# kfkq/DQMC

Hardware: AMD Instinct MI355X
Metric: MC sweeps/sec, 2D Hubbard N=256 Ltau=200 (higher is better)
Workload: dtype f64; 1 GPU; cfg3: 16x16 Hubbard U=8.0 beta=8.0 Ltau=200 n_stab=10 t=1 mu=-0.1; chains_per_gpu=1, n_chains_total=1, parallelism=independent chains, 1 gpu x 1 chain

## Files before the change

dqmc_amd/csrc/common.h:

```cpp
#pragma once

#include <hip/hip_runtime.h>
#include <cstdint>
#include <memory>
#include <string>

struct dqmc_engine;

namespace dq {

constexpr int WAVE = 64;

void set_error(const std::string& msg);
const char* get_error();

#define DQ_HIP(call)                                                                    \
    do {                                                                                \
        hipError_t _e = (call);                                                         \
        if (_e != hipSuccess) {                                                         \
            ::dq::set_error(std::string(#call) + ": " + hipGetErrorString(_e));         \
            return -2;                                              \
        }                                                                               \
    } while (0)

#define DQ_TRY(expr)                \
    do {                            \
        int _rc = (expr);           \
        if (_rc != 0) return _rc;   \
    } while (0)

template <class T, hipError_t (*Free)(void*)> struct HipDelete { void operator()(T* p) const { (void)Free(p); } };
template <class T> using DevPtr = std::unique_ptr<T[], HipDelete<T, hipFree>>;
using PinnedPtr = std::unique_ptr<char[], HipDelete<char, hipHostFree>>;
template <class T> int dev_alloc(DevPtr<T>& out, size_t count) {
    void* p = nullptr;
    DQ_HIP(hipMalloc(&p, sizeof(T) * count));
    out.reset(static_cast<T*>(p));
    return 0;
}

constexpr int DQ_STATUS_PIVOT = 1;
constexpr int DQ_STATUS_COOP_QR = 2;
constexpr int DQ_STATUS_HANDOFF = 4;
constexpr int DQ_STATUS_CENSUS = 8;

struct Mat {
    double* p = nullptr;
    long stride = 0;
    __host__ __device__ double* at(int c) const { return p + (long)c * stride; }
};
struct CMat {
    const double* p = nullptr;
    long stride = 0;
    CMat() = default;
    __host__ __device__ CMat(const double* p_, long s) : p(p_), stride(s) {}
    __host__ __device__ CMat(const Mat& m) : p(m.p), stride(m.stride) {}
    __host__ __device__ const double* at(int c) const { return p + (long)c * stride; }
};
using Vec = Mat;
using CVec = CMat;

struct GemmDesc {
    CMat A, B;
    Mat C;
    Mat CT{nullptr, 0};
    CVec rs, ks, cs;
    int n = 0;
    int transA = 0;
    int accumulate = 0;
};
int launch_gemm(const GemmDesc& g, int n_chains, hipStream_t s);

int launch_build_expv(const int8_t* fields, long f_stride, int nt, int n, const double* tab_expv ,
                      double* expv, double* invexpv, long v_stride, int n_chains, hipStream_t s);
int launch_split_d(CVec d, Vec dl_inv, Vec ds, double* logsum, int n, int n_chains, hipStream_t s);
int launch_split_d2(CVec d1, Vec dl1, Vec ds1, CVec d2, Vec dl2, Vec ds2, int n, int n_chains, hipStream_t s);
int launch_measure_equal_time(CMat G, double* out, long out_stride, int L1, int L2, int accumulate, int n_chains, hipStream_t s);
int launch_measure_unequal_time(const double* Gtt, const double* Gt0, const double* G0t, double* out, long out_stride, int L1, int L2, int nt,
                                int accumulate, int n_chains, hipStream_t s);
int launch_axpb_identity(CMat in, Mat out, double a, double b, int n, int n_chains, hipStream_t s);
int launch_copy(CMat in, Mat out, long count, int n_chains, hipStream_t s);
int launch_set_identity(Mat out, int n, int n_chains, hipStream_t s);
int launch_transpose_scale(CMat in, Mat out, CVec rs, int n, int n_chains, hipStream_t s);
int launch_max_abs_diff(CMat A, CMat B, double* err, long err_stride, int n, int n_chains, hipStream_t s);
int launch_add_scaled_cols(CMat A, CMat B, CVec cs, Mat C, int n, int n_chains, hipStream_t s);
int launch_scale_rows(CMat in, CVec rs, Mat out, int n, int n_chains, hipStream_t s);
struct DevStats { double acc_rate, max_err, sum_err, n_err; long long n_accepted, n_proposed; };
int launch_fold_stats(DevStats* st, const int* acc, long acc_stride, int n_slices, const double* err, long err_stride, int n_err,
                      int n, int nt, int n_chains, hipStream_t s);

struct QrWork {
    double* tau; long tau_stride;
    int* jpvt; long jpvt_stride;
    unsigned long long* sync = nullptr; long sync_stride = 0;
    int* abort_words = nullptr;
    int* info = nullptr;
    double* pw = nullptr; long pw_stride = 0;
    bool pw_two_launch = false;
    int* pivpos = nullptr; long pivpos_stride = 0;
};
bool qr_panel_fused_fits(int n);
bool qr_panel_fused_default(int n);
long qr_panel_work_doubles(int n, bool two_launch);
int launch_qr_panel(Mat A, Mat L, QrWork w, int n, int n_chains, hipStream_t s);
long qrcp_coop_sync_granules(int n);
int qrcp_coop_workgroups(int n, int n_chains);
enum class QrFamily { Panel, ColumnOwner, Cooperative, Streaming };
int launch_to_ldr(QrFamily f, Mat A, Mat L, Vec d, Mat R, QrWork w, int n, int n_chains, hipStream_t s);

int launch_lu_blocked(Mat A, int* perm, long perm_stride, int* rowpos, long rowpos_stride, double* logabsdet, int accumulate_logdet,
                      int* info, int n, int n_chains, hipStream_t s);
int launch_lu_solve(CMat LU, const int* perm, long perm_stride, Mat X, CVec dg, int mode, int n, int n_chains, hipStream_t s);

int launch_tri_solve(CMat R, const int* perm, long perm_stride, Mat X, CVec dg, double* scratch, long scratch_stride, int n, int n_chains, hipStream_t s);

bool gj_fused_fits(int n);
bool gj_fused_default(int n);
int launch_gj_solve(Mat A, Mat B, Mat X, Mat SA, double* tinv, int* perm, long perm_stride, int* rowpos, int* rowpos_alt, long rowpos_stride,
                    double* logabsdet, int accumulate_logdet, int* info, int n, int n_chains, bool fused, hipStream_t s);

struct UpdateTables {
    double rb[4][3];
    double delta[4][3];
    double ev[4];
    double iev[4];
    double pad[32];
};
struct SliceRider {
    const double* A = nullptr; const double* B = nullptr; double* C = nullptr; const double* rs = nullptr; const double* ks = nullptr;
    __host__ __device__ GemmDesc gemm(int n) const { GemmDesc g; g.A = CMat(A, 0); g.B = CMat(B, 0); g.C = Mat{C, 0}; g.rs = CVec(rs, 0); g.ks = CVec(ks, 0); g.n = n; return g; }
};
struct UpdateDesc {
    Mat G;
    int8_t* fields; long f_stride;
    double* expv; double* invexpv; long v_stride;
    const UpdateTables* tabs;
    const int32_t* perm; const uint8_t* kprop; const double* u; long rs_stride;
    double* Upanel; double* Wpanel; long panel_stride;
    double* Cpanel = nullptr;
    int* state; long state_stride;
    double* prep; long prep_stride;
    Mat GT{nullptr, 0};
    int gt_valid = 0;
    void* slice_sync = nullptr;
    unsigned slice_epoch = 0;
    int slice_absent_tile = -1;
    int slice_absent_l = -1;
    int slice_late_tile = -1, slice_late_us = 0;
    int* info = nullptr;
    int* acc_out; long acc_stride;
    int n, nt;
    SliceRider rider;
};
constexpr int UPDATE_KD = 32;

struct SliceSync {
    unsigned long long seq; unsigned int error; unsigned int solo_count; unsigned int pad[12];
    unsigned int arrive[496];
};
constexpr size_t SLICE_SYNC_BYTES = 2048;
static_assert(sizeof(SliceSync) == SLICE_SYNC_BYTES, "SliceSync layout");
constexpr unsigned SLICE_EPOCH_LIMIT = 1u << 24;
constexpr unsigned SLICE_SOLO_BIT = 1u << 30, SLICE_FINAL_BIT = 1u << 31;
constexpr int SLICE_RING_ROWS = 2 * UPDATE_KD;
constexpr unsigned SLICE_K_MASK = 0xffu, SLICE_BASE_SHIFT = 8, SLICE_BASE_MASK = SLICE_RING_ROWS - 1;
__host__ __device__ inline unsigned slice_tag(unsigned epoch, unsigned window) { return (epoch << 8) | window; }
enum class SlicePath { PersistentWalk, PersistentWalkDump, PersistentSubmatrix, Solo, Pairs, PairsTailSolo };
int launch_update_slice(SlicePath path, const UpdateDesc& d, int l, int acc_slot, int n_chains, hipStream_t s);
int launch_update_slice_sm(const UpdateDesc& d, int l, int acc_slot, int n_chains, hipStream_t s);
int slice_flush_workgroups(int n);
bool slice_reserve(int device, int n, int n_chains);
void slice_release(int device, int n, int n_chains);
int launch_rank1(Mat G, int i, double delta, double* scratch , long scratch_stride, int n, int n_chains, hipStream_t s);

int launch_rng_fill(int32_t* perm, uint8_t* kprop, double* u, int n, int nt, unsigned long long seed, unsigned first_chain, unsigned h,
                    int n_chains, hipStream_t s);

struct CbDesc {
    CMat in;
    Mat out{nullptr, 0}, outT{nullptr, 0};
    const int* partner = nullptr;
    int n_groups = 0, reverse = 0, inverse = 0;
    const double* par = nullptr; long par_stride = 0;
    CVec rs_in, cs_in, rs_out, cs_out;
    int n = 0;
};
int launch_cb_apply(const CbDesc& d, int n_chains, hipStream_t s);

int update_init_device();
int update_sm_init_device();
int qr_init_device();
int qr_colown_init_device();
int init_device_kernels(int device);

struct EngineFieldsView { int device, n, nt, n_chains; int8_t* fields; hipStream_t stream; };
int engine_fields_view(dqmc_engine* h, EngineFieldsView* v);
int engine_fields_changed(dqmc_engine* h);
int engine_exchange_scratch(dqmc_engine* h, int8_t** saved, int8_t** recv, int** tab);

}
```

dqmc_amd/csrc/engine.hip:

```cpp
#include "common.h"
#include "../../include/dqmc_hip.h"

#include <cmath>
#include <cstdlib>
#include <cstring>
#include <map>
#include <memory>
#include <mutex>
#include <vector>

namespace dq {

static thread_local std::string g_err;
void set_error(const std::string& msg) { g_err = msg; }
const char* get_error() { return g_err.c_str(); }

int init_device_kernels(int device) {
    static std::mutex mu; static bool done[64] = {};
    std::lock_guard<std::mutex> lk(mu);
    if (device < 0 || device >= 64) { set_error("device ordinal out of range"); return -1; }
    if (done[device]) return 0;
    DQ_HIP(hipSetDevice(device));
    DQ_TRY(update_init_device()); DQ_TRY(update_sm_init_device()); DQ_TRY(qr_init_device()); DQ_TRY(qr_colown_init_device());
    done[device] = true;
    return 0;
}

struct Switches { bool qr_panel; int qr_panel_fused, gj_fused; bool qr_streaming, walk_submatrix, lu_classic, slice_multikernel, bbar_rider, slice_stream; };
static const Switches& switches() {
    static const Switches sw = [] {
        const char* panel = getenv("DQMC_QR_PANEL");
        const char* fused = getenv("DQMC_QR_PANEL_FUSED");
        const char* gj = getenv("DQMC_GJ_FUSED");
        const char* rider = getenv("DQMC_BBAR_RIDER");
        const char* stream = getenv("DQMC_SLICE_STREAM");
        return Switches{!(panel && atoi(panel) == 0), fused ? (atoi(fused) != 0 ? 1 : 0) : -1, gj ? (atoi(gj) != 0 ? 1 : 0) : -1, getenv("DQMC_QR_STREAMING") != nullptr, getenv("DQMC_WALK_SUBMATRIX") != nullptr,
                        getenv("DQMC_LU_CLASSIC") != nullptr, getenv("DQMC_SLICE_MULTIKERNEL") != nullptr, !(rider && atoi(rider) == 0), !(stream && atoi(stream) == 0)};
    }();
    return sw;
}

constexpr int GJ_MAX_N = 1024, GJ_MAX_CHAINS = 8;
constexpr int TRI_MAX_N = 640;

static QrFamily pick_qr(int n, int chains, bool allow_panel) {
    const Switches& sw = switches();
    if (sw.qr_streaming) return QrFamily::Streaming;
    if (allow_panel && sw.qr_panel && n >= 64 && n <= 1024 && n % 16 == 0 && chains <= 8) return QrFamily::Panel;
    if (n <= 256) return QrFamily::ColumnOwner;
    return qrcp_coop_workgroups(n, chains) <= 200 ? QrFamily::Cooperative : QrFamily::Streaming;
}

struct KernelPlan {
    QrFamily qr;
    enum class Solve { GaussJordan, BlockedLu } solve;
    enum class Rinv { Blocked, PerColumn } rinv;
    static KernelPlan pick(int n, int chains) {
        return KernelPlan{pick_qr(n, chains, true),
                          n <= GJ_MAX_N && chains <= GJ_MAX_CHAINS && !switches().lu_classic ? Solve::GaussJordan : Solve::BlockedLu,
                          n <= TRI_MAX_N ? Rinv::Blocked : Rinv::PerColumn};
    }
};

static SlicePath pick_slice_path(int n, int chains, bool reserved) {
    const Switches& sw = switches();
    const bool walk = n <= 256;
    if (sw.slice_multikernel) return SlicePath::Pairs;
    if (reserved) return walk && !sw.walk_submatrix ? (sw.slice_stream ? SlicePath::PersistentWalk : SlicePath::PersistentWalkDump) : SlicePath::PersistentSubmatrix;
    if (!walk) return SlicePath::Pairs;
    return chains >= 224 ? SlicePath::Solo : SlicePath::PairsTailSolo;
}
static bool is_persistent_walk(SlicePath p) { return p == SlicePath::PersistentWalk || p == SlicePath::PersistentWalkDump; }
static bool is_persistent(SlicePath p) { return is_persistent_walk(p) || p == SlicePath::PersistentSubmatrix; }

struct LdrRef {
    Mat L; Vec d; Mat R;
    int* jpvt = nullptr;
    bool* tri = nullptr;
    Mat X{nullptr, 0};
    bool* xok = nullptr;
    void touch() const { if (xok) *xok = false; }
};
struct LdrStore {
    int n = 0, C = 0;
    DevPtr<double> L, d, R, X;
    DevPtr<int> jpvt;
    std::unique_ptr<bool[]> tri, xok;
    int alloc(int k, int n_, int C_, bool with_x = false) {
        n = n_; C = C_;
        const size_t nn = (size_t)n * n;
        DQ_TRY(dev_alloc(L, (size_t)k * C * nn)); DQ_TRY(dev_alloc(d, (size_t)k * C * n));
        DQ_TRY(dev_alloc(R, (size_t)k * C * nn)); DQ_TRY(dev_alloc(jpvt, (size_t)k * C * n));
        if (with_x) DQ_TRY(dev_alloc(X, (size_t)k * C * nn));
        tri.reset(new bool[k]()); xok.reset(new bool[k]());
        return 0;
    }
    LdrRef at(int i) const {
        const long nn = (long)n * n;
        LdrRef f{Mat{L.get() + (long)i * C * nn, nn}, Vec{d.get() + (long)i * C * n, (long)n}, Mat{R.get() + (long)i * C * nn, nn},
                 jpvt.get() + (long)i * C * n, &tri[i]};
        if (X) { f.X = Mat{X.get() + (long)i * C * nn, nn}; f.xok = &xok[i]; }
        return f;
    }
};

struct Ctx {
    int n = 0, C = 0, device = 0;
    long nn = 0;
    hipStream_t stream = nullptr;
    static constexpr int NT = 6, NV = 5;
    DevPtr<double> pool;
    DevPtr<double> vpool;
    DevPtr<int> ipool;
    DevPtr<unsigned long long> qsync;
    DevPtr<int> qabort;
    DevPtr<double> tinv;
    DevPtr<double> qpw;
    bool gj_fused = false;
    bool qpw_two_launch = false;
    DevPtr<int> qpivpos;
    DevPtr<double> trinv;
    KernelPlan plan{};

    Mat T(int k) const { return Mat{pool.get() + (long)k * C * nn, nn}; }
    Vec V(int k) const { return Vec{vpool.get() + (long)k * C * n, (long)n}; }
    int* jpvt() const { return ipool.get(); }
    int* lperm() const { return ipool.get() + (long)C * n; }
    int* rowpos() const { return ipool.get() + 2L * C * n; }
    int* rowpos_alt() const { return ipool.get() + 3L * C * n; }
    int* info() const { return ipool.get() + 4L * C * n; }

    int init(int n_, int C_, int device_) {
        n = n_; C = C_; device = device_; nn = (long)n * n;
        DQ_HIP(hipSetDevice(device));
        DQ_TRY(init_device_kernels(device));
        DQ_HIP(hipStreamCreateWithFlags(&stream, hipStreamNonBlocking));
        DQ_TRY(dev_alloc(pool, (size_t)NT * C * nn));
        DQ_TRY(dev_alloc(vpool, (size_t)NV * C * n));
        DQ_TRY(dev_alloc(ipool, 4L * C * n + 4));
        plan = KernelPlan::pick(n, C);
        if (plan.qr == QrFamily::Cooperative) { DQ_TRY(dev_alloc(qsync, (size_t)qrcp_coop_sync_granules(n) * C)); DQ_TRY(dev_alloc(qabort, C)); }
        if (plan.qr == QrFamily::Panel) {
            const int fused = switches().qr_panel_fused;
            qpw_two_launch = !(fused < 0 ? qr_panel_fused_default(n) : fused == 1 && qr_panel_fused_fits(n));
            const size_t qpw_count = (size_t)qr_panel_work_doubles(n, qpw_two_launch) * C;
            DQ_TRY(dev_alloc(qpw, qpw_count)); DQ_TRY(dev_alloc(qpivpos, (size_t)n * C));
            DQ_HIP(hipMemsetAsync(qpw.get(), 0, sizeof(double) * qpw_count, stream));
        }
        if (plan.solve == KernelPlan::Solve::GaussJordan) {
            DQ_TRY(dev_alloc(tinv, (size_t)2048 * C));
            const int fused = switches().gj_fused;
            gj_fused = fused < 0 ? gj_fused_default(n) : fused == 1 && gj_fused_fits(n);
        }
        if (plan.rinv == KernelPlan::Rinv::Blocked) DQ_TRY(dev_alloc(trinv, (size_t)16 * (n + 16) * C));
        DQ_HIP(hipMemsetAsync(ipool.get(), 0, sizeof(int) * (4L * C * n + 4), stream));
        return 0;
    }
    ~Ctx() { if (stream) (void)hipStreamDestroy(stream); }

    int gemm(CMat A, CMat B, Mat Cm, CVec rs = CVec(), CVec ks = CVec(), CVec cs = CVec(), int transA = 0, int accumulate = 0, Mat CT = Mat{nullptr, 0}) {
        GemmDesc g; g.A = A; g.B = B; g.C = Cm; g.CT = CT; g.rs = rs; g.ks = ks; g.cs = cs; g.n = n; g.transA = transA; g.accumulate = accumulate;
        return launch_gemm(g, C, stream);
    }
    int to_ldr(Mat A, LdrRef out, bool direct = true) {
        const bool keep = direct && out.jpvt != nullptr;
        QrWork w{V(4).p, (long)n, keep ? out.jpvt : jpvt(), (long)n};
        w.sync = qsync.get(); w.sync_stride = qrcp_coop_sync_granules(n); w.abort_words = qabort.get(); w.info = info();
        w.pw = qpw.get(); w.pw_stride = qr_panel_work_doubles(n, qpw_two_launch); w.pw_two_launch = qpw_two_launch; w.pivpos = qpivpos.get(); w.pivpos_stride = n;
        if (out.tri) *out.tri = keep;
        out.touch();
        return launch_to_ldr(plan.qr, A, out.L, out.d, out.R, w, n, C, stream);
    }
    int r_inverse_scaled(LdrRef F, CVec dinv, Mat scratch, Mat lu_scratch, Mat* Xout) {
        const Mat X = F.X.p ? F.X : scratch;
        *Xout = X;
        if (F.xok && *F.xok) return 0;
        if (F.tri && *F.tri && F.jpvt) {
            if (plan.rinv == KernelPlan::Rinv::Blocked) DQ_TRY(launch_tri_solve(F.R, F.jpvt, n, X, dinv, trinv.get(), 16L * (n + 16), n, C, stream));
            else DQ_TRY(launch_lu_solve(F.R, F.jpvt, n, X, dinv, 2, n, C, stream));
        } else {
            DQ_TRY(launch_copy(F.R, lu_scratch, nn, C, stream));
            DQ_TRY(launch_lu_blocked(lu_scratch, lperm(), n, rowpos(), n, nullptr, 0, info(), n, C, stream));
            DQ_TRY(launch_lu_solve(lu_scratch, lperm(), n, X, dinv, 1, n, C, stream));
        }
        if (F.xok) *F.xok = true;
        return 0;
    }
    int mat_mul_ldr(CMat M, LdrRef F, LdrRef out) {
        DQ_TRY(gemm(M, F.L, T(0), CVec(), CVec(), CVec(F.d)));
        LdrRef q{out.L, out.d, T(1)};
        DQ_TRY(to_ldr(T(0), q));
        if (out.tri) *out.tri = false;
        out.touch();
        return gemm(T(1), F.R, out.R);
    }
    int ldr_mul_mat(LdrRef F, CMat M, LdrRef out) {
        DQ_TRY(gemm(F.R, M, T(0), CVec(F.d)));
        LdrRef q{T(1), out.d, out.R, out.jpvt, out.tri};
        q.xok = out.xok;
        DQ_TRY(to_ldr(T(0), q));
        return gemm(F.L, T(1), out.L);
    }
    int ldr_mul_ldr(LdrRef F1, LdrRef F2, LdrRef out) {
        DQ_TRY(gemm(F1.R, F2.L, T(0), CVec(F1.d), CVec(), CVec(F2.d)));
        LdrRef q{T(1), out.d, T(2)};
        DQ_TRY(to_ldr(T(0), q));
        if (out.tri) *out.tri = false;
        out.touch();
        DQ_TRY(gemm(F1.L, T(1), out.L));
        return gemm(T(2), F2.R, out.R);
    }
    int solve(Mat M, Mat RHS, Mat out, double* logdet_acc, Mat* Y) {
        if (plan.solve == KernelPlan::Solve::GaussJordan) {
            DQ_TRY(launch_gj_solve(M, RHS, out, T(5), tinv.get(), lperm(), n, rowpos(), rowpos_alt(), n, logdet_acc, 1, info(), n, C, gj_fused, stream));
            *Y = out; return 0;
        }
        DQ_TRY(launch_lu_blocked(M, lperm(), n, rowpos(), n, logdet_acc, 1, info(), n, C, stream));
        DQ_TRY(launch_lu_solve(M, lperm(), n, RHS, CVec(), 0, n, C, stream));
        *Y = RHS; return 0;
    }
    int inv_I_plus_ldr(LdrRef F, Mat G, double* logdet ) {
        DQ_TRY(launch_split_d(F.d, V(0), V(1), logdet, n, C, stream));
        Mat X; DQ_TRY(r_inverse_scaled(F, V(0), T(1), T(0), &X));
        DQ_TRY(launch_add_scaled_cols(X, F.L, V(1), T(2), n, C, stream));
        DQ_TRY(launch_transpose_scale(T(2), T(3), CVec(), n, C, stream));
        DQ_TRY(launch_transpose_scale(X, T(4), CVec(), n, C, stream));
        Mat Y; DQ_TRY(solve(T(3), T(4), T(0), logdet, &Y));
        return launch_transpose_scale(Y, G, CVec(), n, C, stream);
    }
    int inv_I_plus_ldr_mul_ldr(LdrRef F1, LdrRef F2, Mat G, Mat GT = Mat{nullptr, 0}) {
        DQ_TRY(launch_split_d2(F1.d, V(0), V(1), F2.d, V(2), V(3), n, C, stream));
        Mat X; DQ_TRY(r_inverse_scaled(F2, V(2), T(1), T(0), &X));
        DQ_TRY(gemm(F1.L, X, T(2), V(0), CVec(), CVec(), 1));
        DQ_TRY(gemm(F1.R, F2.L, T(2), V(1), CVec(), V(3), 0, 1));
        DQ_TRY(launch_transpose_scale(F1.L, T(3), V(0), n, C, stream));
        Mat Y; DQ_TRY(solve(T(2), T(3), T(0), nullptr, &Y));
        return gemm(X, Y, G, CVec(), CVec(), CVec(), 0, 0, GT);
    }
    int inv_invldr_plus_ldr(LdrRef F1, LdrRef F2, Mat G, bool negate) {
        DQ_TRY(launch_split_d(F1.d, V(0), V(1), nullptr, n, C, stream));
        DQ_TRY(launch_split_d(F2.d, V(2), V(3), nullptr, n, C, stream));
        Mat X; DQ_TRY(r_inverse_scaled(F2, V(2), T(1), T(0), &X));
        DQ_TRY(gemm(F1.L, X, T(2), V(0), CVec(), CVec(), 1));
        DQ_TRY(gemm(F1.R, F2.L, T(2), V(1), CVec(), V(3), 0, 1));
        DQ_TRY(launch_scale_rows(F1.R, V(1), T(3), n, C, stream));
        Mat Y; DQ_TRY(solve(T(2), T(3), T(0), nullptr, &Y));
        DQ_TRY(gemm(X, Y, G));
        if (negate) DQ_TRY(launch_axpb_identity(G, G, -1.0, 0.0, n, C, stream));
        return 0;
    }
};

static int take_status(const Ctx& c, int* bits = nullptr) {
    int w[4] = {0, 0, 0, 0};
    DQ_HIP(hipMemcpy(w, c.info(), sizeof w, hipMemcpyDeviceToHost));
    if (bits) *bits = w[0];
    if (w[0] == 0) return 0;
    (void)hipMemset(c.info(), 0, sizeof w);
    if (w[0] & DQ_STATUS_HANDOFF) {
        set_error("persistent slice kernel: a workgroup that had checked in stopped answering (device fault or pre-emption beyond the spin bound); the chain state is undefined -- set the fields again and call dqmc_init; this engine uses the scan / flush kernel pairs from now on");
    } else if (w[0] & DQ_STATUS_CENSUS) {
        char msg[640];
        snprintf(msg, sizeof msg, "persistent sub-matrix slice kernel: its workgroups did not all become resident at time slice %d (device shared with other "
                 "work?).  That slice and every later slice of the call(s) in flight proposed NOTHING (fields unchanged there, acceptance counts 0, their part of "
                 "the random stream is spent); wraps and stabilisations ran, so fields, G and the stack are consistent with each other, but the sweep is not the "
                 "one the stream describes from that slice on.  This engine uses the scan / flush kernel pairs from now on: restore the fields of the last "
                 "completed sweep and call dqmc_init, or keep the state as a valid (shortened) sweep", w[1] - 1);
        set_error(msg);
    } else if (w[0] & DQ_STATUS_COOP_QR) {
        set_error("cooperative QRCP gave up waiting for a partner workgroup (not co-resident?)");
    } else {
        set_error("LU factorisation hit a zero or NaN pivot");
    }
    return DQMC_ENUMERIC;
}

struct Engine {
    int n = 0, nt = 0, n_stab = 0, n_stack = 0, C = 1, device = 0;
    long nn = 0;
    std::vector<int> loc_l_end;
    std::vector<double> g_host, gamma_host, eta_host;
    std::vector<unsigned char> seen;
    Ctx ctx;
    hipStream_t s = nullptr;

    DevPtr<double> expK, invexpK;
    bool cb = false; int cb_groups = 0;
    DevPtr<int> cb_partner;
    DevPtr<double> cb_par;
    DevPtr<int8_t> fields;
    DevPtr<double> expv, invexpv;
    DevPtr<UpdateTables> tabs; DevPtr<double> tab8;
    bool gt_valid = false;
    bool gt_check = false; long long gt_checks = 0; DevPtr<double> gt_err;
    DevPtr<double> G, Gtmp, GT;
    DevPtr<double> pg_eye, pg_ones;
    DevPtr<double> bb0, bb1;
    long long rider_launches = 0;
    LdrStore stack;
    LdrStore spare;
    DevPtr<double> logdet;
    DevPtr<int32_t> rs_perm; DevPtr<uint8_t> rs_k; DevPtr<double> rs_u;
    PinnedPtr h_stage;
    bool rng_seeded = false; uint64_t rng_seed = 0; uint32_t rng_first_chain = 0, rng_counter = 0;
    hipEvent_t stage_free = nullptr;
    DevPtr<double> Upanel, Wpanel;
    int panel_rows = UPDATE_KD;
    DevPtr<double> Cpanel;
    struct InitBatch { DevPtr<double> bb, tau; LdrStore f; } ib;
    DevPtr<int> state;
    DevPtr<double> prep;
    DevPtr<double> meas_now, meas_sum;
    struct UnequalTime { DevPtr<double> G[3], tmp, err, meas_now, meas_sum; LdrStore bt; } ut;
    bool ut_valid = false; long long ut_meas_count = 0;
    struct HalfWarp { DevPtr<double> expK, invexpK, out; } hw;
    long long meas_count = 0;
    DevPtr<char> slice_sync;
    bool reserved = false;
    SlicePath slice_path = SlicePath::Pairs;
    unsigned slice_epoch = 0;
    int slice_absent_l = -1;
    int slice_late_tile = -1, slice_late_us = 0;
    int slice_absent_tile = -1;
    DevPtr<int> acc;
    struct Exchange { DevPtr<int8_t> saved, recv; DevPtr<int> tab; } xch;
    DevPtr<double> err;
    DevPtr<DevStats> dstats;
    bool stack_valid = false;
    bool profiling = false;
    std::vector<std::pair<hipEvent_t, hipEvent_t>> ev_pairs;
    size_t ev_used = 0;
    double upd_ms = 0.0; long long upd_launches = 0; long long upd_accept_base = 0;

    Mat mG() const { return Mat{G.get(), nn}; }
    CVec ev(int l) const { return CVec(expv.get() + (long)l * n, (long)nt * n); }
    CVec iev(int l) const { return CVec(invexpv.get() + (long)l * n, (long)nt * n); }
    int stack_idx(int l) const { return l / n_stab; }
    int local_l(int l) const { return l % n_stab; }

    ~Engine() {
        if (s) (void)hipStreamSynchronize(s);
        if (reserved) slice_release(device, n, C);
        for (auto& p : ev_pairs) { (void)hipEventDestroy(p.first); (void)hipEventDestroy(p.second); }
        if (stage_free) (void)hipEventDestroy(stage_free);
    }

    int create(int device_, int C_, int n_, int nt_, int n_stab_, const double* g, const double* gamma, const double* eta,
               const double* eK, const double* ieK) {
        device = device_; C = C_; n = n_; nt = nt_; n_stab = n_stab_; nn = (long)n * n;
        n_stack = (int)std::ceil(static_cast<double>(nt) / n_stab);
        loc_l_end.assign(n_stack, n_stab - 1);
        if (nt % n_stab != 0) loc_l_end[n_stack - 1] = nt % n_stab - 1;
        g_host.assign(g, g + C); gamma_host.assign(gamma, gamma + 4); eta_host.assign(eta, eta + 4);
        DQ_TRY(ctx.init(n, C, device)); s = ctx.stream;
        reserved = slice_reserve(device, n, C);
        slice_path = pick_slice_path(n, C, reserved);
        if (const char* a = getenv("DQMC_DEBUG_SLICE_ABSENT")) { slice_absent_tile = atoi(a); if (const char* c = strchr(a, ':')) slice_absent_l = atoi(c + 1); }
        if (const char* a = getenv("DQMC_DEBUG_SLICE_LATE")) { slice_late_tile = atoi(a); if (const char* c = strchr(a, ':')) slice_late_us = atoi(c + 1); }
        DQ_TRY(dev_alloc(expK, C * nn)); DQ_TRY(dev_alloc(invexpK, C * nn));
        DQ_TRY(dev_alloc(fields, (size_t)C * nt * n)); DQ_TRY(dev_alloc(expv, (size_t)C * nt * n)); DQ_TRY(dev_alloc(invexpv, (size_t)C * nt * n));
        DQ_TRY(dev_alloc(tabs, C)); DQ_TRY(dev_alloc(tab8, (size_t)C * 8));
        if (C == 1) { DQ_TRY(dev_alloc(pg_eye, nn)); DQ_TRY(dev_alloc(pg_ones, (size_t)n)); DQ_TRY(launch_set_identity(Mat{pg_eye.get(), nn}, n, 1, s)); const std::vector<double> one_h((size_t)n, 1.0); DQ_HIP(hipMemcpy(pg_ones.get(), one_h.data(), sizeof(double) * n, hipMemcpyHostToDevice)); }
        DQ_TRY(dev_alloc(G, C * nn)); DQ_TRY(dev_alloc(Gtmp, C * nn)); DQ_TRY(dev_alloc(GT, C * nn)); DQ_TRY(dev_alloc(bb0, C * nn)); DQ_TRY(dev_alloc(bb1, C * nn));
        DQ_TRY(stack.alloc(n_stack, n, C, C <= 8)); DQ_TRY(spare.alloc(1, n, C));
        DQ_TRY(dev_alloc(logdet, C));
        DQ_TRY(dev_alloc(rs_perm, (size_t)C * nt * n)); DQ_TRY(dev_alloc(rs_k, (size_t)C * nt * n)); DQ_TRY(dev_alloc(rs_u, (size_t)C * nt * n));
        panel_rows = slice_path == SlicePath::PersistentWalk ? SLICE_RING_ROWS : UPDATE_KD;
        DQ_TRY(dev_alloc(Upanel, (size_t)C * panel_rows * n)); DQ_TRY(dev_alloc(Wpanel, (size_t)C * panel_rows * n)); DQ_TRY(dev_alloc(Cpanel, (size_t)C * UPDATE_KD * UPDATE_KD));
        DQ_TRY(dev_alloc(state, (size_t)C * 4)); DQ_TRY(dev_alloc(prep, (size_t)C * 4 * n)); DQ_TRY(dev_alloc(meas_now, (size_t)C * (3 + n))); DQ_TRY(dev_alloc(meas_sum, (size_t)C * (3 + n))); DQ_HIP(hipMemsetAsync(meas_sum.get(), 0, sizeof(double) * C * (3 + n), s)); DQ_TRY(dev_alloc(slice_sync, (size_t)C * SLICE_SYNC_BYTES)); DQ_HIP(hipMemsetAsync(slice_sync.get(), 0, (size_t)C * SLICE_SYNC_BYTES, s)); DQ_TRY(dev_alloc(acc, (size_t)C * nt)); DQ_TRY(dev_alloc(err, (size_t)C * n_stack));
        DQ_TRY(dev_alloc(dstats, C));
        void* stage = nullptr;
        DQ_HIP(hipHostMalloc(&stage, (size_t)C * nt * n * (sizeof(int32_t) + sizeof(uint8_t) + sizeof(double)), hipHostMallocDefault)); h_stage.reset(static_cast<char*>(stage));
        DQ_HIP(hipEventCreateWithFlags(&stage_free, hipEventDisableTiming));
        DQ_HIP(hipEventRecord(stage_free, s));
        DQ_HIP(hipMemcpyAsync(expK.get(), eK, sizeof(double) * C * nn, hipMemcpyHostToDevice, s));
        DQ_HIP(hipMemcpyAsync(invexpK.get(), ieK, sizeof(double) * C * nn, hipMemcpyHostToDevice, s));
        DQ_HIP(hipMemsetAsync(fields.get(), 0, (size_t)C * nt * n, s));
        DQ_HIP(hipMemsetAsync(G.get(), 0, sizeof(double) * C * nn, s));
        DQ_HIP(hipMemsetAsync(dstats.get(), 0, sizeof(DevStats) * C, s));
        DQ_HIP(hipMemsetAsync(logdet.get(), 0, sizeof(double) * C, s));
        DQ_HIP(hipMemsetAsync(state.get(), 0, sizeof(int) * C * 4, s));
        std::vector<UpdateTables> ht(C); std::vector<double> h8((size_t)C * 8);
        static const int proposal[4][3] = {{1, 2, 3}, {0, 2, 3}, {0, 1, 3}, {0, 1, 2}};
        const double alpha = -1.0;
        for (int c = 0; c < C; ++c) {
            std::memset(&ht[c], 0, sizeof(UpdateTables));
            for (int o = 0; o < 4; ++o) for (int k = 0; k < 3; ++k) {
                const int nf = proposal[o][k];
                const double gammaR = gamma[nf] / gamma[o];
                const double d_eta = eta[nf] - eta[o];
                const double bosonR = std::exp(alpha * g[c] * d_eta);
                ht[c].rb[o][k] = gammaR * bosonR;
                ht[c].delta[o][k] = (1.0 / bosonR) - 1.0;
            }
            for (int f = 0; f < 4; ++f) { ht[c].ev[f] = std::exp(g[c] * eta[f]); ht[c].iev[f] = std::exp(-g[c] * eta[f]); h8[(size_t)c * 8 + f] = ht[c].ev[f]; h8[(size_t)c * 8 + 4 + f] = ht[c].iev[f]; }
        }
        DQ_HIP(hipMemcpyAsync(tabs.get(), ht.data(), sizeof(UpdateTables) * C, hipMemcpyHostToDevice, s));
        DQ_HIP(hipMemcpyAsync(tab8.get(), h8.data(), sizeof(double) * C * 8, hipMemcpyHostToDevice, s));
        DQ_TRY(launch_build_expv(fields.get(), (long)nt * n, nt, n, tab8.get(), expv.get(), invexpv.get(), (long)nt * n, C, s));
        DQ_HIP(hipStreamSynchronize(s));
        return 0;
    }

    int cb_apply(CMat in, Mat out, Mat outT, bool reverse, bool inverse, CVec rs_in, CVec cs_in, CVec rs_out, CVec cs_out, int chains, long par_stride) {
        CbDesc d; d.in = in; d.out = out; d.outT = outT; d.partner = cb_partner.get(); d.n_groups = cb_groups; d.reverse = reverse ? 1 : 0; d.inverse = inverse ? 1 : 0;
        d.par = cb_par.get(); d.par_stride = par_stride; d.rs_in = rs_in; d.cs_in = cs_in; d.rs_out = rs_out; d.cs_out = cs_out; d.n = n;
        return launch_cb_apply(d, chains, s);
    }
    int set_checkerboard(int n_groups, const int32_t* bonds, const int32_t* group_sizes, const double* ch, const double* sh, const double* f) {
        if (n_groups < 1 || n_groups > 64 || !bonds || !group_sizes || !ch || !sh || !f) { set_error("set_checkerboard: bad argument"); return DQMC_EINVAL; }
        if (n > 4096) { set_error("set_checkerboard: n_sites > 4096"); return DQMC_EINVAL; }
        std::vector<int> partner((size_t)n_groups * n);
        size_t b = 0;
        for (int g = 0; g < n_groups; ++g) {
            int* pt = partner.data() + (size_t)g * n;
            for (int i = 0; i < n; ++i) pt[i] = i;
            if (group_sizes[g] < 0 || group_sizes[g] > n / 2) { set_error("set_checkerboard: a group holds at most n_sites/2 bonds"); return DQMC_EINVAL; }
            for (int k = 0; k < group_sizes[g]; ++k, ++b) {
                const int i = bonds[2 * b], j = bonds[2 * b + 1];
                if (i < 0 || i >= n || j < 0 || j >= n || i == j) { set_error("set_checkerboard: bond site out of range"); return DQMC_EINVAL; }
                if (pt[i] != i || pt[j] != j) { set_error("set_checkerboard: the bonds of one group must be disjoint"); return DQMC_EINVAL; }
                pt[i] = j; pt[j] = i;
            }
        }
        std::vector<double> par((size_t)C * 4);
        for (int c = 0; c < C; ++c) {
            if (!(f[c] > 0.0) || !std::isfinite(ch[c]) || !std::isfinite(sh[c])) { set_error("set_checkerboard: diag_factor must be positive, cosh / sinh finite"); return DQMC_EINVAL; }
            par[4 * c] = ch[c]; par[4 * c + 1] = sh[c]; par[4 * c + 2] = f[c]; par[4 * c + 3] = 1.0 / f[c];
        }
        DQ_HIP(hipStreamSynchronize(s));
        if (!cb_par) DQ_TRY(dev_alloc(cb_par, (size_t)C * 4));
        DevPtr<int> pt;
        DQ_TRY(dev_alloc(pt, partner.size()));
        DQ_HIP(hipMemcpy(pt.get(), partner.data(), sizeof(int) * partner.size(), hipMemcpyHostToDevice));
        DQ_HIP(hipMemcpy(cb_par.get(), par.data(), sizeof(double) * par.size(), hipMemcpyHostToDevice));
        cb_partner = std::move(pt); cb_groups = n_groups; cb = true;
        Mat id{bb0.get(), nn};
        DQ_TRY(launch_set_identity(id, n, C, s));
        DQ_TRY(cb_apply(id, Mat{expK.get(), nn}, Mat{nullptr, 0}, false, false, CVec(), CVec(), CVec(), CVec(), C, 4));
        DQ_TRY(cb_apply(id, Mat{invexpK.get(), nn}, Mat{nullptr, 0}, true, true, CVec(), CVec(), CVec(), CVec(), C, 4));
        stack_valid = false; gt_valid = false; ut_valid = false;
        DQ_HIP(hipStreamSynchronize(s));
        return 0;
    }

    int Bbar(int is, Mat* out) {
        const int l0 = is * n_stab;
        Mat cur{bb0.get(), nn}, nxt{bb1.get(), nn};
        DQ_TRY(launch_scale_rows(CMat(expK.get(), nn), ev(l0), cur, n, C, s));
        for (int loc = 1; loc <= loc_l_end[is]; ++loc) {
            if (cb) DQ_TRY(cb_apply(cur, nxt, Mat{nullptr, 0}, false, false, CVec(), CVec(), ev(l0 + loc), CVec(), C, 4));
            else DQ_TRY(ctx.gemm(CMat(expK.get(), nn), cur, nxt, ev(l0 + loc)));
            std::swap(cur, nxt);
        }
        *out = cur; return 0;
    }
    int init() {
        if (C == 1 && n <= 256 && nt % n_stab == 0 && n_stack >= 2) return init_batched();
        const LdrRef tmp = spare.at(0);
        for (int i = n_stack - 1; i >= 0; --i) {
            Mat bb; DQ_TRY(Bbar(i, &bb));
            if (i == n_stack - 1) DQ_TRY(ctx.to_ldr(bb, stack.at(i)));
            else { DQ_TRY(ctx.to_ldr(bb, tmp)); DQ_TRY(ctx.ldr_mul_ldr(stack.at(i + 1), tmp, stack.at(i))); }
        }
        stack_valid = true;
        gt_valid = false;
        return ctx.inv_I_plus_ldr(stack.at(0), mG(), logdet.get());
    }
    int init_batched() {
        const int S = n_stack;
        if (!ib.tau) {
            InitBatch b; DQ_TRY(dev_alloc(b.bb, (size_t)2 * S * nn)); DQ_TRY(dev_alloc(b.tau, (size_t)S * n)); DQ_TRY(b.f.alloc(S, n, 1));
            ib = std::move(b);
        }
        const long bstride = (long)n_stab * n;
        Mat cur{ib.bb.get(), nn}, nxt{ib.bb.get() + (size_t)S * nn, nn};
        DQ_TRY(launch_scale_rows(CMat(expK.get(), 0), CVec(expv.get(), bstride), cur, n, S, s));
        for (int loc = 1; loc < n_stab; ++loc) {
            if (cb) DQ_TRY(cb_apply(cur, nxt, Mat{nullptr, 0}, false, false, CVec(), CVec(), CVec(expv.get() + (long)loc * n, bstride), CVec(), S, 0));
            else {
                GemmDesc g; g.A = CMat(expK.get(), 0); g.B = cur; g.C = nxt; g.rs = CVec(expv.get() + (long)loc * n, bstride); g.n = n;
                DQ_TRY(launch_gemm(g, S, s));
            }
            std::swap(cur, nxt);
        }
        const LdrRef all = ib.f.at(0);
        QrWork w{ib.tau.get(), (long)n, all.jpvt, (long)n};
        w.info = ctx.info();
        DQ_TRY(launch_to_ldr(pick_qr(n, S, false), cur, all.L, all.d, all.R, w, n, S, s));
        const LdrRef last = stack.at(S - 1), own = ib.f.at(S - 1);
        DQ_TRY(launch_copy(own.L, last.L, nn, 1, s));
        DQ_TRY(launch_copy(own.R, last.R, nn, 1, s));
        DQ_HIP(hipMemcpyAsync(last.d.p, own.d.p, sizeof(double) * n, hipMemcpyDeviceToDevice, s));
        DQ_HIP(hipMemcpyAsync(last.jpvt, own.jpvt, sizeof(int) * n, hipMemcpyDeviceToDevice, s));
        *last.tri = true; last.touch();
        for (int i = S - 2; i >= 0; --i) DQ_TRY(ctx.ldr_mul_ldr(stack.at(i + 1), ib.f.at(i), stack.at(i)));
        stack_valid = true;
        gt_valid = false;
        return ctx.inv_I_plus_ldr(stack.at(0), mG(), logdet.get());
    }
    int wrap_forward(int l) {
        if (cb) {
            DQ_TRY(cb_apply(mG(), Mat{nullptr, 0}, ctx.T(0), false, false, CVec(), CVec(), CVec(), CVec(), C, 4));
            gt_valid = use_gt();
            return cb_apply(ctx.T(0), Mat{GT.get(), nn}, mG(), false, true, CVec(), CVec(), iev(l), ev(l), C, 4);
        }
        DQ_TRY(ctx.gemm(CMat(expK.get(), nn), mG(), ctx.T(0)));
        gt_valid = use_gt();
        return ctx.gemm(ctx.T(0), CMat(invexpK.get(), nn), mG(), ev(l), CVec(), iev(l), 0, 0, use_gt() ? Mat{GT.get(), nn} : Mat{nullptr, 0});
    }
    bool piggyback() const { return C == 1 && !cb && n <= 256 && pg_eye != nullptr; }
    bool bbar_rides() const { return piggyback() && is_persistent_walk(slice_path) && switches().bbar_rider; }
    SliceRider rider_forward(int l, const double* Pprev, double* Pnext) const {
        SliceRider r; r.A = expK.get(); r.B = Pprev; r.C = Pnext; r.rs = expv.get() + (long)(l - 1) * n;
        return r;
    }
    SliceRider rider_backward(int l, const double* Pprev, double* Pnext) const {
        SliceRider r; r.A = Pprev; r.B = expK.get(); r.C = Pnext; r.ks = expv.get() + (long)l * n;
        return r;
    }
    int wrap_forward_piggy(int l, const double* Pprev, double* Pnext) {
        GemmDesc g; g.A = CMat(expK.get(), 0); g.B = CMat(G.get(), (long)(Pprev - G.get())); g.C = Mat{ctx.T(0).p, (long)(Pnext - ctx.T(0).p)};
        g.rs = CVec(pg_ones.get(), (long)((expv.get() + (long)(l - 1) * n) - pg_ones.get())); g.n = n;
        DQ_TRY(launch_gemm(g, 2, s));
        gt_valid = use_gt();
        return ctx.gemm(ctx.T(0), CMat(invexpK.get(), nn), mG(), ev(l), CVec(), iev(l), 0, 0, use_gt() ? Mat{GT.get(), nn} : Mat{nullptr, 0});
    }
    int wrap_backward_piggy(int l, const double* Pprev, double* Pnext) {
        DQ_TRY(ctx.gemm(CMat(invexpK.get(), nn), mG(), ctx.T(0), CVec(), iev(l)));
        gt_valid = use_gt();
        GemmDesc g; g.A = CMat(ctx.T(0).p, (long)(Pprev - ctx.T(0).p)); g.B = CMat(expK.get(), 0); g.C = Mat{G.get(), (long)(Pnext - G.get())};
        g.ks = CVec(expv.get() + (long)l * n, 0); g.n = n;
        if (use_gt()) g.CT = Mat{GT.get(), (long)(ctx.T(1).p - GT.get())};
        return launch_gemm(g, 2, s);
    }
    int wrap_backward(int l) {
        if (cb) {
            DQ_TRY(cb_apply(mG(), Mat{nullptr, 0}, ctx.T(0), true, true, iev(l), ev(l), CVec(), CVec(), C, 4));
            gt_valid = use_gt();
            return cb_apply(ctx.T(0), Mat{GT.get(), nn}, mG(), true, false, CVec(), CVec(), CVec(), CVec(), C, 4);
        }
        DQ_TRY(ctx.gemm(CMat(invexpK.get(), nn), mG(), ctx.T(0), CVec(), iev(l)));
        gt_valid = use_gt();
        return ctx.gemm(ctx.T(0), CMat(expK.get(), nn), mG(), CVec(), ev(l), CVec(), 0, 0, use_gt() ? Mat{GT.get(), nn} : Mat{nullptr, 0});
    }
    bool use_gt() const { return n <= 256 || slice_path == SlicePath::PersistentSubmatrix; }
    UpdateDesc udesc() const {
        UpdateDesc d; d.G = mG(); d.fields = fields.get(); d.f_stride = (long)nt * n; d.expv = expv.get(); d.invexpv = invexpv.get(); d.v_stride = (long)nt * n;
        d.tabs = tabs.get(); d.perm = rs_perm.get(); d.kprop = rs_k.get(); d.u = rs_u.get(); d.rs_stride = (long)nt * n; d.Upanel = Upanel.get(); d.Wpanel = Wpanel.get(); d.Cpanel = Cpanel.get();
        d.panel_stride = (long)panel_rows * n; d.state = state.get(); d.state_stride = 4; d.prep = prep.get(); d.prep_stride = 4L * n; d.slice_sync = is_persistent(slice_path) ? slice_sync.get() : nullptr; d.slice_epoch = slice_epoch; d.slice_absent_tile = slice_absent_tile; d.slice_absent_l = slice_absent_l; d.slice_late_tile = slice_late_tile; d.slice_late_us = slice_late_us; d.GT = Mat{GT.get(), nn}; d.gt_valid = gt_valid ? 1 : 0; d.info = ctx.info(); d.acc_out = acc.get(); d.acc_stride = nt; d.n = n; d.nt = nt;
        return d;
    }
    int local_update(int l, const SliceRider* rider = nullptr) {
        hipEvent_t e0 = nullptr, e1 = nullptr;
        if (profiling) {
            if (ev_used == ev_pairs.size()) { hipEvent_t a, b; DQ_HIP(hipEventCreate(&a)); DQ_HIP(hipEventCreate(&b)); ev_pairs.emplace_back(a, b); }
            e0 = ev_pairs[ev_used].first; e1 = ev_pairs[ev_used].second; ++ev_used;
            DQ_HIP(hipEventRecord(e0, s));
        }
        if (is_persistent(slice_path)) {
            if (++slice_epoch >= SLICE_EPOCH_LIMIT) { DQ_HIP(hipMemsetAsync(slice_sync.get(), 0, (size_t)C * SLICE_SYNC_BYTES, s)); slice_epoch = 1; }
        }
        UpdateDesc d = udesc();
        if (rider) d.rider = *rider;
        DQ_TRY(launch_update_slice(slice_path, d, l, l, C, s));
        if (rider) ++rider_launches;
        if (profiling) DQ_HIP(hipEventRecord(e1, s));
        return 0;
    }
    int check_stream(const char* who, const int32_t* perm, const uint8_t* kprop, const double* u, size_t rows) {
        if (!perm || !kprop || !u) { set_error(std::string(who) + ": null random-stream pointer"); return DQMC_EINVAL; }
        seen.assign((size_t)n, 0);
        for (size_t row = 0; row < rows; ++row) {
            const int32_t* pr = perm + row * n; const uint8_t* kr = kprop + row * n; const unsigned char mark = (unsigned char)(1 + (row & 1));
            if ((row & 1) == 0) std::fill(seen.begin(), seen.end(), 0);
            for (int idx = 0; idx < n; ++idx) {
                const int32_t i = pr[idx];
                if (i < 0 || i >= n || seen[i] == mark || kr[idx] > 2) { set_error(std::string(who) + ": perm is not a permutation of the sites, or kprop > 2"); return DQMC_EINVAL; }
                seen[i] = mark;
            }
        }
        return 0;
    }
    int upload_stream(const int32_t* perm, const uint8_t* kprop, const double* u) {
        const size_t cnt = (size_t)C * nt * n;
        DQ_TRY(check_stream("sweep", perm, kprop, u, (size_t)C * nt));
        DQ_HIP(hipEventSynchronize(stage_free));
        char* base = h_stage.get();
        double* hu = reinterpret_cast<double*>(base);
        int32_t* hp = reinterpret_cast<int32_t*>(base + cnt * sizeof(double));
        uint8_t* hk = reinterpret_cast<uint8_t*>(base + cnt * (sizeof(double) + sizeof(int32_t)));
        std::memcpy(hu, u, cnt * sizeof(double)); std::memcpy(hp, perm, cnt * sizeof(int32_t)); std::memcpy(hk, kprop, cnt);
        DQ_HIP(hipMemcpyAsync(rs_u.get(), hu, cnt * sizeof(double), hipMemcpyHostToDevice, s));
        DQ_HIP(hipMemcpyAsync(rs_perm.get(), hp, cnt * sizeof(int32_t), hipMemcpyHostToDevice, s));
        DQ_HIP(hipMemcpyAsync(rs_k.get(), hk, cnt, hipMemcpyHostToDevice, s));
        DQ_HIP(hipEventRecord(stage_free, s));
        return 0;
    }
    int fill_stream(uint32_t h) {
        return launch_rng_fill(rs_perm.get(), rs_k.get(), rs_u.get(), n, nt, rng_seed, rng_first_chain, h, C, s);
    }
    int stage_stream(const char* who, const int32_t* perm, const uint8_t* kprop, const double* u) {
        if (perm && kprop && u) return upload_stream(perm, kprop, u);
        if (perm || kprop || u) { set_error(std::string(who) + ": pass all three random-stream arrays or none"); return DQMC_EINVAL; }
        if (!rng_seeded) { set_error(std::string(who) + ": null random-stream pointer (the engine draws its own stream only after dqmc_rng_seed)"); return DQMC_EINVAL; }
        if (rng_counter == UINT32_MAX) { set_error(std::string(who) + ": the half-sweep counter of this seed is used up (2^32 - 1)"); return DQMC_ERANGE; }
        DQ_TRY(fill_stream(rng_counter));
        ++rng_counter;
        return 0;
    }
    int sweep_fwd() {
        int n_err = 0;
        DQ_HIP(hipMemsetAsync(err.get(), 0, sizeof(double) * C * n_stack, s));
        const bool pg = piggyback(), ride = bbar_rides();
        double* Pcur = bb0.get(); double* Pnxt = bb1.get();
        for (int l = 0; l < nt; ++l) {
            const int is = stack_idx(l), loc = local_l(l);
            if (pg && loc >= 1) {
                const double* Pprev = loc == 1 ? pg_eye.get() : Pcur;
                if (ride) { const SliceRider r = rider_forward(l, Pprev, Pnxt); DQ_TRY(wrap_forward(l)); DQ_TRY(local_update(l, &r)); }
                else { DQ_TRY(wrap_forward_piggy(l, Pprev, Pnxt)); DQ_TRY(local_update(l)); }
                std::swap(Pcur, Pnxt);
            } else { DQ_TRY(wrap_forward(l)); DQ_TRY(local_update(l)); }
            if (loc == loc_l_end[is]) {
                std::swap(G, Gtmp);
                Mat bb;
                if (pg) {
                    if (loc == 0) DQ_TRY(launch_scale_rows(CMat(expK.get(), nn), ev(l), Mat{Pnxt, nn}, n, C, s));
                    else DQ_TRY(ctx.gemm(CMat(expK.get(), nn), CMat(Pcur, nn), Mat{Pnxt, nn}, ev(l)));
                    std::swap(Pcur, Pnxt); bb = Mat{Pcur, nn};
                } else DQ_TRY(Bbar(is, &bb));
                if (is == 0) DQ_TRY(ctx.to_ldr(bb, stack.at(0)));
                else DQ_TRY(ctx.mat_mul_ldr(bb, stack.at(is - 1), stack.at(is)));
                gt_valid = false;
                if (l == nt - 1) DQ_TRY(ctx.inv_I_plus_ldr(stack.at(is), mG(), logdet.get()));
                else DQ_TRY(ctx.inv_I_plus_ldr_mul_ldr(stack.at(is), stack.at(is + 1), mG()));
                DQ_TRY(launch_max_abs_diff(CMat(Gtmp.get(), nn), mG(), err.get() + n_err, n_stack, n, C, s));
                ++n_err;
            }
        }
        return launch_fold_stats(dstats.get(), acc.get(), nt, nt, err.get(), n_stack, n_err, n, nt, C, s);
    }
    int sweep_bwd() {
        int n_err = 0;
        DQ_HIP(hipMemsetAsync(err.get(), 0, sizeof(double) * C * n_stack, s));
        const bool pg = piggyback(), ride = bbar_rides();
        double* Pcur = bb0.get(); double* Pnxt = bb1.get();
        SliceRider pending; bool have_pending = false;
        for (int l = nt - 1; l >= 0; --l) {
            DQ_TRY(local_update(l, have_pending ? &pending : nullptr));
            if (have_pending) { std::swap(Pcur, Pnxt); have_pending = false; }
            const int is = stack_idx(l);
            if (pg) {
                const double* Pprev = local_l(l) == loc_l_end[is] ? pg_eye.get() : Pcur;
                if (ride && local_l(l) != 0) { DQ_TRY(wrap_backward(l)); pending = rider_backward(l, Pprev, Pnxt); have_pending = true; }
                else { DQ_TRY(wrap_backward_piggy(l, Pprev, Pnxt)); std::swap(Pcur, Pnxt); }
            } else DQ_TRY(wrap_backward(l));
            if (local_l(l) == 0) {
                std::swap(G, Gtmp);
                Mat bb;
                if (pg) bb = Mat{Pcur, nn}; else DQ_TRY(Bbar(is, &bb));
                if (is == n_stack - 1) DQ_TRY(ctx.to_ldr(bb, stack.at(is)));
                else DQ_TRY(ctx.ldr_mul_mat(stack.at(is + 1), bb, stack.at(is)));
                gt_valid = false;
                if (l == 0) DQ_TRY(ctx.inv_I_plus_ldr(stack.at(is), mG(), logdet.get()));
                else {
                    DQ_TRY(ctx.inv_I_plus_ldr_mul_ldr(stack.at(is - 1), stack.at(is), mG(), use_gt() ? Mat{GT.get(), nn} : Mat{nullptr, 0}));
                    gt_valid = use_gt();
                    if (gt_check && gt_valid) {
                        DQ_TRY(launch_transpose_scale(mG(), ctx.T(0), CVec(), n, C, s));
                        DQ_TRY(launch_max_abs_diff(CMat(GT.get(), nn), ctx.T(0), gt_err.get(), 1, n, C, s));
                        ++gt_checks;
                    }
                }
                DQ_TRY(launch_max_abs_diff(CMat(Gtmp.get(), nn), mG(), err.get() + n_err, n_stack, n, C, s));
                ++n_err;
            }
        }
        return launch_fold_stats(dstats.get(), acc.get(), nt, nt, err.get(), n_stack, n_err, n, nt, C, s);
    }
    Mat utm(int which, int l) const { return Mat{ut.G[which].get() + (long)l * C * nn, nn}; }
    int sweep_unequal() {
        if (!ut.tmp) {
            UnequalTime u;
            for (int w = 0; w < 3; ++w) DQ_TRY(dev_alloc(u.G[w], (size_t)(nt + 1) * C * nn));
            DQ_TRY(dev_alloc(u.tmp, (size_t)3 * C * nn)); DQ_TRY(dev_alloc(u.err, (size_t)C * 3 * n_stack));
            const size_t mcount = (size_t)C * 3 * (nt + 1) * n;
            DQ_TRY(dev_alloc(u.meas_now, mcount)); DQ_TRY(dev_alloc(u.meas_sum, mcount)); DQ_TRY(u.bt.alloc(2, n, C));
            DQ_HIP(hipMemsetAsync(u.meas_sum.get(), 0, sizeof(double) * mcount, s));
            ut = std::move(u);
        }
        auto bt = [&](int b) { return ut.bt.at(b); };
        int cur = 0, n_err = 0;
        DQ_HIP(hipMemsetAsync(ut.err.get(), 0, sizeof(double) * C * 3 * n_stack, s));
        DQ_TRY(launch_copy(mG(), utm(0, 0), nn, C, s));
        for (int l = 0; l < nt; ++l) {
            if (l == 0) {
                DQ_TRY(launch_copy(utm(0, 0), utm(1, 0), nn, C, s));
                DQ_TRY(launch_axpb_identity(utm(0, 0), utm(2, 0), 1.0, -1.0, n, C, s));
            }
            DQ_TRY(ctx.gemm(CMat(expK.get(), nn), utm(0, l), ctx.T(0)));
            DQ_TRY(ctx.gemm(ctx.T(0), CMat(invexpK.get(), nn), utm(0, l + 1), ev(l), CVec(), iev(l)));
            DQ_TRY(ctx.gemm(CMat(expK.get(), nn), utm(1, l), utm(1, l + 1), ev(l)));
            DQ_TRY(ctx.gemm(utm(2, l), CMat(invexpK.get(), nn), utm(2, l + 1), CVec(), CVec(), iev(l)));
            const int is = stack_idx(l);
            if (local_l(l) == loc_l_end[is]) {
                for (int w = 0; w < 3; ++w) DQ_TRY(launch_copy(utm(w, l + 1), Mat{ut.tmp.get() + (long)w * C * nn, nn}, nn, C, s));
                Mat bb; DQ_TRY(Bbar(is, &bb));
                if (is == 0) DQ_TRY(ctx.to_ldr(bb, bt(cur)));
                else { DQ_TRY(ctx.mat_mul_ldr(bb, bt(cur), bt(cur ^ 1))); cur ^= 1; }
                if (l == nt - 1) {
                    DQ_TRY(ctx.inv_I_plus_ldr(bt(cur), utm(0, l + 1), logdet.get()));
                    DQ_TRY(launch_axpb_identity(utm(0, l + 1), utm(1, l + 1), -1.0, 1.0, n, C, s));
                    DQ_TRY(launch_axpb_identity(utm(0, l + 1), utm(2, l + 1), -1.0, 0.0, n, C, s));
                } else {
                    DQ_TRY(ctx.inv_I_plus_ldr_mul_ldr(bt(cur), stack.at(is + 1), utm(0, l + 1)));
                    DQ_TRY(ctx.inv_invldr_plus_ldr(bt(cur), stack.at(is + 1), utm(1, l + 1), false));
                    DQ_TRY(ctx.inv_invldr_plus_ldr(stack.at(is + 1), bt(cur), utm(2, l + 1), true));
                }
                for (int w = 0; w < 3; ++w) {
                    DQ_TRY(launch_max_abs_diff(CMat(ut.tmp.get() + (long)w * C * nn, nn), utm(w, l + 1), ut.err.get() + n_err, 3L * n_stack, n, C, s));
                    ++n_err;
                }
            }
        }
        ut_valid = true;
        return launch_fold_stats(dstats.get(), acc.get(), nt, 0, ut.err.get(), 3L * n_stack, n_err, n, nt, C, s);
    }
    int sync_and_check() {
        DQ_HIP(hipStreamSynchronize(s));
        if (profiling && ev_used) {
            for (size_t k = 0; k < ev_used; ++k) { float ms = 0.f; DQ_HIP(hipEventElapsedTime(&ms, ev_pairs[k].first, ev_pairs[k].second)); upd_ms += ms; }
            upd_launches += (long long)ev_used; ev_used = 0;
        }
        int bits = 0;
        const int rc = take_status(ctx, &bits);
        if (bits & (DQ_STATUS_HANDOFF | DQ_STATUS_CENSUS)) {
            slice_path = pick_slice_path(n, C, false); gt_valid = false;
            if (bits & DQ_STATUS_HANDOFF) { (void)hipMemset(slice_sync.get(), 0, (size_t)C * SLICE_SYNC_BYTES); slice_epoch = 0; }
        }
        return rc;
    }
    int download_fields(std::vector<int8_t>& f) const {
        std::vector<int8_t> dev((size_t)C * nt * n);
        DQ_HIP(hipMemcpy(dev.data(), fields.get(), dev.size(), hipMemcpyDeviceToHost));
        f.resize(dev.size());
        for (int c = 0; c < C; ++c) for (int i = 0; i < n; ++i) for (int l = 0; l < nt; ++l)
            f[(size_t)c * nt * n + l + (size_t)nt * i] = dev[(size_t)c * nt * n + (size_t)l * n + i];
        return 0;
    }
    int copy_out_equal_time(const double* src, double* scalars, double* chi_r) const {
        const size_t w = 3 + (size_t)n;
        std::vector<double> tmp((size_t)C * w);
        DQ_HIP(hipMemcpy(tmp.data(), src, sizeof(double) * tmp.size(), hipMemcpyDeviceToHost));
        for (int c = 0; c < C; ++c) {
            if (scalars) std::copy(tmp.begin() + c * w, tmp.begin() + c * w + 3, scalars + 3 * (size_t)c);
            if (chi_r) std::copy(tmp.begin() + c * w + 3, tmp.begin() + (c + 1) * w, chi_r + (size_t)c * n);
        }
        return 0;
    }
};

struct Stateless {
    Ctx ctx;
    LdrStore ldr;
    DevPtr<double> mats;
    DevPtr<double> logdet;
    Mat M(int k) const { return Mat{mats.get() + k * ctx.nn, ctx.nn}; }
};
static std::mutex g_ctx_mu;
static std::map<int, std::unique_ptr<Stateless>> g_ctx;

static int get_ctx(int n, Stateless** out) {
    if (n <= 0) { set_error("n must be positive"); return DQMC_EINVAL; }
    int count = 0;
    if (hipGetDeviceCount(&count) != hipSuccess || count == 0) { set_error("no HIP device available: this library requires a gfx950 GPU"); return DQMC_ENODEVICE; }
    auto it = g_ctx.find(n);
    if (it == g_ctx.end()) {
        std::unique_ptr<Stateless> x(new Stateless);
        DQ_TRY(x->ctx.init(n, 1, 0));
        DQ_TRY(x->ldr.alloc(3, n, 1)); DQ_TRY(dev_alloc(x->mats, 4L * n * n)); DQ_TRY(dev_alloc(x->logdet, 1));
        it = g_ctx.emplace(n, std::move(x)).first;
    }
    *out = it->second.get();
    return hipSetDevice(0) == hipSuccess ? 0 : DQMC_ENODEVICE;
}
static int upload_ldr(Stateless* x, int k, const double* L, const double* d, const double* R, LdrRef* out) {
    const Ctx& c = x->ctx;
    *out = x->ldr.at(k); *out->tri = false;
    DQ_HIP(hipMemcpyAsync(out->L.p, L, sizeof(double) * c.nn, hipMemcpyHostToDevice, c.stream));
    DQ_HIP(hipMemcpyAsync(out->R.p, R, sizeof(double) * c.nn, hipMemcpyHostToDevice, c.stream));
    DQ_HIP(hipMemcpyAsync(out->d.p, d, sizeof(double) * c.n, hipMemcpyHostToDevice, c.stream));
    return 0;
}
static int download_ldr(Ctx* c, LdrRef f, double* L, double* d, double* R) {
    DQ_HIP(hipMemcpyAsync(L, f.L.p, sizeof(double) * c->nn, hipMemcpyDeviceToHost, c->stream));
    DQ_HIP(hipMemcpyAsync(R, f.R.p, sizeof(double) * c->nn, hipMemcpyDeviceToHost, c->stream));
    DQ_HIP(hipMemcpyAsync(d, f.d.p, sizeof(double) * c->n, hipMemcpyDeviceToHost, c->stream));
    DQ_HIP(hipStreamSynchronize(c->stream));
    return take_status(*c);
}

}

using namespace dq;

struct dqmc_engine { Engine e; };

#define ENGINE_CALL(h) if (!(h)) { set_error("null engine"); return DQMC_EINVAL; } Engine& e = (h)->e; DQ_HIP(hipSetDevice(e.device))

namespace dq {
int engine_fields_view(dqmc_engine* h, EngineFieldsView* v) {
    if (!h || !v) { set_error("null engine"); return DQMC_EINVAL; }
    Engine& e = h->e;
    v->device = e.device; v->n = e.n; v->nt = e.nt; v->n_chains = e.C; v->fields = e.fields.get(); v->stream = e.s;
    return 0;
}
int engine_fields_changed(dqmc_engine* h) {
    ENGINE_CALL(h);
    e.stack_valid = false; e.gt_valid = false;
    return launch_build_expv(e.fields.get(), (long)e.nt * e.n, e.nt, e.n, e.tab8.get(), e.expv.get(), e.invexpv.get(), (long)e.nt * e.n, e.C, e.s);
}
int engine_exchange_scratch(dqmc_engine* h, int8_t** saved, int8_t** recv, int** tab) {
    ENGINE_CALL(h);
    if (!e.xch.tab) {
        Engine::Exchange x; DQ_TRY(dev_alloc(x.saved, (size_t)e.C * e.nt * e.n)); DQ_TRY(dev_alloc(x.recv, (size_t)2 * e.nt * e.n)); DQ_TRY(dev_alloc(x.tab, (size_t)2 * e.C));
        e.xch = std::move(x);
    }
    *saved = e.xch.saved.get(); *recv = e.xch.recv.get(); *tab = e.xch.tab.get();
    return 0;
}
}

#define API_LOCK std::lock_guard<std::mutex> _lk(g_ctx_mu)

extern "C" {

const char* dqmc_last_error(void) { return get_error(); }
const char* dqmc_backend(void) { return "hip:gfx950"; }
int dqmc_device_count(void) { int c = 0; if (hipGetDeviceCount(&c) != hipSuccess) return 0; return c; }

int dqmc_to_ldr(int n, const double* M, double* L, double* d, double* R) {
    API_LOCK; Stateless* x; DQ_TRY(get_ctx(n, &x)); Ctx* c = &x->ctx;
    if (!M || !L || !d || !R) { set_error("null pointer"); return DQMC_EINVAL; }
    DQ_HIP(hipMemcpyAsync(x->M(0).p, M, sizeof(double) * c->nn, hipMemcpyHostToDevice, c->stream));
    LdrRef out = x->ldr.at(0);
    DQ_TRY(c->to_ldr(x->M(0), out));
    return download_ldr(c, out, L, d, R);
}
int dqmc_ldr_mul_mat(int n, const double* L, const double* d, const double* R, const double* M, double* Lo, double* d_o, double* Ro) {
    API_LOCK; Stateless* x; DQ_TRY(get_ctx(n, &x)); Ctx* c = &x->ctx;
    LdrRef F; DQ_TRY(upload_ldr(x, 0, L, d, R, &F));
    DQ_HIP(hipMemcpyAsync(x->M(0).p, M, sizeof(double) * c->nn, hipMemcpyHostToDevice, c->stream));
    LdrRef out = x->ldr.at(2);
    DQ_TRY(c->ldr_mul_mat(F, x->M(0), out));
    return download_ldr(c, out, Lo, d_o, Ro);
}
int dqmc_mat_mul_ldr(int n, const double* M, const double* L, const double* d, const double* R, double* Lo, double* d_o, double* Ro) {
    API_LOCK; Stateless* x; DQ_TRY(get_ctx(n, &x)); Ctx* c = &x->ctx;
    LdrRef F; DQ_TRY(upload_ldr(x, 0, L, d, R, &F));
    DQ_HIP(hipMemcpyAsync(x->M(0).p, M, sizeof(double) * c->nn, hipMemcpyHostToDevice, c->stream));
    LdrRef out = x->ldr.at(2);
    DQ_TRY(c->mat_mul_ldr(x->M(0), F, out));
    return download_ldr(c, out, Lo, d_o, Ro);
}
int dqmc_ldr_mul_ldr(int n, const double* L1, const double* d1, const double* R1, const double* L2, const double* d2, const double* R2, double* Lo, double* d_o, double* Ro) {
    API_LOCK; Stateless* x; DQ_TRY(get_ctx(n, &x)); Ctx* c = &x->ctx;
    LdrRef F1, F2; DQ_TRY(upload_ldr(x, 0, L1, d1, R1, &F1)); DQ_TRY(upload_ldr(x, 1, L2, d2, R2, &F2));
    LdrRef out = x->ldr.at(2);
    DQ_TRY(c->ldr_mul_ldr(F1, F2, out));
    return download_ldr(c, out, Lo, d_o, Ro);
}
int dqmc_inv_I_plus_ldr(int n, const double* L, const double* d, const double* R, double* G, double* logdet) {
    API_LOCK; Stateless* x; DQ_TRY(get_ctx(n, &x)); Ctx* c = &x->ctx;
    LdrRef F; DQ_TRY(upload_ldr(x, 0, L, d, R, &F));
    DQ_TRY(c->inv_I_plus_ldr(F, x->M(1), x->logdet.get()));
    DQ_HIP(hipMemcpyAsync(G, x->M(1).p, sizeof(double) * c->nn, hipMemcpyDeviceToHost, c->stream));
    double ld = 0.0;
    DQ_HIP(hipMemcpyAsync(&ld, x->logdet.get(), sizeof(double), hipMemcpyDeviceToHost, c->stream));
    DQ_HIP(hipStreamSynchronize(c->stream));
    if (logdet) *logdet = ld;
    return take_status(*c);
}
int dqmc_inv_I_plus_ldr_mul_ldr(int n, const double* L1, const double* d1, const double* R1, const double* L2, const double* d2, const double* R2, double* G) {
    API_LOCK; Stateless* x; DQ_TRY(get_ctx(n, &x)); Ctx* c = &x->ctx;
    LdrRef F1, F2; DQ_TRY(upload_ldr(x, 0, L1, d1, R1, &F1)); DQ_TRY(upload_ldr(x, 1, L2, d2, R2, &F2));
    DQ_TRY(c->inv_I_plus_ldr_mul_ldr(F1, F2, x->M(1)));
    DQ_HIP(hipMemcpyAsync(G, x->M(1).p, sizeof(double) * c->nn, hipMemcpyDeviceToHost, c->stream));
    DQ_HIP(hipStreamSynchronize(c->stream));
    return take_status(*c);
}
int dqmc_gemm(int n, const double* A, int transA, const double* B, int transB, double* Cm) {
    API_LOCK; Stateless* x; DQ_TRY(get_ctx(n, &x)); Ctx* c = &x->ctx;
    DQ_HIP(hipMemcpyAsync(x->M(0).p, A, sizeof(double) * c->nn, hipMemcpyHostToDevice, c->stream));
    DQ_HIP(hipMemcpyAsync(x->M(1).p, B, sizeof(double) * c->nn, hipMemcpyHostToDevice, c->stream));
    CMat Bm = x->M(1);
    if (transB) { DQ_TRY(launch_transpose_scale(x->M(1), x->M(2), CVec(), n, 1, c->stream)); Bm = x->M(2); }
    DQ_TRY(c->gemm(x->M(0), Bm, x->M(3), CVec(), CVec(), CVec(), transA ? 1 : 0));
    DQ_HIP(hipMemcpyAsync(Cm, x->M(3).p, sizeof(double) * c->nn, hipMemcpyDeviceToHost, c->stream));
    DQ_HIP(hipStreamSynchronize(c->stream));
    return 0;
}
int dqmc_rank1_update(int n, double* G, int i, double delta) {
    API_LOCK; Stateless* x; DQ_TRY(get_ctx(n, &x)); Ctx* c = &x->ctx;
    if (i < 0 || i >= n) { set_error("site index out of range"); return DQMC_ERANGE; }
    DQ_HIP(hipMemcpyAsync(x->M(0).p, G, sizeof(double) * c->nn, hipMemcpyHostToDevice, c->stream));
    DQ_TRY(launch_rank1(x->M(0), i, delta, x->M(1).p, 2L * n + 1, n, 1, c->stream));
    DQ_HIP(hipMemcpyAsync(G, x->M(0).p, sizeof(double) * c->nn, hipMemcpyDeviceToHost, c->stream));
    DQ_HIP(hipStreamSynchronize(c->stream));
    return 0;
}

int dqmc_create_batch(dqmc_engine** out, int device, int n_chains, int n_sites, int nt, int n_stab, const double* g,
                      const double gamma[4], const double eta[4], const double* expK, const double* invexpK) {
    if (!out || n_chains <= 0 || n_sites <= 0 || nt <= 0 || n_stab <= 0 || !g || !gamma || !eta || !expK || !invexpK) { set_error("bad argument"); return DQMC_EINVAL; }
    if (n_sites > 1024) { set_error("n_sites > 1024 is not supported by the single-workgroup kernels"); return DQMC_EINVAL; }
    int count = 0;
    if (hipGetDeviceCount(&count) != hipSuccess || count == 0) { set_error("no HIP device available: this library requires a gfx950 GPU"); return DQMC_ENODEVICE; }
    if (device < 0 || device >= count) { set_error("device ordinal out of range"); return DQMC_EINVAL; }
    dqmc_engine* h = new (std::nothrow) dqmc_engine;
    if (!h) return DQMC_ENOMEM;
    int rc = h->e.create(device, n_chains, n_sites, nt, n_stab, g, gamma, eta, expK, invexpK);
    if (rc) { delete h; return rc; }
    *out = h; return 0;
}
int dqmc_create(dqmc_engine** out, int device, int n_sites, int nt, int n_stab, double g, const double gamma[4], const double eta[4],
                const double* expK, const double* invexpK) {
    return dqmc_create_batch(out, device, 1, n_sites, nt, n_stab, &g, gamma, eta, expK, invexpK);
}
int dqmc_set_checkerboard(dqmc_engine* h, int n_groups, const int32_t* bonds, const int32_t* group_sizes, const double* cosh_t, const double* sinh_t,
                          const double* diag_factor) {
    ENGINE_CALL(h);
    return e.set_checkerboard(n_groups, bonds, group_sizes, cosh_t, sinh_t, diag_factor);
}
void dqmc_destroy(dqmc_engine* h) { if (h) { (void)hipSetDevice(h->e.device); delete h; } }
int dqmc_n_chains(dqmc_engine* h) { return h ? h->e.C : 0; }

int dqmc_set_fields(dqmc_engine* h, const int64_t* f) {
    ENGINE_CALL(h);
    std::vector<int8_t> tmp((size_t)e.C * e.nt * e.n);
    for (int c = 0; c < e.C; ++c) for (int i = 0; i < e.n; ++i) for (int l = 0; l < e.nt; ++l) {
        const int64_t v = f[(size_t)c * e.nt * e.n + l + (size_t)e.nt * i];
        if (v < 0 || v > 3) { set_error("field value outside {0,1,2,3}"); return DQMC_EINVAL; }
        tmp[(size_t)c * e.nt * e.n + (size_t)l * e.n + i] = (int8_t)v;
    }
    DQ_HIP(hipStreamSynchronize(e.s));
    DQ_HIP(hipMemcpy(e.fields.get(), tmp.data(), tmp.size(), hipMemcpyHostToDevice));
    DQ_TRY(launch_build_expv(e.fields.get(), (long)e.nt * e.n, e.nt, e.n, e.tab8.get(), e.expv.get(), e.invexpv.get(), (long)e.nt * e.n, e.C, e.s));
    DQ_HIP(hipStreamSynchronize(e.s));
    return 0;
}
int dqmc_get_fields(dqmc_engine* h, int64_t* f) {
    ENGINE_CALL(h);
    DQ_TRY(e.sync_and_check());
    std::vector<int8_t> tmp; DQ_TRY(e.download_fields(tmp));
    std::copy(tmp.begin(), tmp.end(), f);
    return 0;
}
int dqmc_init(dqmc_engine* h) { ENGINE_CALL(h); DQ_TRY(e.init()); return e.sync_and_check(); }
int dqmc_get_G(dqmc_engine* h, double* G) {
    ENGINE_CALL(h); DQ_TRY(e.sync_and_check());
    DQ_HIP(hipMemcpy(G, e.G.get(), sizeof(double) * e.C * e.nn, hipMemcpyDeviceToHost)); return 0;
}
int dqmc_set_G(dqmc_engine* h, const double* G) {
    ENGINE_CALL(h); DQ_HIP(hipStreamSynchronize(e.s));
    DQ_HIP(hipMemcpy(e.G.get(), G, sizeof(double) * e.C * e.nn, hipMemcpyHostToDevice)); e.gt_valid = false; return 0;
}
int dqmc_get_logdet(dqmc_engine* h, double* ld) {
    ENGINE_CALL(h); DQ_TRY(e.sync_and_check());
    DQ_HIP(hipMemcpy(ld, e.logdet.get(), sizeof(double) * e.C, hipMemcpyDeviceToHost)); return 0;
}
int dqmc_n_stack(dqmc_engine* h) { return h ? h->e.n_stack : 0; }
int dqmc_get_stack(dqmc_engine* h, int i, double* L, double* d, double* R) {
    ENGINE_CALL(h);
    if (i < 0 || i >= e.n_stack) { set_error("LDR Stack index out of bounds"); return DQMC_ERANGE; }
    if (!e.stack_valid) { set_error("stack not initialised: call dqmc_init first"); return DQMC_EINVAL; }
    DQ_TRY(e.sync_and_check());
    LdrRef f = e.stack.at(i);
    DQ_HIP(hipMemcpy(L, f.L.p, sizeof(double) * e.C * e.nn, hipMemcpyDeviceToHost));
    DQ_HIP(hipMemcpy(R, f.R.p, sizeof(double) * e.C * e.nn, hipMemcpyDeviceToHost));
    DQ_HIP(hipMemcpy(d, f.d.p, sizeof(double) * e.C * e.n, hipMemcpyDeviceToHost));
    return 0;
}
int dqmc_sweep_0_to_beta(dqmc_engine* h, const int32_t* perm, const uint8_t* kprop, const double* u) {
    ENGINE_CALL(h);
    if (!e.stack_valid) { set_error("dqmc_init must be called before sweeping"); return DQMC_EINVAL; }
    DQ_TRY(e.stage_stream("sweep_0_to_beta", perm, kprop, u)); return e.sweep_fwd();
}
int dqmc_sweep_beta_to_0(dqmc_engine* h, const int32_t* perm, const uint8_t* kprop, const double* u) {
    ENGINE_CALL(h);
    if (!e.stack_valid) { set_error("dqmc_init must be called before sweeping"); return DQMC_EINVAL; }
    DQ_TRY(e.stage_stream("sweep_beta_to_0", perm, kprop, u)); return e.sweep_bwd();
}
int dqmc_sync(dqmc_engine* h) { ENGINE_CALL(h); return e.sync_and_check(); }
int dqmc_rng_seed(dqmc_engine* h, uint64_t seed, uint32_t first_chain, uint32_t counter) {
    ENGINE_CALL(h);
    if ((uint64_t)first_chain + (uint64_t)e.C - 1 > UINT32_MAX) { set_error("rng_seed: first_chain + n_chains - 1 exceeds 32 bits"); return DQMC_EINVAL; }
    e.rng_seeded = true; e.rng_seed = seed; e.rng_first_chain = first_chain; e.rng_counter = counter;
    return 0;
}
int dqmc_rng_state(dqmc_engine* h, uint64_t* seed, uint32_t* first_chain, uint32_t* counter, int* seeded) {
    if (!h) { set_error("null engine"); return DQMC_EINVAL; }
    const Engine& e = h->e;
    if (seed) *seed = e.rng_seed;
    if (first_chain) *first_chain = e.rng_first_chain;
    if (counter) *counter = e.rng_counter;
    if (seeded) *seeded = e.rng_seeded ? 1 : 0;
    return 0;
}
int dqmc_rng_draw(dqmc_engine* h, uint32_t counter, int32_t* perm, uint8_t* kprop, double* u) {
    ENGINE_CALL(h);
    if (!perm || !kprop || !u) { set_error("rng_draw: null pointer"); return DQMC_EINVAL; }
    if (!e.rng_seeded) { set_error("rng_draw: the engine has no seed (dqmc_rng_seed)"); return DQMC_EINVAL; }
    DQ_TRY(e.fill_stream(counter));
    DQ_TRY(e.sync_and_check());
    const size_t cnt = (size_t)e.C * e.nt * e.n;
    DQ_HIP(hipMemcpy(perm, e.rs_perm.get(), cnt * sizeof(int32_t), hipMemcpyDeviceToHost));
    DQ_HIP(hipMemcpy(kprop, e.rs_k.get(), cnt, hipMemcpyDeviceToHost));
    DQ_HIP(hipMemcpy(u, e.rs_u.get(), cnt * sizeof(double), hipMemcpyDeviceToHost));
    return 0;
}
int dqmc_get_stats(dqmc_engine* h, dqmc_stats* out) {
    ENGINE_CALL(h); DQ_TRY(e.sync_and_check());
    static_assert(sizeof(DevStats) == sizeof(dqmc_stats), "stats layout");
    DQ_HIP(hipMemcpy(out, e.dstats.get(), sizeof(DevStats) * e.C, hipMemcpyDeviceToHost)); return 0;
}
int dqmc_wrap_forward(dqmc_engine* h, int l) {
    ENGINE_CALL(h);
    if (l < 0 || l >= e.nt) { set_error("time slice out of range"); return DQMC_ERANGE; }
    return e.wrap_forward(l);
}
int dqmc_wrap_backward(dqmc_engine* h, int l) {
    ENGINE_CALL(h);
    if (l < 0 || l >= e.nt) { set_error("time slice out of range"); return DQMC_ERANGE; }
    return e.wrap_backward(l);
}
int dqmc_local_update_slice(dqmc_engine* h, int l, const int32_t* perm, const uint8_t* kprop, const double* u, int* accepted) {
    ENGINE_CALL(h);
    if (l < 0 || l >= e.nt) { set_error("time slice out of range"); return DQMC_ERANGE; }
    DQ_TRY(e.check_stream("local_update_slice", perm, kprop, u, e.C));
    DQ_HIP(hipStreamSynchronize(e.s));
    for (int c = 0; c < e.C; ++c) {
        const size_t off = ((size_t)c * e.nt + l) * e.n;
        DQ_HIP(hipMemcpy(e.rs_perm.get() + off, perm + (size_t)c * e.n, sizeof(int32_t) * e.n, hipMemcpyHostToDevice));
        DQ_HIP(hipMemcpy(e.rs_k.get() + off, kprop + (size_t)c * e.n, e.n, hipMemcpyHostToDevice));
        DQ_HIP(hipMemcpy(e.rs_u.get() + off, u + (size_t)c * e.n, sizeof(double) * e.n, hipMemcpyHostToDevice));
    }
    DQ_TRY(e.local_update(l));
    DQ_TRY(launch_fold_stats(e.dstats.get(), e.acc.get() + l, e.nt, 1, e.err.get(), e.n_stack, 0, e.n, e.nt, e.C, e.s));
    DQ_TRY(e.sync_and_check());
    if (accepted) for (int c = 0; c < e.C; ++c) DQ_HIP(hipMemcpy(accepted + c, e.acc.get() + (size_t)c * e.nt + l, sizeof(int), hipMemcpyDeviceToHost));
    return 0;
}
int dqmc_rng_fill_time(dqmc_engine* h, int launches, double* ms_per_launch) {
    ENGINE_CALL(h);
    if (launches < 1 || !ms_per_launch) { set_error("rng_fill_time: launches >= 1 and a result pointer"); return DQMC_EINVAL; }
    if (!e.rng_seeded) { set_error("rng_fill_time: the engine has no seed (dqmc_rng_seed)"); return DQMC_EINVAL; }
    hipEvent_t e0 = nullptr, e1 = nullptr;
    DQ_HIP(hipEventCreate(&e0));
    if (hipEventCreate(&e1) != hipSuccess) { (void)hipEventDestroy(e0); set_error("rng_fill_time: hipEventCreate failed"); return DQMC_ENODEVICE; }
    int rc = e.fill_stream(e.rng_counter);
    if (rc == 0 && hipEventRecord(e0, e.s) != hipSuccess) rc = DQMC_ENODEVICE;
    for (int k = 0; k < launches && rc == 0; ++k) rc = e.fill_stream(e.rng_counter);
    if (rc == 0 && hipEventRecord(e1, e.s) != hipSuccess) rc = DQMC_ENODEVICE;
    if (rc == 0) rc = e.sync_and_check();
    float ms = 0.f;
    if (rc == 0 && hipEventElapsedTime(&ms, e0, e1) != hipSuccess) rc = DQMC_ENODEVICE;
    (void)hipEventDestroy(e0); (void)hipEventDestroy(e1);
    if (rc == 0) *ms_per_launch = (double)ms / launches;
    return rc;
}
int dqmc_calculate_Bbar(dqmc_engine* h, int is, double* out) {
    ENGINE_CALL(h);
    if (is < 0 || is >= e.n_stack) { set_error("stack index out of range"); return DQMC_ERANGE; }
    Mat bb; DQ_TRY(e.Bbar(is, &bb)); DQ_HIP(hipStreamSynchronize(e.s));
    DQ_HIP(hipMemcpy(out, bb.p, sizeof(double) * e.C * e.nn, hipMemcpyDeviceToHost)); return 0;
}
int dqmc_global_action(dqmc_engine* h, double* S) {
    ENGINE_CALL(h); DQ_TRY(e.sync_and_check());
    std::vector<int8_t> tmp; std::vector<double> ld(e.C);
    DQ_TRY(e.download_fields(tmp));
    DQ_HIP(hipMemcpy(ld.data(), e.logdet.get(), sizeof(double) * e.C, hipMemcpyDeviceToHost));
    const double alpha = -1.0;
    const size_t per = (size_t)e.nt * e.n;
    for (int c = 0; c < e.C; ++c) {
        double lb = 0.0, lg = 0.0;
        for (size_t k = 0; k < per; ++k) {
            const int f = tmp[c * per + k];
            lb += alpha * e.g_host[c] * e.eta_host[f]; lg += std::log(e.gamma_host[f]);
        }
        S[c] = -2.0 * ld[c] - (lb + lg);
    }
    return 0;
}
int dqmc_sweep_unequal_time(dqmc_engine* h) {
    ENGINE_CALL(h);
    if (!e.stack_valid) { set_error("sweep_unequal_time: call dqmc_init first"); return DQMC_EINVAL; }
    return e.sweep_unequal();
}
int dqmc_get_G_tau(dqmc_engine* h, int which, int l, double* out) {
    ENGINE_CALL(h);
    if (which < 0 || which > 2 || l < 0 || l > e.nt) { set_error("get_G_tau: which in 0..2, l in 0..nt"); return DQMC_ERANGE; }
    if (!e.ut_valid) { set_error("get_G_tau: run dqmc_sweep_unequal_time first"); return DQMC_EINVAL; }
    DQ_TRY(e.sync_and_check());
    DQ_HIP(hipMemcpy(out, e.utm(which, l).p, sizeof(double) * e.C * e.nn, hipMemcpyDeviceToHost));
    return 0;
}
int dqmc_half_warp(dqmc_engine* h, const double* expK_half, const double* invexpK_half, int which, int l, double* out) {
    ENGINE_CALL(h);
    if (!out) { set_error("half_warp: out is NULL"); return DQMC_EINVAL; }
    if (which < -1 || which > 2 || (which >= 0 && (l < 0 || l > e.nt))) { set_error("half_warp: which in -1..2, l in 0..nt"); return DQMC_ERANGE; }
    if (which >= 0 && !e.ut_valid) { set_error("half_warp: run dqmc_sweep_unequal_time first"); return DQMC_EINVAL; }
    if ((expK_half == nullptr) != (invexpK_half == nullptr)) { set_error("half_warp: pass both half-step matrices or neither"); return DQMC_EINVAL; }
    if (expK_half) {
        if (!e.hw.out) { Engine::HalfWarp x; DQ_TRY(dev_alloc(x.expK, e.nn)); DQ_TRY(dev_alloc(x.invexpK, e.nn)); DQ_TRY(dev_alloc(x.out, (size_t)e.C * e.nn)); e.hw = std::move(x); }
        DQ_HIP(hipStreamSynchronize(e.s));
        DQ_HIP(hipMemcpy(e.hw.expK.get(), expK_half, sizeof(double) * e.nn, hipMemcpyHostToDevice));
        DQ_HIP(hipMemcpy(e.hw.invexpK.get(), invexpK_half, sizeof(double) * e.nn, hipMemcpyHostToDevice));
    } else if (!e.hw.out) { set_error("half_warp: no half-step matrices uploaded yet"); return DQMC_EINVAL; }
    const CMat M = which < 0 ? CMat(e.mG()) : CMat(e.utm(which, l));
    DQ_TRY(e.ctx.gemm(CMat(e.hw.invexpK.get(), 0), M, e.ctx.T(0)));
    DQ_TRY(e.ctx.gemm(e.ctx.T(0), CMat(e.hw.expK.get(), 0), Mat{e.hw.out.get(), e.nn}));
    DQ_TRY(e.sync_and_check());
    DQ_HIP(hipMemcpy(out, e.hw.out.get(), sizeof(double) * e.C * e.nn, hipMemcpyDeviceToHost));
    return 0;
}
int dqmc_measure_unequal_time(dqmc_engine* h, int L1, int L2, int accumulate, double* out) {
    ENGINE_CALL(h);
    if (L1 < 1 || L2 < 1 || L1 * L2 != e.n) { set_error("measure_unequal_time: L1*L2 must equal n_sites"); return DQMC_EINVAL; }
    if (!e.ut_valid) { set_error("measure_unequal_time: run dqmc_sweep_unequal_time first"); return DQMC_EINVAL; }
    const long stride = 3L * (e.nt + 1) * e.n;
    if (accumulate) {
        DQ_TRY(launch_measure_unequal_time(e.ut.G[0].get(), e.ut.G[1].get(), e.ut.G[2].get(), e.ut.meas_sum.get(), stride, L1, L2, e.nt, 1, e.C, e.s));
        ++e.ut_meas_count; return 0;
    }
    if (!out) { set_error("measure_unequal_time: out is NULL"); return DQMC_EINVAL; }
    DQ_TRY(launch_measure_unequal_time(e.ut.G[0].get(), e.ut.G[1].get(), e.ut.G[2].get(), e.ut.meas_now.get(), stride, L1, L2, e.nt, 0, e.C, e.s));
    DQ_TRY(e.sync_and_check());
    DQ_HIP(hipMemcpy(out, e.ut.meas_now.get(), sizeof(double) * e.C * stride, hipMemcpyDeviceToHost));
    return 0;
}
int dqmc_measure_unequal_fetch(dqmc_engine* h, double* out_sum, int64_t* n_measurements, int reset) {
    ENGINE_CALL(h); DQ_TRY(e.sync_and_check());
    if (!e.ut.meas_sum) { set_error("measure_unequal_fetch: nothing measured yet"); return DQMC_EINVAL; }
    const size_t cnt = (size_t)e.C * 3 * (e.nt + 1) * e.n;
    if (out_sum) DQ_HIP(hipMemcpy(out_sum, e.ut.meas_sum.get(), sizeof(double) * cnt, hipMemcpyDeviceToHost));
    if (n_measurements) *n_measurements = e.ut_meas_count;
    if (reset) { DQ_HIP(hipMemset(e.ut.meas_sum.get(), 0, sizeof(double) * cnt)); e.ut_meas_count = 0; }
    return 0;
}
int dqmc_measure_equal_time(dqmc_engine* h, int L1, int L2, double* scalars, double* chi_r) {
    ENGINE_CALL(h);
    if (L1 < 1 || L2 < 1 || L1 * L2 != e.n) { set_error("measure_equal_time: L1*L2 must equal n_sites"); return DQMC_EINVAL; }
    DQ_TRY(launch_measure_equal_time(CMat(e.G.get(), e.nn), e.meas_now.get(), 3 + e.n, L1, L2, 0, e.C, e.s));
    DQ_TRY(e.sync_and_check());
    return e.copy_out_equal_time(e.meas_now.get(), scalars, chi_r);
}
int dqmc_measure_accumulate(dqmc_engine* h, int L1, int L2) {
    ENGINE_CALL(h);
    if (L1 < 1 || L2 < 1 || L1 * L2 != e.n) { set_error("measure_accumulate: L1*L2 must equal n_sites"); return DQMC_EINVAL; }
    DQ_TRY(launch_measure_equal_time(CMat(e.G.get(), e.nn), e.meas_sum.get(), 3 + e.n, L1, L2, 1, e.C, e.s));
    ++e.meas_count;
    return 0;
}
int dqmc_measure_fetch(dqmc_engine* h, double* scalars_sum, double* chi_r_sum, int64_t* n_measurements, int reset) {
    ENGINE_CALL(h); DQ_TRY(e.sync_and_check());
    DQ_TRY(e.copy_out_equal_time(e.meas_sum.get(), scalars_sum, chi_r_sum));
    if (n_measurements) *n_measurements = e.meas_count;
    if (reset) { DQ_HIP(hipMemset(e.meas_sum.get(), 0, sizeof(double) * e.C * (3 + e.n))); e.meas_count = 0; }
    return 0;
}
int dqmc_update_kernel_time(dqmc_engine* h, double* ms, int64_t* n_launches, int64_t* n_accepted) {
    ENGINE_CALL(h); DQ_TRY(e.sync_and_check());
    std::vector<DevStats> st(e.C);
    DQ_HIP(hipMemcpy(st.data(), e.dstats.get(), sizeof(DevStats) * e.C, hipMemcpyDeviceToHost));
    long long acc = 0; for (auto& x : st) acc += x.n_accepted;
    if (ms) *ms = e.upd_ms; if (n_launches) *n_launches = e.upd_launches; if (n_accepted) *n_accepted = acc - e.upd_accept_base;
    e.upd_ms = 0.0; e.upd_launches = 0; e.upd_accept_base = acc;
    return 0;
}
int dqmc_debug_snapshot(dqmc_engine* h, double* wrap_err, int* accepted, unsigned int* sync_words, unsigned int* slice_epoch) {
    ENGINE_CALL(h);
    DQ_HIP(hipStreamSynchronize(e.s));
    if (wrap_err) DQ_HIP(hipMemcpy(wrap_err, e.err.get(), sizeof(double) * e.n_stack, hipMemcpyDeviceToHost));
    if (accepted) DQ_HIP(hipMemcpy(accepted, e.acc.get(), sizeof(int) * e.nt, hipMemcpyDeviceToHost));
    if (sync_words) DQ_HIP(hipMemcpy(sync_words, e.slice_sync.get(), sizeof(unsigned int) * 80, hipMemcpyDeviceToHost));
    if (slice_epoch) *slice_epoch = e.slice_epoch;
    return 0;
}
int dqmc_bbar_rider_launches(dqmc_engine* h, int64_t* n_launches) {
    ENGINE_CALL(h);
    if (n_launches) *n_launches = e.rider_launches;
    return 0;
}
int dqmc_debug_gt_check(dqmc_engine* h, int on, double* max_err, int64_t* n_checks) {
    ENGINE_CALL(h); DQ_TRY(e.sync_and_check());
    if (!e.gt_err) { DQ_TRY(dev_alloc(e.gt_err, e.C)); DQ_HIP(hipMemset(e.gt_err.get(), 0, sizeof(double) * e.C)); }
    if (max_err) DQ_HIP(hipMemcpy(max_err, e.gt_err.get(), sizeof(double) * e.C, hipMemcpyDeviceToHost));
    if (n_checks) *n_checks = e.gt_checks;
    DQ_HIP(hipMemset(e.gt_err.get(), 0, sizeof(double) * e.C));
    e.gt_checks = 0; e.gt_check = on != 0;
    return 0;
}
int dqmc_slice_path(dqmc_engine* h) {
    if (!h) return -1;
    Engine& e = h->e;
    if (!is_persistent(e.slice_path)) return 0;
    unsigned solo = 0;
    for (int c = 0; c < e.C && !solo; ++c) {
        SliceSync hs; if (hipMemcpy(&hs, e.slice_sync.get() + (size_t)c * SLICE_SYNC_BYTES, 64, hipMemcpyDeviceToHost) != hipSuccess) break;
        solo = hs.solo_count;
    }
    return solo ? 2 : 1;
}
int dqmc_set_profiling(dqmc_engine* h, int on) {
    ENGINE_CALL(h); DQ_TRY(e.sync_and_check());
    e.profiling = on != 0; return 0;
}

}
```

dqmc_amd/csrc/lu_gj.hip:

```cpp
#include "common.h"
#include "wave.h"
#include <cstdlib>
#include <utility>

namespace dq {

namespace {
constexpr int GJ_NB = 32;
using d4 = __attribute__((ext_vector_type(4))) double;

__device__ __forceinline__ void lds_wait() { asm volatile("s_waitcnt lgkmcnt(0)" ::: "memory"); }

template <int NR, int J>
__device__ __forceinline__ void gj_step(double (&a)[NR][GJ_NB], bool (&live)[NR], int (&mypos)[NR], int& myperm, bool& singular, int lane, int k0) {
    unsigned long long best = 0ULL; int bq = -1;
#pragma unroll
    for (int q = 0; q < NR; ++q) {
        const unsigned long long kq = live[q] ? ((unsigned long long)__double_as_longlong(fabs(a[q][J])) | 1ULL) : 0ULL;
        if (kq > best) { best = kq; bq = q; }
    }
    const unsigned hi = (unsigned)(best >> 32), lo = (unsigned)best;
    const unsigned m1 = wave_max_u32(hi);
    const unsigned m2 = wave_max_u32(hi == m1 ? lo : 0u);
    const unsigned long long winners = __ballot(hi == m1 && lo == m2 && bq >= 0);
    const int pl = winners ? (int)__builtin_ctzll(winners) : 0;
    const int pq = __builtin_amdgcn_readlane(bq, pl);
    if (lane == J) myperm = pl + 64 * pq;
    double prow[GJ_NB - J];
#pragma unroll
    for (int q = 0; q < NR; ++q) {
        if (q == pq) {
#pragma unroll
            for (int c = J; c < GJ_NB; ++c) prow[c - J] = readlane_f64(a[q][c], pl);
        }
    }
#pragma unroll
    for (int q = 0; q < NR; ++q)
        if (q == pq && lane == pl) { live[q] = false; mypos[q] = k0 + J; }
    const double piv = prow[0];
    singular = singular || !(fabs(piv) > 0.0);
    double r = __builtin_amdgcn_rcp(piv);
    r = fma(fma(-piv, r, 1.0), r, r);
    r = fma(fma(-piv, r, 1.0), r, r);
#pragma unroll
    for (int q = 0; q < NR; ++q) {
        if (live[q]) {
            const double l = a[q][J] * r;
            a[q][J] = l;
#pragma unroll
            for (int c = J + 1; c < GJ_NB; ++c) a[q][c] = fma(-l, prow[c - J], a[q][c]);
        }
    }
}
template <int NR, int J>
struct GjSteps {
    static __device__ __forceinline__ void run(double (&a)[NR][GJ_NB], bool (&live)[NR], int (&mypos)[NR], int& myperm, bool& singular, int lane, int nbw, int k0) {
        if (J < nbw) gj_step<NR, J>(a, live, mypos, myperm, singular, lane, k0);
        GjSteps<NR, J + 1>::run(a, live, mypos, myperm, singular, lane, nbw, k0);
    }
};
template <int NR>
struct GjSteps<NR, GJ_NB> {
    static __device__ __forceinline__ void run(double (&)[NR][GJ_NB], bool (&)[NR], int (&)[NR], int&, bool&, int, int, int) {}
};
}

template <int NR>
__global__ __launch_bounds__(64) void gj_panel_kernel(CMat Am, int* rowpos_p, long rowpos_stride, int* perm_p, long perm_stride, double* tinv_p,
                                                      double* logabsdet, int accumulate, int* info, int n, int k0) {
    __shared__ __attribute__((aligned(16))) double LU[GJ_NB][GJ_NB];
    const int chain = blockIdx.y;
    const double* __restrict__ A = Am.at(chain);
    int* rowpos = rowpos_p + (long)chain * rowpos_stride;
    int* perm = perm_p + (long)chain * perm_stride;
    double* tinv = tinv_p + (long)chain * 2 * GJ_NB * GJ_NB;
    const int lane = threadIdx.x;
    const int nbw = min(GJ_NB, n - k0);

    bool live[NR]; int mypos[NR];
    double a[NR][GJ_NB];
#pragma unroll
    for (int q = 0; q < NR; ++q) {
        const int r = lane + 64 * q;
        live[q] = r < n && (k0 == 0 ? true : rowpos[r] < 0);
        mypos[q] = -1;
#pragma unroll
        for (int c = 0; c < GJ_NB; ++c) a[q][c] = (live[q] && c < nbw) ? A[r + (long)n * (k0 + c)] : 0.0;
    }
    for (int e = lane; e < GJ_NB * GJ_NB; e += 64) (&LU[0][0])[e] = ((e >> 5) == (e & 31)) ? 1.0 : 0.0;
    int myperm = 0; bool singular = false;

    GjSteps<NR, 0>::run(a, live, mypos, myperm, singular, lane, nbw, k0);

    lds_wait();
#pragma unroll
    for (int q = 0; q < NR; ++q) {
        const int r = lane + 64 * q;
        if (r < n) { if (k0 == 0) rowpos[r] = mypos[q]; else if (mypos[q] >= 0) rowpos[r] = mypos[q]; }
        if (mypos[q] >= 0) {
            double* dst = &LU[mypos[q] - k0][0];
#pragma unroll
            for (int c = 0; c < GJ_NB; c += 2) *reinterpret_cast<double2*>(dst + c) = make_double2(a[q][c], a[q][c + 1]);
        }
    }
    if (lane < nbw) perm[k0 + lane] = myperm;
    lds_wait();
#pragma unroll
    for (int e = 0; e < GJ_NB * GJ_NB / 64; ++e) tinv[lane + 64 * e] = (&LU[0][0])[lane + 64 * e];
    {
        const double pv = lane < nbw ? fabs(LU[lane][lane]) : 1.0;
        const double ls = wave_sum(log(pv));
        if (lane == 0) {
            if (logabsdet) logabsdet[chain] = ((accumulate || k0 > 0) ? logabsdet[chain] : 0.0) + ls;
            if (info && (singular || !(ls == ls))) atomicOr(info, DQ_STATUS_PIVOT);
        }
    }
    {
        const int blk = lane >> 4, c = lane & 15;
        const bool up = blk >= 2;
        const int base = (blk & 1) * 16;
        const double* T0 = &LU[0][0] + (up ? (base + 15) * 33 : base * 33);
        const int sg = up ? -1 : 1;
        const int cc = up ? 15 - c : c;
        double x[16];
#pragma unroll
        for (int j = 0; j < 16; ++j) {
            double s0 = (j == cc) ? 1.0 : 0.0, s1 = 0.0;
#pragma unroll
            for (int m = 0; m < j; ++m) {
                const double t = T0[sg * (j * 32 + m)];
                if (m & 1) s1 = fma(-t, x[m], s1); else s0 = fma(-t, x[m], s0);
            }
            const double s = s0 + s1;
            x[j] = up ? s / T0[sg * (j * 33)] : s;
        }
        double* out = tinv + GJ_NB * GJ_NB + 256 * blk + 16 * c;
#pragma unroll
        for (int j = 0; j < 16; ++j) out[up ? 15 - j : j] = x[j];
    }
}

__device__ __forceinline__ void gj_panel_logdet(double (&LU)[GJ_NB][GJ_NB], double* logabsdet, int accumulate, int* info, int chain, int lane, int nbw, int k0, int s_sing) {
    const double pv = lane < nbw ? fabs(LU[lane][lane]) : 1.0;
    const double ls = wave_sum(log(pv));
    if (lane == 0) {
        if (logabsdet) logabsdet[chain] = ((accumulate || k0 > 0) ? logabsdet[chain] : 0.0) + ls;
        if (info && (s_sing || !(ls == ls))) atomicOr(info, DQ_STATUS_PIVOT);
    }
}
template <int... Js>
__device__ __forceinline__ void gj_tri_steps(double (&x)[16], const double* T0, int sg, int cc, bool up, bool hi, double rd, std::integer_sequence<int, Js...>) {
    auto step = [&](auto jc) {
        constexpr int j = decltype(jc)::value;
        double s0 = (j == cc) ? 1.0 : 0.0, s1 = 0.0;
#pragma unroll
        for (int m = 0; m < j; ++m) {
            const double tt = T0[sg * (j * 32 + m)];
            if (m & 1) s1 = fma(-tt, x[m], s1); else s0 = fma(-tt, x[m], s0);
        }
        const double s = s0 + s1;
        const double r0 = readlane_f64(rd, 15 - j), r1 = readlane_f64(rd, 31 - j);
        x[j] = up ? s * (hi ? r1 : r0) : s;
    };
    (step(std::integral_constant<int, Js>{}), ...);
}
__device__ __forceinline__ void gj_panel_tri_inverses(double (&LU)[GJ_NB][GJ_NB], double* inv, int lane) {
    const int blk = lane >> 4, c = lane & 15;
    const bool up = blk >= 2;
    const int base = (blk & 1) * 16;
    const double* T0 = &LU[0][0] + (up ? (base + 15) * 33 : base * 33);
    const int sg = up ? -1 : 1;
    const int cc = up ? 15 - c : c;
    const double rd = 1.0 / LU[lane & 31][lane & 31];
    double x[16];
    gj_tri_steps(x, T0, sg, cc, up, (blk & 1) != 0, rd, std::make_integer_sequence<int, 16>{});
    double* out = inv + 256 * blk + 16 * c;
#pragma unroll
    for (int j = 0; j < 16; ++j) out[up ? 15 - j : j] = x[j];
}

#ifdef DQ_GJ_STAMPS
#define GST(i) { unsigned long long t_; asm volatile("s_waitcnt lgkmcnt(0)\n\ts_memtime %0\n\ts_waitcnt lgkmcnt(0)" : "=s"(t_) :: "memory"); gst[i] += t_ - gprev; gprev = t_; }
#define GST_ARGS , unsigned long long (&gst)[8], unsigned long long& gprev
#define GST_PASS , gst, gprev
#else
#define GST(i)
#define GST_ARGS
#define GST_PASS
#endif
template <int J, int NW, int RPL>
__device__ __forceinline__ void gj_step_mw(double (&a)[RPL][GJ_NB], unsigned& live, int (&mypos)[RPL], int& myperm, bool& singular, int lane, int wave, int k0,
                                           double (*slot_row)[NW][GJ_NB + 2], unsigned long long (*slot_key)[(NW + 1) & ~1] GST_ARGS) {
    constexpr int PAR = J & 1;
    constexpr int C0 = J & ~1;
    GST(0)
    double aj = a[0][J]; int bs = 0;
    if (RPL > 1) asm volatile("" : "+v"(aj));
    unsigned long long key = (live & 1u) ? ((unsigned long long)__double_as_longlong(fabs(aj)) | 1ULL) : 0ULL;
#pragma unroll
    for (int q = 1; q < RPL; ++q) {
        double v = a[q][J];
        asm volatile("" : "+v"(v));
        const unsigned long long kq = ((live >> q) & 1u) ? ((unsigned long long)__double_as_longlong(fabs(v)) | 1ULL) : 0ULL;
        if (kq > key) { key = kq; aj = v; bs = q; }
    }
    double rme = __builtin_amdgcn_rcp(aj);
    rme = fma(fma(-aj, rme, 1.0), rme, rme);
    rme = fma(fma(-aj, rme, 1.0), rme, rme);
    const unsigned hi = (unsigned)(key >> 32), lo = (unsigned)key;
    const unsigned m1 = wave_max_u32(hi);
    const unsigned m2 = wave_max_u32(hi == m1 ? lo : 0u);
    const unsigned long long winners = __ballot(hi == m1 && lo == m2 && key != 0ULL);
    const int cl = winners ? (int)__builtin_ctzll(winners) : 0;
    GST(1)
    if (lane == cl) {
#pragma unroll
        for (int q = 0; q < RPL; ++q) {
            if (bs == q) {
#pragma unroll
                for (int c = C0; c < GJ_NB; c += 2) *reinterpret_cast<double2*>(&slot_row[PAR][wave][c]) = make_double2(a[q][c], a[q][c + 1]);
            }
        }
        slot_row[PAR][wave][GJ_NB] = rme;
        slot_key[PAR][wave] = winners ? ((((unsigned long long)m1 << 32) | m2) & ~0x1FFULL) | (unsigned long long)(cl | (bs << 6)) | 0x100ULL : 0ULL;
    }
    GST(2)
    asm volatile("s_waitcnt lgkmcnt(0)" ::: "memory");
    __builtin_amdgcn_s_barrier();
    asm volatile("" ::: "memory");
    GST(3)
    constexpr int NWK = (NW + 1) & ~1;
    ulonglong2 kp[NWK / 2];
#pragma unroll
    for (int q = 0; q < NWK / 2; ++q) kp[q] = *reinterpret_cast<const ulonglong2*>(&slot_key[PAR][2 * q]);
    unsigned long long best = kp[0].x; int pw = 0;
    if ((kp[0].y >> 9) > (best >> 9)) { best = kp[0].y; pw = 1; }
#pragma unroll
    for (int q = 1; q < NWK / 2; ++q) {
        if ((kp[q].x >> 9) > (best >> 9)) { best = kp[q].x; pw = 2 * q; }
        if ((kp[q].y >> 9) > (best >> 9)) { best = kp[q].y; pw = 2 * q + 1; }
    }
    const int pl = (int)(best & 0x3FULL), ps = (int)((best >> 6) & 3ULL);
    GST(4)
    double prow[GJ_NB - C0];
#pragma unroll
    for (int c = C0; c < GJ_NB; c += 2) { const double2 v = *reinterpret_cast<const double2*>(&slot_row[PAR][pw][c]); prow[c - C0] = v.x; prow[c + 1 - C0] = v.y; }
    const double r = slot_row[PAR][pw][GJ_NB];
    GST(5)
    if (lane == J && wave == 0) myperm = pl + 64 * pw + 64 * NW * ps;
    const bool mine = wave == pw && lane == pl;
    singular = singular || !(fabs(prow[J - C0]) > 0.0);
#pragma unroll
    for (int q = 0; q < RPL; ++q) {
        if (mine && ps == q) { live &= ~(1u << q); mypos[q] = k0 + J; }
        const bool lv = (live >> q) & 1u;
        const double l = lv ? a[q][J] * r : 0.0;
        a[q][J] = lv ? l : a[q][J];
#pragma unroll
        for (int c = J + 1; c < GJ_NB; ++c) a[q][c] = fma(-l, prow[c - C0], a[q][c]);
    }
    GST(6)
}
template <int J, int NW, int RPL>
struct GjStepsMW {
    static __device__ __forceinline__ void run(double (&a)[RPL][GJ_NB], unsigned& live, int (&mypos)[RPL], int& myperm, bool& singular, int lane, int wave, int nbw, int k0,
                                               double (*slot_row)[NW][GJ_NB + 2], unsigned long long (*slot_key)[(NW + 1) & ~1] GST_ARGS) {
        if (J < nbw) gj_step_mw<J, NW, RPL>(a, live, mypos, myperm, singular, lane, wave, k0, slot_row, slot_key GST_PASS);
        GjStepsMW<J + 1, NW, RPL>::run(a, live, mypos, myperm, singular, lane, wave, nbw, k0, slot_row, slot_key GST_PASS);
    }
};
template <int NW, int RPL>
struct GjStepsMW<GJ_NB, NW, RPL> {
    static __device__ __forceinline__ void run(double (&)[RPL][GJ_NB], unsigned&, int (&)[RPL], int&, bool&, int, int, int, int, double (*)[NW][GJ_NB + 2],
                                               unsigned long long (*)[(NW + 1) & ~1] GST_ARGS) {}
};
template <int NW, int RPL>
struct GjPanelShared {
    double LU[GJ_NB][GJ_NB];
    double slot_row[2][NW][GJ_NB + 2];
    unsigned long long slot_key[2][(NW + 1) & ~1];
    int s_sing;
};
template <int NW, int RPL, bool CLAMPED>
__device__ __forceinline__ void gj_panel_load(const double* __restrict__ A, const int* rowpos, int n, int k0, int nbw, int t, double (&a)[RPL][GJ_NB], unsigned& live,
                                              int (&oldpos)[RPL]) {
    live = 0u;
#pragma unroll
    for (int q = 0; q < RPL; ++q) {
        const int r = t + 64 * NW * q;
        const int rc = r < n ? r : 0;
        if (CLAMPED) {
            double v[GJ_NB];
#pragma unroll
            for (int c = 0; c < GJ_NB; ++c) v[c] = A[rc + (long)n * (k0 + (c < nbw ? c : 0))];
            oldpos[q] = k0 == 0 ? -1 : rowpos[rc];
            const bool lv = r < n && oldpos[q] < 0;
            live |= lv ? (1u << q) : 0u;
#pragma unroll
            for (int c = 0; c < GJ_NB; ++c) a[q][c] = (lv && c < nbw) ? v[c] : 0.0;
        } else {
            oldpos[q] = k0 == 0 ? -1 : rowpos[rc];
            const bool lv = r < n && oldpos[q] < 0;
            live |= lv ? (1u << q) : 0u;
#pragma unroll
            for (int c = 0; c < GJ_NB; ++c) a[q][c] = (lv && c < nbw) ? A[r + (long)n * (k0 + c)] : 0.0;
        }
    }
}
template <int NW, int RPL>
__device__ __forceinline__ void gj_panel_factor(GjPanelShared<NW, RPL>& sh, double (&a)[RPL][GJ_NB], unsigned& live, int (&mypos)[RPL], int& myperm, int t, int nbw, int k0
#ifdef DQ_GJ_STAMPS
                                                , unsigned long long& gstart, unsigned long long& gsteps_end
#endif
                                                ) {
    constexpr int NWK = (NW + 1) & ~1;
    static_assert(RPL <= 4, "two key bits name the slot");
    const int lane = t & 63, wave = t >> 6;
    bool singular = false;
    myperm = 0;
#pragma unroll
    for (int q = 0; q < RPL; ++q) mypos[q] = -1;
    for (int e = t; e < GJ_NB * GJ_NB; e += blockDim.x) (&sh.LU[0][0])[e] = ((e >> 5) == (e & 31)) ? 1.0 : 0.0;
    if (t == 0) sh.s_sing = 0;
    if (t < 2 * NWK) (&sh.slot_key[0][0])[t] = 0ULL;
    lds_wait();
    __builtin_amdgcn_s_barrier();
    asm volatile("" ::: "memory");

#ifdef DQ_GJ_STAMPS
    unsigned long long gst[8] = {0, 0, 0, 0, 0, 0, 0, 0}, gprev;
    asm volatile("s_waitcnt vmcnt(0)\n\ts_memtime %0\n\ts_waitcnt lgkmcnt(0)" : "=s"(gprev) :: "memory"); gstart = gprev;
#endif
    GjStepsMW<0, NW, RPL>::run(a, live, mypos, myperm, singular, lane, wave, nbw, k0, sh.slot_row, sh.slot_key GST_PASS);
#ifdef DQ_GJ_STAMPS
    gsteps_end = gprev;
    if (t == 0 && k0 == 0 && blockIdx.x == 0 && blockIdx.y == 0)
        printf("gj panel k0=0 grid.x=%d, %d waves x %d rows per lane, clocks over %d steps (each segment includes one stamp, ~130): (loop) %llu | search %llu | publish %llu | barrier %llu | keys %llu | row %llu | fma %llu | total %llu\n",
               (int)gridDim.x, (int)(blockDim.x >> 6), RPL, nbw, gst[0], gst[1], gst[2], gst[3], gst[4], gst[5], gst[6], gprev - gstart);
#endif

    lds_wait();
    __builtin_amdgcn_s_barrier();
    asm volatile("" ::: "memory");
#pragma unroll
    for (int q = 0; q < RPL; ++q) {
        if (mypos[q] >= 0) {
            double* dst = &sh.LU[mypos[q] - k0][0];
#pragma unroll
            for (int c = 0; c < GJ_NB; c += 2) *reinterpret_cast<double2*>(dst + c) = make_double2(a[q][c], a[q][c + 1]);
        }
    }
    if (singular && lane == 0) sh.s_sing = 1;
}
#ifdef DQ_GJ_STAMPS
#define GJ_STAMP_VM(x) asm volatile("s_waitcnt vmcnt(0)\n\ts_memtime %0\n\ts_waitcnt lgkmcnt(0)" : "=s"(x) :: "memory")
#endif

template <int NW, int RPL>
__global__ __launch_bounds__(64 * NW) void gj_panel_mw_kernel(CMat Am, int* rowpos_p, long rowpos_stride, int* perm_p, long perm_stride, double* tinv_p,
                                                          double* logabsdet, int accumulate, int* info, int n, int k0) {
    __shared__ __attribute__((aligned(16))) GjPanelShared<NW, RPL> sh;
    const int chain = blockIdx.y;
    const double* __restrict__ A = Am.at(chain);
    int* rowpos = rowpos_p + (long)chain * rowpos_stride;
    int* perm = perm_p + (long)chain * perm_stride;
    double* tinv = tinv_p + (long)chain * 2 * GJ_NB * GJ_NB;
    const int t = threadIdx.x, lane = t & 63, wave = t >> 6;
#ifdef DQ_GJ_STAMPS
    unsigned long long gentry, gstart, gprev;
    asm volatile("s_memtime %0\n\ts_waitcnt lgkmcnt(0)" : "=s"(gentry) :: "memory");
#endif
    const int nbw = min(GJ_NB, n - k0);
    unsigned live;
    int oldpos[RPL], mypos[RPL], myperm;
    double a[RPL][GJ_NB];
    gj_panel_load<NW, RPL, false>(A, rowpos, n, k0, nbw, t, a, live, oldpos);
#ifdef DQ_GJ_STAMPS
    gj_panel_factor<NW, RPL>(sh, a, live, mypos, myperm, t, nbw, k0, gstart, gprev);
#else
    gj_panel_factor<NW, RPL>(sh, a, live, mypos, myperm, t, nbw, k0);
#endif
#pragma unroll
    for (int q = 0; q < RPL; ++q) {
        const int r = t + 64 * NW * q;
        if (r < n) { if (k0 == 0) rowpos[r] = mypos[q]; else if (mypos[q] >= 0) rowpos[r] = mypos[q]; }
    }
    if (wave == 0 && lane < nbw) perm[k0 + lane] = myperm;
    __syncthreads();
    for (int e = t; e < GJ_NB * GJ_NB; e += blockDim.x) tinv[e] = (&sh.LU[0][0])[e];
#ifdef DQ_GJ_STAMPS
    unsigned long long gmid;
    GJ_STAMP_VM(gmid);
#endif
    if (wave == 0) gj_panel_tri_inverses(sh.LU, tinv + GJ_NB * GJ_NB, lane);
    else if (wave == 1) gj_panel_logdet(sh.LU, logabsdet, accumulate, info, chain, lane, nbw, k0, sh.s_sing);
#ifdef DQ_GJ_STAMPS
    unsigned long long gend;
    GJ_STAMP_VM(gend);
    if (t == 0 && k0 == 0 && blockIdx.y == 0) printf("   prologue %llu | steps %llu | LU hand-over (+ printf) %llu | epilogue %llu\n", gstart - gentry, gprev - gstart, gmid - gprev, gend - gmid);
#endif
}

__global__ __launch_bounds__(256) void gj_update_kernel(Mat Am, Mat Bm, Mat SAm, Mat Xm, const int* rowpos_p, long rowpos_stride,
                                                        const int* perm_p, long perm_stride, const double* tinv_p, int n, int k0, int nA, int nS, int nCA) {
    const int chain = blockIdx.y;
    double* __restrict__ A = Am.at(chain);
    double* __restrict__ B = Bm.at(chain);
    double* __restrict__ SA = SAm.at(chain);
    double* __restrict__ X = Xm.at(chain);
    const int* rowpos = rowpos_p + (long)chain * rowpos_stride;
    const int* perm = perm_p + (long)chain * perm_stride;
    const double* __restrict__ LUg = tinv_p + (long)chain * 2 * GJ_NB * GJ_NB;
    const double* __restrict__ Tinv = LUg + GJ_NB * GJ_NB;
    const int nbw = min(GJ_NB, n - k0);
    const int row_tiles = nA + nS + 1;
    const int rt = blockIdx.x % row_tiles, ct = blockIdx.x / row_tiles;
    const int lane = threadIdx.x & 63, wave = threadIdx.x >> 6;
    const int r16 = lane & 15, kk = lane >> 4;
    const int wr = wave & 1, wc = wave >> 1;
    const bool colA = ct < nCA;
    const int col = (colA ? k0 + nbw + 32 * ct : 32 * (ct - nCA)) + 16 * wc + r16;
    const bool col_ok = col < n;
    const long coff = (long)n * (col_ok ? col : n - 1);
    const double* __restrict__ src12 = colA ? A : B;
    double* __restrict__ dstS = colA ? SA : X;

    double a12[2][4];
#pragma unroll
    for (int h = 0; h < 2; ++h)
#pragma unroll
        for (int s = 0; s < 4; ++s) {
            const int k = 16 * h + 4 * s + kk;
            const int pr = perm[k0 + (k < nbw ? k : 0)];
            const double v = src12[pr + coff];
            a12[h][s] = (k < nbw && col_ok) ? v : 0.0;
        }
    const bool writer = rt == nA + nS;
    const bool rowS = rt >= nA;
    const int row0 = (rowS ? 32 * (rt - nA) : 32 * rt) + 16 * wr;
    const int rowlim = rowS ? k0 : n;
    const double* __restrict__ msrc = rowS ? SA : A;
    double* __restrict__ dst = rowS ? dstS : (colA ? A : B);
    double mult[2][4];
    double cold[4];
    bool st_ok[4];
    if (!writer) {
        const int mrow = min(row0 + r16, rowlim - 1);
#pragma unroll
        for (int h = 0; h < 2; ++h)
#pragma unroll
            for (int s = 0; s < 4; ++s) {
                const int k = 16 * h + kk + 4 * s;
                const double v = msrc[mrow + (long)n * (k0 + (k < nbw ? k : 0))];
                mult[h][s] = k < nbw ? v : 0.0;
            }
#pragma unroll
        for (int reg = 0; reg < 4; ++reg) {
            const int r = row0 + kk + 4 * reg;
            const int rc = min(r, rowlim - 1);
            st_ok[reg] = col_ok && r < rowlim && (rowS || rowpos[rc] < 0);
            cold[reg] = dst[rc + coff];
        }
    }
    double lai[4], lbi[4], uai[4], ubi[4], cl[4], cu[4];
#pragma unroll
    for (int s = 0; s < 4; ++s) {
        const int k = 4 * s + kk;
        lai[s] = Tinv[0 * 256 + r16 + 16 * k]; lbi[s] = Tinv[1 * 256 + r16 + 16 * k];
        uai[s] = Tinv[2 * 256 + r16 + 16 * k]; ubi[s] = Tinv[3 * 256 + r16 + 16 * k];
        cl[s] = -LUg[(16 + r16) * 32 + k];
        cu[s] = -LUg[r16 * 32 + 16 + k];
    }
    const d4 zero4 = {0.0, 0.0, 0.0, 0.0};
    d4 t1[2], u[2];
    t1[0] = zero4;
#pragma unroll
    for (int s = 0; s < 4; ++s) t1[0] = __builtin_amdgcn_mfma_f64_16x16x4f64(lai[s], a12[0][s], t1[0], 0, 0, 0);
    d4 w = {a12[1][0], a12[1][1], a12[1][2], a12[1][3]};
#pragma unroll
    for (int s = 0; s < 4; ++s) w = __builtin_amdgcn_mfma_f64_16x16x4f64(cl[s], t1[0][s], w, 0, 0, 0);
    t1[1] = zero4;
#pragma unroll
    for (int s = 0; s < 4; ++s) t1[1] = __builtin_amdgcn_mfma_f64_16x16x4f64(lbi[s], w[s], t1[1], 0, 0, 0);
    u[1] = zero4;
#pragma unroll
    for (int s = 0; s < 4; ++s) u[1] = __builtin_amdgcn_mfma_f64_16x16x4f64(ubi[s], t1[1][s], u[1], 0, 0, 0);
    w = t1[0];
#pragma unroll
    for (int s = 0; s < 4; ++s) w = __builtin_amdgcn_mfma_f64_16x16x4f64(cu[s], u[1][s], w, 0, 0, 0);
    u[0] = zero4;
#pragma unroll
    for (int s = 0; s < 4; ++s) u[0] = __builtin_amdgcn_mfma_f64_16x16x4f64(uai[s], w[s], u[0], 0, 0, 0);
    if (writer) {
#pragma unroll
        for (int reg = 0; reg < 4; ++reg) {
            const int i = 16 * wr + kk + 4 * reg;
            if (i < nbw && col_ok) dstS[k0 + i + coff] = u[wr][reg];
        }
        return;
    }
    d4 acc = {0.0, 0.0, 0.0, 0.0};
#pragma unroll
    for (int h = 0; h < 2; ++h)
#pragma unroll
        for (int s = 0; s < 4; ++s) acc = __builtin_amdgcn_mfma_f64_16x16x4f64(mult[h][s], u[h][s], acc, 0, 0, 0);
#pragma unroll
    for (int reg = 0; reg < 4; ++reg)
        if (st_ok[reg]) dst[row0 + kk + 4 * reg + coff] = cold[reg] - acc[reg];
}

template <int NW, int RPL>
__global__ __launch_bounds__(64 * NW) void gj_step_kernel(Mat Am, Mat Bm, Mat SAm, Mat Xm, const int* rowpos_old_p, int* rowpos_new_p, long rowpos_stride,
                                                          double* logabsdet, int accumulate, int* info, int n, int k0, int nA, int nS, int nCA) {
    static_assert(NW == 4, "the update's 2 x 2 waves are the panel's");
    __shared__ __attribute__((aligned(16))) GjPanelShared<NW, RPL> sh;
    __shared__ __attribute__((aligned(16))) double s_inv[4 * 256];
    __shared__ int s_rowpos[64 * NW * RPL];
    __shared__ int s_perm[GJ_NB];
    const int chain = blockIdx.y;
    double* __restrict__ A = Am.at(chain);
    double* __restrict__ B = Bm.at(chain);
    double* __restrict__ SA = SAm.at(chain);
    double* __restrict__ X = Xm.at(chain);
    const int* rowpos_old = rowpos_old_p + (long)chain * rowpos_stride;
    int* rowpos_new = rowpos_new_p + (long)chain * rowpos_stride;
    const int t = threadIdx.x, lane = t & 63, wave = t >> 6;
#ifdef DQ_GJ_STAMPS
    unsigned long long gentry, gstart, gprev;
    asm volatile("s_memtime %0\n\ts_waitcnt lgkmcnt(0)" : "=s"(gentry) :: "memory");
#endif
    const int nbw = min(GJ_NB, n - k0);

    unsigned live;
    int oldpos[RPL], mypos[RPL], myperm;
    double a[RPL][GJ_NB];
    gj_panel_load<NW, RPL, true>(A, rowpos_old, n, k0, nbw, t, a, live, oldpos);

    const int row_tiles = nA + nS + 1;
    const int rt = blockIdx.x % row_tiles, ct = blockIdx.x / row_tiles;
    const int r16 = lane & 15, kk = lane >> 4;
    const int wr = wave & 1, wc = wave >> 1;
    const bool colA = ct < nCA;
    const int col = (colA ? k0 + nbw + 32 * ct : 32 * (ct - nCA)) + 16 * wc + r16;
    const bool col_ok = col < n;
    const long coff = (long)n * (col_ok ? col : n - 1);
    const double* __restrict__ src12 = colA ? A : B;
    double* __restrict__ dstS = colA ? SA : X;
    const bool writer = rt == nA + nS;
    const bool rowS = rt >= nA;
    const int row0 = (rowS ? 32 * (rt - nA) : 32 * rt) + 16 * wr;
    const int rowlim = rowS ? k0 : n;
    const double* __restrict__ msrc = rowS ? SA : A;
    double* __restrict__ dst = rowS ? dstS : (colA ? A : B);
    double mult[2][4];
    double cold[4];
    {
        const int mrow = max(min(row0 + r16, rowlim - 1), 0);
#pragma unroll
        for (int h = 0; h < 2; ++h)
#pragma unroll
            for (int s = 0; s < 4; ++s) {
                const int k = 16 * h + kk + 4 * s;
                const double v = msrc[mrow + (long)n * (k0 + (k < nbw ? k : 0))];
                mult[h][s] = k < nbw ? v : 0.0;
            }
#pragma unroll
        for (int reg = 0; reg < 4; ++reg) cold[reg] = dst[max(min(row0 + kk + 4 * reg, rowlim - 1), 0) + coff];
    }

#ifdef DQ_GJ_STAMPS
    gj_panel_factor<NW, RPL>(sh, a, live, mypos, myperm, t, nbw, k0, gstart, gprev);
#else
    gj_panel_factor<NW, RPL>(sh, a, live, mypos, myperm, t, nbw, k0);
#endif
#pragma unroll
    for (int q = 0; q < RPL; ++q) {
        const int r = t + 64 * NW * q;
        const int np = mypos[q] >= 0 ? mypos[q] : oldpos[q];
        s_rowpos[r] = np;
        if (blockIdx.x == 0 && r < n) rowpos_new[r] = np;
    }
    if (wave == 0 && lane < GJ_NB) s_perm[lane] = lane < nbw ? myperm : 0;
    __syncthreads();
#ifdef DQ_GJ_STAMPS
    unsigned long long gmid, ginv, ggather;
    GJ_STAMP_VM(gmid);
#endif

    double a12[2][4];
#pragma unroll
    for (int h = 0; h < 2; ++h)
#pragma unroll
        for (int s = 0; s < 4; ++s) {
            const int k = 16 * h + 4 * s + kk;
            const double v = src12[s_perm[k < nbw ? k : 0] + coff];
            a12[h][s] = (k < nbw && col_ok) ? v : 0.0;
        }
    bool st_ok[4];
#pragma unroll
    for (int reg = 0; reg < 4; ++reg) {
        const int r = row0 + kk + 4 * reg;
        st_ok[reg] = !writer && col_ok && r < rowlim && (rowS || s_rowpos[max(min(r, rowlim - 1), 0)] < 0);
    }
    if (wave == 0) gj_panel_tri_inverses(sh.LU, s_inv, lane);
    else if (wave == 1 && blockIdx.x == 0) gj_panel_logdet(sh.LU, logabsdet, accumulate, info, chain, lane, nbw, k0, sh.s_sing);
#ifdef DQ_GJ_STAMPS
    asm volatile("s_waitcnt lgkmcnt(0)\n\ts_memtime %0\n\ts_waitcnt lgkmcnt(0)" : "=s"(ginv) :: "memory");
#endif
    __syncthreads();
#ifdef DQ_GJ_STAMPS
    GJ_STAMP_VM(ggather);
#endif

    const double* LUs = &sh.LU[0][0];
    double lai[4], lbi[4], uai[4], ubi[4], cl[4], cu[4];
#pragma unroll
    for (int s = 0; s < 4; ++s) {
        const int k = 4 * s + kk;
        lai[s] = s_inv[0 * 256 + r16 + 16 * k]; lbi[s] = s_inv[1 * 256 + r16 + 16 * k];
        uai[s] = s_inv[2 * 256 + r16 + 16 * k]; ubi[s] = s_inv[3 * 256 + r16 + 16 * k];
        cl[s] = -LUs[(16 + r16) * 32 + k];
        cu[s] = -LUs[r16 * 32 + 16 + k];
    }
    const d4 zero4 = {0.0, 0.0, 0.0, 0.0};
    d4 t1[2], u[2];
    t1[0] = zero4;
#pragma unroll
    for (int s = 0; s < 4; ++s) t1[0] = __builtin_amdgcn_mfma_f64_16x16x4f64(lai[s], a12[0][s], t1[0], 0, 0, 0);
    d4 w = {a12[1][0], a12[1][1], a12[1][2], a12[1][3]};
#pragma unroll
    for (int s = 0; s < 4; ++s) w = __builtin_amdgcn_mfma_f64_16x16x4f64(cl[s], t1[0][s], w, 0, 0, 0);
    t1[1] = zero4;
#pragma unroll
    for (int s = 0; s < 4; ++s) t1[1] = __builtin_amdgcn_mfma_f64_16x16x4f64(lbi[s], w[s], t1[1], 0, 0, 0);
    u[1] = zero4;
#pragma unroll
    for (int s = 0; s < 4; ++s) u[1] = __builtin_amdgcn_mfma_f64_16x16x4f64(ubi[s], t1[1][s], u[1], 0, 0, 0);
    w = t1[0];
#pragma unroll
    for (int s = 0; s < 4; ++s) w = __builtin_amdgcn_mfma_f64_16x16x4f64(cu[s], u[1][s], w, 0, 0, 0);
    u[0] = zero4;
#pragma unroll
    for (int s = 0; s < 4; ++s) u[0] = __builtin_amdgcn_mfma_f64_16x16x4f64(uai[s], w[s], u[0], 0, 0, 0);
    if (writer) {
#pragma unroll
        for (int reg = 0; reg < 4; ++reg) {
            const int i = 16 * wr + kk + 4 * reg;
            if (i < nbw && col_ok) dstS[k0 + i + coff] = u[wr][reg];
        }
    } else {
        d4 acc = {0.0, 0.0, 0.0, 0.0};
#pragma unroll
        for (int h = 0; h < 2; ++h)
#pragma unroll
            for (int s = 0; s < 4; ++s) acc = __builtin_amdgcn_mfma_f64_16x16x4f64(mult[h][s], u[h][s], acc, 0, 0, 0);
#pragma unroll
        for (int reg = 0; reg < 4; ++reg)
            if (st_ok[reg]) dst[row0 + kk + 4 * reg + coff] = cold[reg] - acc[reg];
    }
#ifdef DQ_GJ_STAMPS
    unsigned long long gend;
    GJ_STAMP_VM(gend);
    if (t == 0 && k0 == 0 && blockIdx.x == 0 && blockIdx.y == 0)
        printf("   fused step: prologue %llu | chain %llu | deposit (+ printf) %llu | inverses (wave 0) %llu | gather wait %llu | update %llu\n", gstart - gentry, gprev - gstart,
               gmid - gprev, ginv - gmid, ggather - ginv, gend - ggather);
#endif
}
bool gj_fused_fits(int n) { return n > 64 && n <= 256; }
bool gj_fused_default(int n) { return n > 128 && n <= 256; }

int launch_gj_solve(Mat A, Mat B, Mat X, Mat SA, double* tinv, int* perm, long perm_stride, int* rowpos, int* rowpos_alt, long rowpos_stride,
                    double* logabsdet, int accumulate_logdet, int* info, int n, int n_chains, bool fused, hipStream_t s) {
    if (n > 1024) { set_error("gj_solve supports n <= 1024"); return -1; }
    if (fused && rowpos_alt && gj_fused_fits(n)) {
        int p = 0;
        for (int k0 = 0; k0 < n; k0 += GJ_NB, ++p) {
            const int nbw = n - k0 < GJ_NB ? n - k0 : GJ_NB;
            const int nA = (n + 31) / 32, nS = k0 / 32;
            const int nCA = (n - k0 - nbw + 31) / 32, nCB = (n + 31) / 32;
            hipLaunchKernelGGL((gj_step_kernel<4, 1>), dim3((nA + nS + 1) * (nCA + nCB), n_chains), dim3(256), 0, s, A, B, SA, X, (const int*)((p & 1) ? rowpos_alt : rowpos),
                               (p & 1) ? rowpos : rowpos_alt, rowpos_stride, logabsdet, accumulate_logdet, info, n, k0, nA, nS, nCA);
        }
        DQ_HIP(hipGetLastError());
        return 0;
    }
    for (int k0 = 0; k0 < n; k0 += GJ_NB) {
        const dim3 pg(1, n_chains);
#define DQ_GJ_PANEL(NW, RPL) hipLaunchKernelGGL((gj_panel_mw_kernel<NW, RPL>), pg, dim3(RPL == 1 ? 64 * ((n + 63) / 64) : 64 * NW), 0, s, CMat(A), rowpos, rowpos_stride, perm, perm_stride, tinv, logabsdet, accumulate_logdet, info, n, k0)
        if (n > 768) DQ_GJ_PANEL(8, 2);
        else if (n > 576) DQ_GJ_PANEL(4, 3);
        else if (n > 512) DQ_GJ_PANEL(3, 3);
        else if (n > 256) DQ_GJ_PANEL(4, 2);
        else if (n > 64) DQ_GJ_PANEL(4, 1);
        else hipLaunchKernelGGL((gj_panel_kernel<1>), pg, dim3(64), 0, s, CMat(A), rowpos, rowpos_stride, perm, perm_stride, tinv, logabsdet, accumulate_logdet, info, n, k0);
        const int nbw = n - k0 < GJ_NB ? n - k0 : GJ_NB;
        const int nA = (n + 31) / 32, nS = k0 / 32;
        const int nCA = (n - k0 - nbw + 31) / 32, nCB = (n + 31) / 32;
        hipLaunchKernelGGL(gj_update_kernel, dim3((nA + nS + 1) * (nCA + nCB), n_chains), dim3(256), 0, s, A, B, SA, X, (const int*)rowpos, rowpos_stride,
                           (const int*)perm, perm_stride, (const double*)tinv, n, k0, nA, nS, nCA);
    }
#undef DQ_GJ_PANEL
    DQ_HIP(hipGetLastError());
    return 0;
}

}
```

dqmc_amd/csrc/qr_panel.hip:

```cpp
#include "common.h"
#include "wave.h"
#include <utility>

namespace dq {

namespace {

#ifdef DQ_QP_STAMPS
#define QST(i) { unsigned long long t_; asm volatile("s_memtime %0\n\ts_waitcnt lgkmcnt(0)" : "=s"(t_) :: "memory"); if (threadIdx.x == 0) qst[i] = t_; }
#else
#define QST(i)
#endif

constexpr int QP_B = 16;
constexpr int QP_SR = 32;
#ifndef QP_SEL_ROWS
#define QP_SEL_ROWS 32
#endif
constexpr int QP_SEL = QP_SEL_ROWS;
typedef double d4 __attribute__((ext_vector_type(4)));

__device__ __forceinline__ unsigned qp_row_bits(unsigned r) {
    unsigned h = r * 0x9E3779B1u + 0x85EBCA77u;
    h ^= h >> 16; h *= 0x85EBCA6Bu; h ^= h >> 13; h *= 0xC2B2AE35u; h ^= h >> 16;
    return h;
}
__device__ __forceinline__ double qp_sign(unsigned bits, int i) {
    return __hiloint2double((int)(0x3FF00000u | (((bits >> i) & 1u) << 31)), 0);
}

__device__ __forceinline__ double rows4_sum(double x) {
    const unsigned lo = (unsigned)__double_as_longlong(x), hi = (unsigned)(__double_as_longlong(x) >> 32);
    auto l16 = __builtin_amdgcn_permlane16_swap(lo, lo, false, false);
    auto h16 = __builtin_amdgcn_permlane16_swap(hi, hi, false, false);
    const double e = __hiloint2double((int)h16[0], (int)l16[0]), o = __hiloint2double((int)h16[1], (int)l16[1]);
    const double s = e + o;
    const unsigned slo = (unsigned)__double_as_longlong(s), shi = (unsigned)(__double_as_longlong(s) >> 32);
    auto l32 = __builtin_amdgcn_permlane32_swap(slo, slo, false, false);
    auto h32 = __builtin_amdgcn_permlane32_swap(shi, shi, false, false);
    return __hiloint2double((int)h32[0], (int)l32[0]) + __hiloint2double((int)h32[1], (int)l32[1]);
}

template <int J>
__device__ __forceinline__ void dpp_fmac_self(double& d, double a) {
    asm volatile("v_fmac_f64_dpp %0, %1, %1 row_newbcast:%2 row_mask:0xf bank_mask:0xf" : "+v"(d) : "v"(a), "n"(J));
}
template <int J>
__device__ __forceinline__ void dpp_axpy_self(double& a, double m) {
    asm volatile("v_fmac_f64_dpp %0, %0, %1 row_newbcast:%2 row_mask:0xf bank_mask:0xf" : "+v"(a) : "v"(m), "n"(J));
}
__device__ __forceinline__ void dpp_fence(double (&a)[16]) {
    asm volatile("s_nop 1" : "+v"(a[0]), "+v"(a[1]), "+v"(a[2]), "+v"(a[3]), "+v"(a[4]), "+v"(a[5]), "+v"(a[6]), "+v"(a[7]),
                             "+v"(a[8]), "+v"(a[9]), "+v"(a[10]), "+v"(a[11]), "+v"(a[12]), "+v"(a[13]), "+v"(a[14]), "+v"(a[15]));
}

__device__ __forceinline__ void dpp_fence1(double& z) { asm volatile("s_nop 1" : "+v"(z)); }
template <int T>
__device__ __forceinline__ void dpp_fmac(double& d, double z, double y) {
    asm volatile("v_fmac_f64_dpp %0, %1, %2 row_newbcast:%3 row_mask:0xf bank_mask:0xf" : "+v"(d) : "v"(z), "v"(y), "n"(T));
}
template <int... Ts>
__device__ __forceinline__ void t_row_dot(double& tj, const double (&trow)[16], double z, std::integer_sequence<int, Ts...>) {
    (dpp_fmac<Ts>(tj, z, trow[Ts]), ...);
}

template <int NW>
struct PanelShared {
    static constexpr int NWP = NW < 2 ? 2 : NW;
    alignas(16) unsigned long long key[2][NWP];
    alignas(16) double cand[2][QP_SEL + 2];
    alignas(16) double part[2][QP_B][NWP];
    alignas(16) double prow[2][QP_B];
    int sel[QP_B];
};

template <int NEWTON>
__device__ __forceinline__ void householder(double alpha, double tail2, double& beta, double& tau, double& scale) {
    const double s = fma(alpha, alpha, tail2);
    double r = __builtin_amdgcn_rsq(s);
    const double h = 0.5 * s;
#pragma unroll
    for (int it = 0; it < NEWTON; ++it) r = r * fma(-h * r, r, 1.5);
    double sq = s * r;
    if (NEWTON > 1) sq = fma(0.5 * r, fma(-sq, sq, s), sq);
    const double b = -copysign(sq, alpha);
    const double d = alpha - b;
    double id = __builtin_amdgcn_rcp(d);
#pragma unroll
    for (int it = 0; it < NEWTON; ++it) id = id * fma(-d, id, 2.0);
    const bool none = tail2 == 0.0;
    beta = none ? alpha : b;
    tau = none ? 0.0 : d * copysign(r, alpha);
    scale = none ? 0.0 : id;
}

__device__ __forceinline__ void lds_barrier() {
    asm volatile("s_waitcnt lgkmcnt(0)" ::: "memory");
    __builtin_amdgcn_s_barrier();
    asm volatile("" ::: "memory");
}

template <int J, int NW, int CPL>
__device__ __forceinline__ void select_step(double (&y)[CPL][QP_SEL], unsigned& live, int t, int lane, int wave, PanelShared<NW>& sh) {
    constexpr int par = J & 1;
    unsigned long long key = 0ULL; int bq = 0; double btail = 0.0;
#pragma unroll
    for (int q = 0; q < CPL; ++q) {
        double tl[4] = {0.0, 0.0, 0.0, 0.0};
#pragma unroll
        for (int i = J + 1; i < QP_SEL; ++i) tl[i & 3] = fma(y[q][i], y[q][i], tl[i & 3]);
        const double tail = (tl[0] + tl[1]) + (tl[2] + tl[3]);
        const double nrm2 = fma(y[q][J], y[q][J], tail);
        const unsigned long long kq = ((live >> q) & 1u) ? (((unsigned long long)__double_as_longlong(nrm2) & ~0x7FFULL) | (unsigned long long)(1024 - (t + 64 * NW * q))) : 0ULL;
        if (kq > key) { key = kq; bq = q; btail = tail; }
    }
    const unsigned long long wmax = wave_max_u64(key);
    const bool cand_ = wmax != 0ULL && key == wmax;
    if (cand_) sh.key[par][wave] = wmax;
    if (wmax == 0ULL && lane == 0) sh.key[par][wave] = 0ULL;
    lds_barrier();
    unsigned long long best = sh.key[par][0]; int ww = 0;
#pragma unroll
    for (int q = 1; q < NW; ++q) { const unsigned long long o = sh.key[par][q]; if (o > best) { best = o; ww = q; } }
    if (cand_ && wave == ww) {
#pragma unroll
        for (int q = 0; q < CPL; ++q) {
            if (bq == q) {
#pragma unroll
                for (int i = J & ~1; i < QP_SEL; i += 2) *reinterpret_cast<double2*>(&sh.cand[par][i]) = double2{y[q][i], y[q][i + 1]};
            }
        }
        sh.cand[par][QP_SEL] = btail;
    }
    lds_barrier();
    const int pcol = 1024 - (int)(best & 0x7FFULL);
    const double* xs = sh.cand[par];
    double x[QP_SEL];
#pragma unroll
    for (int i = J & ~1; i < QP_SEL; i += 2) { const double2 v = *reinterpret_cast<const double2*>(&xs[i]); x[i] = v.x; x[i + 1] = v.y; }
    double beta, tau, scale;
    householder<1>(x[J], xs[QP_SEL], beta, tau, scale);
    const double st = -scale * tau;
#pragma unroll
    for (int q = 0; q < CPL; ++q) {
        double dt[4] = {0.0, 0.0, 0.0, 0.0};
#pragma unroll
        for (int i = J + 1; i < QP_SEL; ++i) dt[i & 3] = fma(x[i], y[q][i], dt[i & 3]);
        const double dot = (dt[0] + dt[1]) + (dt[2] + dt[3]);
        const double cf = st * fma(scale, dot, y[q][J]);
#pragma unroll
        for (int i = J + 1; i < QP_SEL; ++i) y[q][i] = fma(x[i], cf, y[q][i]);
        if (t + 64 * NW * q == pcol) live &= ~(1u << q);
    }
    if (lane == 0 && wave == 0) sh.sel[J] = pcol;
}

template <int J, int NW, int CPL>
__device__ __forceinline__ void panel_step(double (&a)[CPL][16], double (&trow)[QP_B], double& myscale, unsigned diag, unsigned blk_live, int c, int g, int wave,
                                           PanelShared<NW>& sh, double* tau_out) {
    constexpr int par = J & 1;
    if (blk_live) {
        double acc = 0.0;
#pragma unroll
        for (int b = 0; b < CPL; ++b) {
            if ((blk_live >> b) & 1u) {
                double dlo0 = 0.0, dlo1 = 0.0, dhi0 = 0.0, dhi1 = 0.0;
#pragma unroll
                for (int i = 0; i < 16; ++i) {
                    if (i <= J) { if (i & 1) dpp_fmac_self<J>(dlo1, a[b][i]); else dpp_fmac_self<J>(dlo0, a[b][i]); }
                    else { if (i & 1) dpp_fmac_self<J>(dhi1, a[b][i]); else dpp_fmac_self<J>(dhi0, a[b][i]); }
                }
                acc += (dhi0 + dhi1) + (((diag >> b) & 1u) ? 0.0 : dlo0 + dlo1);
                if ((diag >> b) & 1u) sh.prow[par][c] = a[b][J];
            }
        }
        const double part = rows4_sum(acc);
        if (g == 0) sh.part[par][c][wave] = part;
    } else if (g == 0) sh.part[par][c][wave] = 0.0;
    lds_barrier();
    double s_c = sh.part[par][c][0], s_j = sh.part[par][J][0];
#pragma unroll
    for (int q = 1; q < NW; ++q) { s_c += sh.part[par][c][q]; s_j += sh.part[par][J][q]; }
    const double alpha = sh.prow[par][J], apc = sh.prow[par][c];
    double beta, tau, scale;
    householder<2>(alpha, s_j, beta, tau, scale);
    const double zc = fma(scale, s_c, apc);
    if (c == J) myscale = scale;
    if (blk_live) {
        const double mcf = c > J ? -scale * tau * zc : 0.0;
#pragma unroll
        for (int b = 0; b < CPL; ++b) {
            if ((blk_live >> b) & 1u) {
                const bool isd = (diag >> b) & 1u;
                const double mlo = isd ? 0.0 : mcf;
#pragma unroll
                for (int i = 0; i < 16; ++i) {
                    if (i <= J) dpp_axpy_self<J>(a[b][i], mlo);
                    else dpp_axpy_self<J>(a[b][i], mcf);
                }
                const double newd = c > J ? fma(-tau, zc, a[b][J]) : beta;
                a[b][J] = (isd && c >= J) ? newd : a[b][J];
                dpp_fence(a[b]);
            }
        }
    }
    if (wave == 0) {
        double zt = myscale * zc;
        double tj = 0.0;
        dpp_fence1(zt);
        t_row_dot(tj, trow, zt, std::make_integer_sequence<int, J>{});
        trow[J] = c < J ? -tau * tj : (c == J ? tau : 0.0);
        if (g == 0 && c == J) tau_out[J] = tau;
    }
}

}

__host__ __device__ __forceinline__ long qp_off_qacc(int n) { return 2L * QP_SR * n; }
__host__ __device__ __forceinline__ long qp_off_ticket(int n) { return qp_off_qacc(n) + (long)n * n; }
__host__ __device__ __forceinline__ long qp_off_vp(int n) { return qp_off_ticket(n) + 2; }
__host__ __device__ __forceinline__ long qp_off_tm(int n) { return qp_off_vp(n) + (long)n * n; }
__host__ __device__ __forceinline__ long qp_off_vtp(int n) { return qp_off_tm(n) + (long)QP_B * n; }

#ifdef DQ_QP_STAMPS
#define QP_QST_PARAM , unsigned long long* qst
#define QP_QST_ARG , qst
#else
#define QP_QST_PARAM
#define QP_QST_ARG
#endif

template <int NW, int CPL, class Pre, class Mid>
__device__ __forceinline__ bool qp_factor_panel(const double* A, const double* __restrict__ Y, const int* pivpos, int n, int k, PanelShared<NW>& sh,
                                                double* tau_out, double (&a)[CPL][16], double (&trow)[QP_B], double& myscale, unsigned& diag, int& mycol,
                                                Pre&& pre, Mid&& mid QP_QST_PARAM) {
    const int t = threadIdx.x, lane = t & 63, wave = t >> 6;
    QST(0)
    {
        unsigned live = 0u;
        double y[CPL][QP_SEL]; int pp[CPL];
#pragma unroll
        for (int q = 0; q < CPL; ++q) {
            const int col = t + 64 * NW * q, cc = col < n ? col : n - 1;
#pragma unroll
            for (int i = 0; i < QP_SEL; ++i) y[q][i] = Y[(long)i * n + cc];
            pp[q] = pivpos[cc];
        }
        if (pre()) return false;
#pragma unroll
        for (int q = 0; q < CPL; ++q) {
            const int col = t + 64 * NW * q;
            if (col < n && pp[q] < 0) live |= 1u << q;
            if (col >= n) {
#pragma unroll
                for (int i = 0; i < QP_SEL; ++i) y[q][i] = 0.0;
            }
        }
        if (y[0][0] == 1.2345e300) live = 0u;
        QST(1)
#define QP_SEL_STEP(J) select_step<J, NW, CPL>(y, live, t, lane, wave, sh); QST(2 + J)
        QP_SEL_STEP(0) QP_SEL_STEP(1) QP_SEL_STEP(2) QP_SEL_STEP(3) QP_SEL_STEP(4) QP_SEL_STEP(5) QP_SEL_STEP(6) QP_SEL_STEP(7)
        QP_SEL_STEP(8) QP_SEL_STEP(9) QP_SEL_STEP(10) QP_SEL_STEP(11) QP_SEL_STEP(12) QP_SEL_STEP(13) QP_SEL_STEP(14) QP_SEL_STEP(15)
#undef QP_SEL_STEP
    }
    lds_barrier();
    const int c = lane & 15, g = lane >> 4;
    mycol = sh.sel[c];
    myscale = 0.0; diag = 0u;
    unsigned blk_live = 0u;
#pragma unroll
    for (int b = 0; b < CPL; ++b) {
        const int r0 = 64 * NW * b + 64 * wave + 16 * g;
        if (r0 == k) diag |= 1u << b;
        if (64 * NW * b + 64 * wave + 64 > k && 64 * NW * b + 64 * wave < n) blk_live |= 1u << b;
        const double2* src = reinterpret_cast<const double2*>(A + (long)n * mycol + r0);
        const bool rows_live = r0 >= k && r0 < n;
#pragma unroll
        for (int i = 0; i < 16; i += 2) { const double2 v = rows_live ? src[i >> 1] : double2{0.0, 0.0}; a[b][i] = v.x; a[b][i + 1] = v.y; }
        dpp_fence(a[b]);
    }
    asm volatile("s_waitcnt vmcnt(0)" ::: "memory");
#pragma unroll
    for (int i = 0; i < QP_B; ++i) trow[i] = 0.0;
#ifdef DQ_QP_STAMPS
    if (a[0][0] == 1.2345e300) myscale = 1.0;
#endif
    QST(18)
#define QP_PAN(J) panel_step<J, NW, CPL>(a, trow, myscale, diag, blk_live, c, g, wave, sh, tau_out); QST(19 + J)
    QP_PAN(0)
    mid();
    QP_PAN(1) QP_PAN(2) QP_PAN(3) QP_PAN(4) QP_PAN(5) QP_PAN(6) QP_PAN(7)
    QP_PAN(8) QP_PAN(9) QP_PAN(10) QP_PAN(11) QP_PAN(12) QP_PAN(13) QP_PAN(14) QP_PAN(15)
#undef QP_PAN
    return true;
}

template <int NW, int CPL>
__global__ __launch_bounds__(64 * NW) void qp_panel_kernel(Mat Am, QrWork w, int n, int k) {
    __shared__ PanelShared<NW> sh;
    const int chain = blockIdx.y;
    double* __restrict__ A = Am.at(chain);
    double* __restrict__ pw = w.pw + (long)chain * w.pw_stride;
    const double* __restrict__ Y = pw;
    double* __restrict__ Vp = pw + qp_off_vp(n) + (long)n * k;
    double* __restrict__ Tm = pw + qp_off_tm(n) + (long)QP_B * k;
    double* __restrict__ VTp = pw + qp_off_vtp(n) + (long)n * k;
    int* __restrict__ pivpos = w.pivpos + (long)chain * w.pivpos_stride;
    double* tau = w.tau + (long)chain * w.tau_stride;
    int* jpvt = w.jpvt + (long)chain * w.jpvt_stride;
    const int t = threadIdx.x, lane = t & 63, wave = t >> 6;
    const int c = lane & 15, g = lane >> 4;

#ifdef DQ_QP_STAMPS
    __shared__ unsigned long long qst[40];
#endif
    double a[CPL][16], trow[QP_B], myscale;
    unsigned diag; int mycol;
    qp_factor_panel<NW, CPL>(A, Y, pivpos, n, k, sh, tau + k, a, trow, myscale, diag, mycol, [] { return false; }, [] {} QP_QST_ARG);
#pragma unroll
    for (int b = 0; b < CPL; ++b) {
        const int r0 = 64 * NW * b + 64 * wave + 16 * g;
        if (r0 >= k && r0 < n) {
            const bool isd = (diag >> b) & 1u;
            double2* dst = reinterpret_cast<double2*>(A + (long)n * mycol + r0);
            double2* vdst = reinterpret_cast<double2*>(Vp + (long)n * c + r0);
            double v[16], vc[16];
#pragma unroll
            for (int i = 0; i < 16; ++i) {
                const bool below = !isd || i > c;
                v[i] = below ? a[b][i] * myscale : a[b][i];
                vc[i] = below ? v[i] : (i == c ? 1.0 : 0.0);
                VTp[(long)QP_B * (r0 + i) + c] = vc[i];
            }
#pragma unroll
            for (int i = 0; i < 16; i += 2) { dst[i >> 1] = double2{v[i], v[i + 1]}; vdst[i >> 1] = double2{vc[i], vc[i + 1]}; }
        }
    }
    if (wave == 0 && g == 0) {
#pragma unroll
        for (int i = 0; i < QP_B; ++i) Tm[c + QP_B * i] = trow[i];
        jpvt[k + c] = mycol;
        pivpos[mycol] = k + c;
    }
#ifdef DQ_QP_STAMPS
    asm volatile("s_waitcnt vmcnt(0)" ::: "memory");
    QST(35)
    __syncthreads();
    if (t == 0 && k == 0 && blockIdx.y == 0) {
        printf("panel k=0 n=%d (100 MHz ticks x 24 = clk @2.4GHz): load Y %llu | sel steps", n, qst[1] - qst[0]);
        for (int j = 0; j < 16; ++j) printf(" %llu", qst[2 + j] - qst[1 + j]);
        printf(" | gather %llu | panel steps", qst[18] - qst[17]);
        for (int j = 0; j < 16; ++j) printf(" %llu", qst[19 + j] - qst[18 + j]);
        printf(" | write-out %llu | total %llu\n", qst[35] - qst[34], qst[35] - qst[0]);
    }
#endif
}

constexpr int QP_UW = 8;
constexpr int QP_YT = QP_SR / 16;

template <int TPW>
__device__ __forceinline__ void qp_q_role(double (&red)[QP_UW][QP_YT * 4][64], double* __restrict__ Qacc, double* __restrict__ L,
                                          const double* __restrict__ Vp, const double* __restrict__ VTp, const double* __restrict__ Tm,
                                          int n, int k, int cb) {
    const int t = threadIdx.x, lane = t & 63, wave = t >> 6;
    const int r16 = lane & 15, kk = lane >> 4;
    const int col = 16 * cb + r16;
    double* __restrict__ Qc = Qacc + (long)n * col;
    const int m_tiles = (n - k) / 16;
    d4 Qt[TPW]; double v1[TPW][4], v2[TPW][4], tv[4];
#pragma unroll
    for (int ti = 0; ti < TPW; ++ti) {
        const int rt = wave + QP_UW * ti;
        Qt[ti] = d4{0.0, 0.0, 0.0, 0.0};
#pragma unroll
        for (int s = 0; s < 4; ++s) { v1[ti][s] = 0.0; v2[ti][s] = 0.0; }
        if (rt < m_tiles) {
            const int r0 = k + 16 * rt;
#pragma unroll
            for (int r = 0; r < 4; ++r) Qt[ti][r] = Qc[r0 + kk + 4 * r];
#pragma unroll
            for (int s = 0; s < 4; ++s) { v1[ti][s] = VTp[(long)QP_B * (r0 + kk + 4 * s) + r16]; v2[ti][s] = Vp[(long)n * (kk + 4 * s) + (r0 + r16)]; }
        }
    }
#pragma unroll
    for (int s = 0; s < 4; ++s) tv[s] = Tm[(kk + 4 * s) + QP_B * r16];
    const bool first = k == 0;
#pragma unroll
    for (int ti = 0; ti < TPW; ++ti)
#pragma unroll
        for (int r = 0; r < 4; ++r) Qt[ti][r] = first ? ((16 * (wave + QP_UW * ti) + kk + 4 * r == col) ? 1.0 : 0.0) : Qt[ti][r];
    d4 acc = {0.0, 0.0, 0.0, 0.0};
#pragma unroll
    for (int ti = 0; ti < TPW; ++ti) {
#pragma unroll
        for (int s = 0; s < 4; ++s) acc = __builtin_amdgcn_mfma_f64_16x16x4f64(v1[ti][s], Qt[ti][s], acc, 0, 0, 0);
    }
#pragma unroll
    for (int r = 0; r < 4; ++r) red[wave][r][lane] = acc[r];
    __syncthreads();
    d4 W;
#pragma unroll
    for (int r = 0; r < 4; ++r) {
        double v = red[0][r][lane];
#pragma unroll
        for (int q = 1; q < QP_UW; ++q) v += red[q][r][lane];
        W[r] = v;
    }
    d4 wp = {0.0, 0.0, 0.0, 0.0};
#pragma unroll
    for (int s = 0; s < 4; ++s) wp = __builtin_amdgcn_mfma_f64_16x16x4f64(tv[s], W[s], wp, 0, 0, 0);
    wp = -wp;
#pragma unroll
    for (int ti = 0; ti < TPW; ++ti) {
        const int rt = wave + QP_UW * ti;
        if (rt < m_tiles) {
            const int r0 = k + 16 * rt;
#pragma unroll
            for (int s = 0; s < 4; ++s) Qt[ti] = __builtin_amdgcn_mfma_f64_16x16x4f64(v2[ti][s], wp[s], Qt[ti], 0, 0, 0);
            if (rt == 0) {
#pragma unroll
                for (int r = 0; r < 4; ++r) L[(long)n * (k + kk + 4 * r) + col] = Qt[ti][r];
            } else {
#pragma unroll
                for (int r = 0; r < 4; ++r) Qc[r0 + kk + 4 * r] = Qt[ti][r];
            }
        }
    }
}

template <bool UPDATE, int TPW>
__global__ __launch_bounds__(64 * QP_UW) void qp_update_kernel(Mat Am, QrWork w, int n, int k, Mat Lm, int q_first) {
    constexpr int YT = QP_YT;
    __shared__ double red[QP_UW][YT * 4][64];
    const int chain = blockIdx.y;
    double* __restrict__ pw = w.pw + (long)chain * w.pw_stride;
    if (UPDATE && (int)blockIdx.x >= q_first) {
        qp_q_role<TPW>(red, pw + qp_off_qacc(n), Lm.at(chain), pw + qp_off_vp(n) + (long)n * k, pw + qp_off_vtp(n) + (long)n * k,
                       pw + qp_off_tm(n) + (long)QP_B * k, n, k, (int)blockIdx.x - q_first);
        return;
    }
    double* __restrict__ A = Am.at(chain);
    double* __restrict__ Y = pw;
    const double* __restrict__ Vp = pw + qp_off_vp(n) + (long)n * k;
    const double* __restrict__ Tm = pw + qp_off_tm(n) + (long)QP_B * k;
    const double* __restrict__ VTp = pw + qp_off_vtp(n) + (long)n * k;
    int* __restrict__ pivpos = w.pivpos + (long)chain * w.pivpos_stride;
    const int t = threadIdx.x, lane = t & 63, wave = t >> 6;
    const int r16 = lane & 15, kk = lane >> 4;
    const int col = 16 * blockIdx.x + r16;
    double* __restrict__ Ac = A + (long)n * col;
    const int m_tiles = (n - k) / 16;
    int pp = -1;
    if (UPDATE) pp = pivpos[col];
    d4 At[TPW]; double v1[TPW][4], v2[TPW][4], tv[4];
#pragma unroll
    for (int ti = 0; ti < TPW; ++ti) {
        const int rt = wave + QP_UW * ti;
        At[ti] = d4{0.0, 0.0, 0.0, 0.0};
#pragma unroll
        for (int s = 0; s < 4; ++s) { v1[ti][s] = 0.0; v2[ti][s] = 0.0; }
        if (rt < m_tiles) {
            const int r0 = k + 16 * rt;
#pragma unroll
            for (int r = 0; r < 4; ++r) At[ti][r] = Ac[r0 + kk + 4 * r];
            if (UPDATE) {
#pragma unroll
                for (int s = 0; s < 4; ++s) { v1[ti][s] = VTp[(long)QP_B * (r0 + kk + 4 * s) + r16]; v2[ti][s] = Vp[(long)n * (kk + 4 * s) + (r0 + r16)]; }
            }
        }
    }
    if (UPDATE) {
#pragma unroll
        for (int s = 0; s < 4; ++s) tv[s] = Tm[(kk + 4 * s) + QP_B * r16];
    }
    const bool live_col = pp < 0;
    if (UPDATE) { if (__ballot(live_col) == 0ULL) return; }
    else if (t < 16) pivpos[col] = -1;
    d4 wp = {0.0, 0.0, 0.0, 0.0};
    if (UPDATE) {
        d4 acc = {0.0, 0.0, 0.0, 0.0};
#pragma unroll
        for (int ti = 0; ti < TPW; ++ti) {
#pragma unroll
            for (int s = 0; s < 4; ++s) acc = __builtin_amdgcn_mfma_f64_16x16x4f64(v1[ti][s], At[ti][s], acc, 0, 0, 0);
        }
#pragma unroll
        for (int r = 0; r < 4; ++r) red[wave][r][lane] = acc[r];
        __syncthreads();
        d4 W;
#pragma unroll
        for (int r = 0; r < 4; ++r) {
            double v = red[0][r][lane];
#pragma unroll
            for (int q = 1; q < QP_UW; ++q) v += red[q][r][lane];
            W[r] = live_col ? v : 0.0;
        }
#pragma unroll
        for (int s = 0; s < 4; ++s) wp = __builtin_amdgcn_mfma_f64_16x16x4f64(tv[s], W[s], wp, 0, 0, 0);
        wp = -wp;
        __syncthreads();
    }
    d4 ya[YT];
#pragma unroll
    for (int yt = 0; yt < YT; ++yt) ya[yt] = d4{0.0, 0.0, 0.0, 0.0};
#pragma unroll
    for (int ti = 0; ti < TPW; ++ti) {
        const int rt = wave + QP_UW * ti;
        if (rt < m_tiles) {
            const int r0 = k + 16 * rt;
            if (UPDATE) {
#pragma unroll
                for (int s = 0; s < 4; ++s) At[ti] = __builtin_amdgcn_mfma_f64_16x16x4f64(v2[ti][s], wp[s], At[ti], 0, 0, 0);
                if (live_col) {
#pragma unroll
                    for (int r = 0; r < 4; ++r) Ac[r0 + kk + 4 * r] = At[ti][r];
                }
            }
            if (!UPDATE || rt >= 1) {
#pragma unroll
                for (int s = 0; s < 4; ++s) {
                    const unsigned bits = qp_row_bits((unsigned)(r0 + kk + 4 * s));
#pragma unroll
                    for (int yt = 0; yt < YT; ++yt) ya[yt] = __builtin_amdgcn_mfma_f64_16x16x4f64(qp_sign(bits, 16 * yt + r16), At[ti][s], ya[yt], 0, 0, 0);
                }
            }
        }
    }
#pragma unroll
    for (int yt = 0; yt < YT; ++yt)
#pragma unroll
        for (int r = 0; r < 4; ++r) red[wave][4 * yt + r][lane] = ya[yt][r];
    __syncthreads();
    for (int idx = t; idx < YT * 4 * 64; idx += 64 * QP_UW) {
        const int l = idx & 63, q = idx >> 6, yt = q >> 2, r = q & 3;
        double v = red[0][q][l];
#pragma unroll
        for (int qq = 1; qq < QP_UW; ++qq) v += red[qq][q][l];
        Y[(long)(16 * yt + (l >> 4) + 4 * r) * n + 16 * blockIdx.x + (l & 15)] = v;
    }
}

template <int NW, int CPL, int TPW>
__global__ __launch_bounds__(64 * NW) void qp_step_kernel(Mat Am, QrWork w, int n, int k, Mat Lm, int q_first) {
    constexpr int YT = QP_YT;
    constexpr int NV = (QP_UW + NW - 1) / NW;
    constexpr int LDV = 64 * NW * CPL + 1;
    __shared__ PanelShared<NW> sh;
    __shared__ double Vs[QP_B * LDV];
    __shared__ double Ts[QP_B * (QP_B + 1)];
    __shared__ double red[QP_UW][YT * 4][64];
    __shared__ double s_tau[QP_B];
    __shared__ unsigned s_ticket;
#ifdef DQ_QP_STAMPS
    __shared__ unsigned long long qst[40];
#endif
    const int chain = blockIdx.y;
    double* pw = w.pw + (long)chain * w.pw_stride;
    const bool qrole = (int)blockIdx.x >= q_first;
    const int cb = qrole ? (int)blockIdx.x - q_first : (int)blockIdx.x;
    double* A = Am.at(chain);
    const int par = (k / QP_B) & 1;
    const double* __restrict__ Yr = pw + (long)par * QP_SR * n;
    double* __restrict__ Yw = pw + (long)(par ^ 1) * QP_SR * n;
    unsigned* counter = reinterpret_cast<unsigned*>(pw + qp_off_ticket(n));
    int* pivpos = w.pivpos + (long)chain * w.pivpos_stride;
    const int t = threadIdx.x, lane = t & 63, wave = t >> 6;
    const int r16 = lane & 15, kk = lane >> 4;
    const int col = 16 * cb + r16;
    double* Xc = (qrole ? pw + qp_off_qacc(n) : A) + (long)n * col;
    const int m_tiles = (n - k) / 16;
    const int pp_ld = pivpos[col];
    d4 X[NV][TPW];
#pragma unroll
    for (int vi = 0; vi < NV; ++vi) {
#pragma unroll
        for (int ti = 0; ti < TPW; ++ti) {
            const int vw = wave + NW * vi, rt = vw + QP_UW * ti;
            X[vi][ti] = d4{0.0, 0.0, 0.0, 0.0};
            if (vw < QP_UW && rt < m_tiles) {
#pragma unroll
                for (int r = 0; r < 4; ++r) X[vi][ti][r] = Xc[k + 16 * rt + kk + 4 * r];
            }
        }
    }
    const int pp = qrole ? -1 : pp_ld;
    const unsigned last_ticket = gridDim.x - 1;
    bool have_ticket = false;
    unsigned ticket = 0u;
    double a[CPL][16], trow[QP_B], myscale;
    unsigned diag; int mycol;
    const bool factored = qp_factor_panel<NW, CPL>(A, Yr, pivpos, n, k, sh, s_tau, a, trow, myscale, diag, mycol, [&] {
        if (__ballot(pp < 0) != 0ULL) return false;
        if (t == 0) s_ticket = __hip_atomic_fetch_add(counter, 1u, __ATOMIC_RELAXED, __HIP_MEMORY_SCOPE_AGENT);
        __syncthreads();
        have_ticket = true;
        return s_ticket != last_ticket;
    }, [&] {
        if (!have_ticket && t == 0) {
            long off = 0;
            asm volatile("" : "+v"(off));
            ticket = __hip_atomic_fetch_add(counter + off, 1u, __ATOMIC_RELAXED, __HIP_MEMORY_SCOPE_AGENT);
        }
    } QP_QST_ARG);
    if (!factored) return;
    const int c = lane & 15, g = lane >> 4;
#pragma unroll
    for (int b = 0; b < CPL; ++b) {
        const int r0 = 64 * NW * b + 64 * wave + 16 * g;
        if (r0 >= k && r0 < n) {
            const bool isd = (diag >> b) & 1u;
#pragma unroll
            for (int i = 0; i < 16; ++i) {
                const bool below = !isd || i > c;
                Vs[c * LDV + r0 + i] = below ? a[b][i] * myscale : (i == c ? 1.0 : 0.0);
            }
        }
    }
    if (wave == 0 && g == 0) {
#pragma unroll
        for (int i = 0; i < QP_B; ++i) Ts[c + (QP_B + 1) * i] = trow[i];
    }
    if (!have_ticket && t == 0) s_ticket = ticket;
    __syncthreads();
    QST(35)
    if (s_ticket == last_ticket) {
        double* tau = w.tau + (long)chain * w.tau_stride;
        int* jpvt = w.jpvt + (long)chain * w.jpvt_stride;
#pragma unroll
        for (int b = 0; b < CPL; ++b) {
            if ((diag >> b) & 1u) {
#pragma unroll
                for (int i = 0; i < 16; ++i) if (i <= c) A[(long)n * mycol + k + i] = a[b][i];
            }
        }
        if (wave == 0 && g == 0) { jpvt[k + c] = mycol; pivpos[mycol] = k + c; tau[k + c] = s_tau[c]; }
        if (t == 0) *counter = 0u;
        if (have_ticket) return;
    }
    QST(36)
    bool sel_hit = false;
#pragma unroll
    for (int j = 0; j < QP_B; ++j) sel_hit |= sh.sel[j] == col;
    const bool live_col = qrole || (pp < 0 && !sel_hit);
    double tv[4];
#pragma unroll
    for (int s = 0; s < 4; ++s) tv[s] = Ts[(kk + 4 * s) + (QP_B + 1) * r16];
    const bool first = qrole && k == 0;
#pragma unroll
    for (int vi = 0; vi < NV; ++vi)
#pragma unroll
        for (int ti = 0; ti < TPW; ++ti)
#pragma unroll
            for (int r = 0; r < 4; ++r) X[vi][ti][r] = first ? ((16 * (wave + NW * vi + QP_UW * ti) + kk + 4 * r == col) ? 1.0 : 0.0) : X[vi][ti][r];
#pragma unroll
    for (int vi = 0; vi < NV; ++vi) {
        const int vw = wave + NW * vi;
        if (vw < QP_UW) {
            d4 acc = {0.0, 0.0, 0.0, 0.0};
#pragma unroll
            for (int ti = 0; ti < TPW; ++ti) {
                const int rt = vw + QP_UW * ti;
                if (rt < m_tiles) {
                    const double* vrow = Vs + r16 * LDV + (k + 16 * rt + kk);
#pragma unroll
                    for (int s = 0; s < 4; ++s) acc = __builtin_amdgcn_mfma_f64_16x16x4f64(vrow[4 * s], X[vi][ti][s], acc, 0, 0, 0);
                }
            }
#pragma unroll
            for (int r = 0; r < 4; ++r) red[vw][r][lane] = acc[r];
        }
    }
    __syncthreads();
    d4 W;
#pragma unroll
    for (int r = 0; r < 4; ++r) {
        double v = red[0][r][lane];
#pragma unroll
        for (int q = 1; q < QP_UW; ++q) v += red[q][r][lane];
        W[r] = live_col ? v : 0.0;
    }
    d4 wp = {0.0, 0.0, 0.0, 0.0};
#pragma unroll
    for (int s = 0; s < 4; ++s) wp = __builtin_amdgcn_mfma_f64_16x16x4f64(tv[s], W[s], wp, 0, 0, 0);
    wp = -wp;
    __syncthreads();
    QST(37)
    double* L = Lm.at(chain);
#pragma unroll
    for (int vi = 0; vi < NV; ++vi) {
        const int vw = wave + NW * vi;
        if (vw < QP_UW) {
            d4 ya[YT];
#pragma unroll
            for (int yt = 0; yt < YT; ++yt) ya[yt] = d4{0.0, 0.0, 0.0, 0.0};
#pragma unroll
            for (int ti = 0; ti < TPW; ++ti) {
                const int rt = vw + QP_UW * ti;
                if (rt < m_tiles) {
                    const int r0 = k + 16 * rt;
#pragma unroll
                    for (int s = 0; s < 4; ++s) X[vi][ti] = __builtin_amdgcn_mfma_f64_16x16x4f64(Vs[(kk + 4 * s) * LDV + r0 + r16], wp[s], X[vi][ti], 0, 0, 0);
                    if (qrole) {
                        if (rt == 0) {
#pragma unroll
                            for (int r = 0; r < 4; ++r) L[(long)n * (k + kk + 4 * r) + col] = X[vi][ti][r];
                        } else {
#pragma unroll
                            for (int r = 0; r < 4; ++r) Xc[r0 + kk + 4 * r] = X[vi][ti][r];
                        }
                    } else {
                        if (live_col) {
#pragma unroll
                            for (int r = 0; r < 4; ++r) Xc[r0 + kk + 4 * r] = X[vi][ti][r];
                        }
                        if (rt >= 1) {
#pragma unroll
                            for (int s = 0; s < 4; ++s) {
                                const unsigned bits = qp_row_bits((unsigned)(r0 + kk + 4 * s));
#pragma unroll
                                for (int yt = 0; yt < YT; ++yt) ya[yt] = __builtin_amdgcn_mfma_f64_16x16x4f64(qp_sign(bits, 16 * yt + r16), X[vi][ti][s], ya[yt], 0, 0, 0);
                            }
                        }
                    }
                }
            }
            if (!qrole) {
#pragma unroll
                for (int yt = 0; yt < YT; ++yt)
#pragma unroll
                    for (int r = 0; r < 4; ++r) red[vw][4 * yt + r][lane] = ya[yt][r];
            }
        }
    }
    if (qrole) return;
    __syncthreads();
    for (int idx = t; idx < YT * 4 * 64; idx += 64 * NW) {
        const int l = idx & 63, q = idx >> 6, yt = q >> 2, r = q & 3;
        double v = red[0][q][l];
#pragma unroll
        for (int qq = 1; qq < QP_UW; ++qq) v += red[qq][q][l];
        Yw[(long)(16 * yt + (l >> 4) + 4 * r) * n + 16 * cb + (l & 15)] = v;
    }
#ifdef DQ_QP_STAMPS
    asm volatile("s_waitcnt vmcnt(0)" ::: "memory");
    QST(38)
    __syncthreads();
    if (t == 0 && (k == 0 || k == n / 2) && blockIdx.x == 0 && blockIdx.y == 0) {
        printf("step k=%d n=%d (100 MHz ticks): loads %llu | sel steps", k, n, qst[1] - qst[0]);
        for (int j = 0; j < 16; ++j) printf(" %llu", qst[2 + j] - qst[1 + j]);
        printf(" | gather %llu | panel steps", qst[18] - qst[17]);
        for (int j = 0; j < 16; ++j) printf(" %llu", qst[19 + j] - qst[18 + j]);
        printf(" | deposit + ticket %llu | last arriver %llu | W %llu | update + sketch %llu | total %llu\n", qst[35] - qst[34], qst[36] - qst[35],
               qst[37] - qst[36], qst[38] - qst[37], qst[38] - qst[0]);
    }
#endif
}

bool qr_panel_fused_fits(int n) { return n <= 576; }
bool qr_panel_fused_default(int n) { return n <= 512; }
long qr_panel_work_doubles(int n, bool two_launch) { return two_launch ? qp_off_vtp(n) + (long)n * n : qp_off_vp(n); }
static bool qr_panel_ok(int n, const QrWork& w, bool two_launch) {
    return n >= 16 && n <= 1024 && n % 16 == 0 && w.pw != nullptr && w.pivpos != nullptr && w.pw_stride >= qr_panel_work_doubles(n, two_launch);
}

int launch_qr_panel(Mat A, Mat L, QrWork w, int n, int n_chains, hipStream_t s) {
    const bool fused = !w.pw_two_launch && qr_panel_fused_fits(n);
    if (!qr_panel_ok(n, w, !fused)) { set_error("panel QR: n must be a multiple of 16 in [16, 1024] and the workspace present"); return -1; }
    const int nb = n / 16;
    const int tpw = (nb + QP_UW - 1) / QP_UW;
#define QP_UPD(U, K, GRID, QFIRST) do { const dim3 ugrid(GRID, n_chains); \
                          if (tpw <= 2) hipLaunchKernelGGL((qp_update_kernel<U, 2>), ugrid, dim3(64 * QP_UW), 0, s, A, w, n, K, L, QFIRST); \
                          else if (tpw <= 5) hipLaunchKernelGGL((qp_update_kernel<U, 5>), ugrid, dim3(64 * QP_UW), 0, s, A, w, n, K, L, QFIRST); \
                          else hipLaunchKernelGGL((qp_update_kernel<U, 8>), ugrid, dim3(64 * QP_UW), 0, s, A, w, n, K, L, QFIRST); } while (0)
    QP_UPD(false, 0, nb, nb);
    for (int k = 0; k < n; k += QP_B) {
        const bool trailing = k + QP_B < n;
        const int grid = trailing ? 2 * nb : nb, q_first = trailing ? nb : 0;
        if (fused) {
#define QP_STEP(NW, CPL, TPW) hipLaunchKernelGGL((qp_step_kernel<NW, CPL, TPW>), dim3(grid, n_chains), dim3(64 * NW), 0, s, A, w, n, k, L, q_first)
            if (n <= 64) QP_STEP(1, 1, 1); else if (n <= 128) QP_STEP(2, 1, 1); else if (n <= 256) QP_STEP(4, 1, 2); else if (n <= 512) QP_STEP(4, 2, 4);
            else QP_STEP(3, 3, 5);
#undef QP_STEP
            continue;
        }
#define QP_LAUNCH(NW, CPL) hipLaunchKernelGGL((qp_panel_kernel<NW, CPL>), dim3(1, n_chains), dim3(64 * NW), 0, s, A, w, n, k)
        if (n <= 64) QP_LAUNCH(1, 1); else if (n <= 128) QP_LAUNCH(2, 1); else if (n <= 256) QP_LAUNCH(4, 1); else if (n <= 512) QP_LAUNCH(4, 2);
        else if (n <= 576) QP_LAUNCH(3, 3); else if (n <= 768) QP_LAUNCH(4, 3); else QP_LAUNCH(4, 4);
#undef QP_LAUNCH
        QP_UPD(true, k, grid, q_first);
    }
#undef QP_UPD
    DQ_HIP(hipGetLastError());
    return 0;
}

}
```

Measured before the change: 13.55 sweeps/s.

## Compact live rows/columns onto one wave for late GJ and QR panel pivot searches

```diff
diff --git a/dqmc_amd/csrc/common.h b/dqmc_amd/csrc/common.h
--- a/dqmc_amd/csrc/common.h
+++ b/dqmc_amd/csrc/common.h
@@ -98,6 +98,7 @@
     double* pw = nullptr; long pw_stride = 0;
     bool pw_two_launch = false;
     int* pivpos = nullptr; long pivpos_stride = 0;
+    bool pw_compact = true;
 };
 bool qr_panel_fused_fits(int n);
 bool qr_panel_fused_default(int n);
@@ -117,7 +118,7 @@
 bool gj_fused_fits(int n);
 bool gj_fused_default(int n);
 int launch_gj_solve(Mat A, Mat B, Mat X, Mat SA, double* tinv, int* perm, long perm_stride, int* rowpos, int* rowpos_alt, long rowpos_stride,
-                    double* logabsdet, int accumulate_logdet, int* info, int n, int n_chains, bool fused, hipStream_t s);
+                    double* logabsdet, int accumulate_logdet, int* info, int n, int n_chains, bool fused, bool compact, hipStream_t s);
 
 struct UpdateTables {
     double rb[4][3];
diff --git a/dqmc_amd/csrc/engine.hip b/dqmc_amd/csrc/engine.hip
--- a/dqmc_amd/csrc/engine.hip
+++ b/dqmc_amd/csrc/engine.hip
@@ -26,7 +26,7 @@
     return 0;
 }
 
-struct Switches { bool qr_panel; int qr_panel_fused, gj_fused; bool qr_streaming, walk_submatrix, lu_classic, slice_multikernel, bbar_rider, slice_stream; };
+struct Switches { bool qr_panel; int qr_panel_fused, gj_fused; bool qr_streaming, walk_submatrix, lu_classic, slice_multikernel, bbar_rider, slice_stream, panel_compact; };
 static const Switches& switches() {
     static const Switches sw = [] {
         const char* panel = getenv("DQMC_QR_PANEL");
@@ -34,8 +34,9 @@
         const char* gj = getenv("DQMC_GJ_FUSED");
         const char* rider = getenv("DQMC_BBAR_RIDER");
         const char* stream = getenv("DQMC_SLICE_STREAM");
+        const char* compact = getenv("DQMC_PANEL_COMPACT");
         return Switches{!(panel && atoi(panel) == 0), fused ? (atoi(fused) != 0 ? 1 : 0) : -1, gj ? (atoi(gj) != 0 ? 1 : 0) : -1, getenv("DQMC_QR_STREAMING") != nullptr, getenv("DQMC_WALK_SUBMATRIX") != nullptr,
-                        getenv("DQMC_LU_CLASSIC") != nullptr, getenv("DQMC_SLICE_MULTIKERNEL") != nullptr, !(rider && atoi(rider) == 0), !(stream && atoi(stream) == 0)};
+                        getenv("DQMC_LU_CLASSIC") != nullptr, getenv("DQMC_SLICE_MULTIKERNEL") != nullptr, !(rider && atoi(rider) == 0), !(stream && atoi(stream) == 0), !(compact && atoi(compact) == 0)};
     }();
     return sw;
 }
@@ -167,6 +168,7 @@
         QrWork w{V(4).p, (long)n, keep ? out.jpvt : jpvt(), (long)n};
         w.sync = qsync.get(); w.sync_stride = qrcp_coop_sync_granules(n); w.abort_words = qabort.get(); w.info = info();
         w.pw = qpw.get(); w.pw_stride = qr_panel_work_doubles(n, qpw_two_launch); w.pw_two_launch = qpw_two_launch; w.pivpos = qpivpos.get(); w.pivpos_stride = n;
+        w.pw_compact = switches().panel_compact;
         if (out.tri) *out.tri = keep;
         out.touch();
         return launch_to_ldr(plan.qr, A, out.L, out.d, out.R, w, n, C, stream);
@@ -212,7 +214,7 @@
     }
     int solve(Mat M, Mat RHS, Mat out, double* logdet_acc, Mat* Y) {
         if (plan.solve == KernelPlan::Solve::GaussJordan) {
-            DQ_TRY(launch_gj_solve(M, RHS, out, T(5), tinv.get(), lperm(), n, rowpos(), rowpos_alt(), n, logdet_acc, 1, info(), n, C, gj_fused, stream));
+            DQ_TRY(launch_gj_solve(M, RHS, out, T(5), tinv.get(), lperm(), n, rowpos(), rowpos_alt(), n, logdet_acc, 1, info(), n, C, gj_fused, switches().panel_compact, stream));
             *Y = out; return 0;
         }
         DQ_TRY(launch_lu_blocked(M, lperm(), n, rowpos(), n, logdet_acc, 1, info(), n, C, stream));
diff --git a/dqmc_amd/csrc/lu_gj.hip b/dqmc_amd/csrc/lu_gj.hip
--- a/dqmc_amd/csrc/lu_gj.hip
+++ b/dqmc_amd/csrc/lu_gj.hip
@@ -1,6 +1,7 @@
 #include "common.h"
 #include "wave.h"
 #include <cstdlib>
+#include <type_traits>
 #include <utility>
 
 namespace dq {
@@ -180,6 +181,9 @@
 }
 
 #ifdef DQ_GJ_STAMPS
+#ifndef DQ_GJ_STAMP_K0
+#define DQ_GJ_STAMP_K0 0
+#endif
 #define GST(i) { unsigned long long t_; asm volatile("s_waitcnt lgkmcnt(0)\n\ts_memtime %0\n\ts_waitcnt lgkmcnt(0)" : "=s"(t_) :: "memory"); gst[i] += t_ - gprev; gprev = t_; }
 #define GST_ARGS , unsigned long long (&gst)[8], unsigned long long& gprev
 #define GST_PASS , gst, gprev
@@ -188,7 +192,7 @@
 #define GST_ARGS
 #define GST_PASS
 #endif
-template <int J, int NW, int RPL>
+template <int J, int NW, int RPL, bool VAL>
 __device__ __forceinline__ void gj_step_mw(double (&a)[RPL][GJ_NB], unsigned& live, int (&mypos)[RPL], int& myperm, bool& singular, int lane, int wave, int k0,
                                            double (*slot_row)[NW][GJ_NB + 2], unsigned long long (*slot_key)[(NW + 1) & ~1] GST_ARGS) {
     constexpr int PAR = J & 1;
@@ -196,7 +200,8 @@
     GST(0)
     double aj = a[0][J]; int bs = 0;
     if (RPL > 1) asm volatile("" : "+v"(aj));
-    unsigned long long key = (live & 1u) ? ((unsigned long long)__double_as_longlong(fabs(aj)) | 1ULL) : 0ULL;
+    unsigned long long key = (live & 1u) ? (VAL ? ((unsigned long long)__double_as_longlong(fabs(aj)) & ~0x1FFULL) | 0x100ULL : ((unsigned long long)__double_as_longlong(fabs(aj)) | 1ULL)) : 0ULL;
+    static_assert(!VAL || RPL == 1, "the truncated in-wave search is written for one row per lane");
 #pragma unroll
     for (int q = 1; q < RPL; ++q) {
         double v = a[q][J];
@@ -261,19 +266,104 @@
     }
     GST(6)
 }
-template <int J, int NW, int RPL>
+template <int J, int NW, int RPL, bool VAL>
 struct GjStepsMW {
     static __device__ __forceinline__ void run(double (&a)[RPL][GJ_NB], unsigned& live, int (&mypos)[RPL], int& myperm, bool& singular, int lane, int wave, int nbw, int k0,
                                                double (*slot_row)[NW][GJ_NB + 2], unsigned long long (*slot_key)[(NW + 1) & ~1] GST_ARGS) {
-        if (J < nbw) gj_step_mw<J, NW, RPL>(a, live, mypos, myperm, singular, lane, wave, k0, slot_row, slot_key GST_PASS);
-        GjStepsMW<J + 1, NW, RPL>::run(a, live, mypos, myperm, singular, lane, wave, nbw, k0, slot_row, slot_key GST_PASS);
+        if (J < nbw) gj_step_mw<J, NW, RPL, VAL>(a, live, mypos, myperm, singular, lane, wave, k0, slot_row, slot_key GST_PASS);
+        GjStepsMW<J + 1, NW, RPL, VAL>::run(a, live, mypos, myperm, singular, lane, wave, nbw, k0, slot_row, slot_key GST_PASS);
     }
 };
-template <int NW, int RPL>
-struct GjStepsMW<GJ_NB, NW, RPL> {
+template <int NW, int RPL, bool VAL>
+struct GjStepsMW<GJ_NB, NW, RPL, VAL> {
     static __device__ __forceinline__ void run(double (&)[RPL][GJ_NB], unsigned&, int (&)[RPL], int&, bool&, int, int, int, int, double (*)[NW][GJ_NB + 2],
                                                unsigned long long (*)[(NW + 1) & ~1] GST_ARGS) {}
 };
+constexpr int GJ_CMAX = 128;
+struct GjCompactShared {
+    double rows[GJ_NB][GJ_CMAX];
+    int orow[GJ_CMAX];
+    int pos[256];
+};
+template <int J, int C>
+__device__ __forceinline__ void gj_step_cw(double (&a)[C][GJ_NB], unsigned& live, const int (&orow)[C], int (&pos)[C], int& myperm, bool& singular, int lane, int k0) {
+    unsigned long long key = 0ULL; int bq = 0;
+#pragma unroll
+    for (int q = 0; q < C; ++q) {
+        const unsigned long long kq = ((live >> q) & 1u) ? ((unsigned long long)__double_as_longlong(fabs(a[q][J])) & ~0x1FFULL) | 0x100ULL : 0ULL;
+        if (kq > key) { key = kq; bq = q; }
+    }
+    const unsigned hi = (unsigned)(key >> 32), lo = (unsigned)key;
+    const unsigned m1 = wave_max_u32(hi);
+    const unsigned m2 = wave_max_u32(hi == m1 ? lo : 0u);
+    const unsigned long long winners = __ballot(hi == m1 && lo == m2 && key != 0ULL);
+    const int pl = winners ? (int)__builtin_ctzll(winners) : 0;
+    const int pq = C > 1 ? __builtin_amdgcn_readlane(bq, pl) : 0;
+    double prow[GJ_NB - J]; int prw = 0;
+#pragma unroll
+    for (int q = 0; q < C; ++q) {
+        if (q == pq) {
+#pragma unroll
+            for (int c = J; c < GJ_NB; ++c) prow[c - J] = readlane_f64(a[q][c], pl);
+            prw = __builtin_amdgcn_readlane(orow[q], pl);
+        }
+    }
+    if (lane == J) myperm = prw;
+    const double piv = prow[0];
+    singular = singular || !(fabs(piv) > 0.0);
+    double r = __builtin_amdgcn_rcp(piv);
+    r = fma(fma(-piv, r, 1.0), r, r);
+    r = fma(fma(-piv, r, 1.0), r, r);
+#pragma unroll
+    for (int q = 0; q < C; ++q) {
+        if (lane == pl && pq == q) { live &= ~(1u << q); pos[q] = k0 + J; }
+        const bool lv = (live >> q) & 1u;
+        const double l = lv ? a[q][J] * r : 0.0;
+        a[q][J] = lv ? l : a[q][J];
+#pragma unroll
+        for (int c = J + 1; c < GJ_NB; ++c) a[q][c] = fma(-l, prow[c - J], a[q][c]);
+    }
+}
+template <int J, int C>
+struct GjStepsCW {
+    static __device__ __forceinline__ void run(double (&a)[C][GJ_NB], unsigned& live, const int (&orow)[C], int (&pos)[C], int& myperm, bool& singular, int lane, int nbw, int k0) {
+        if (J < nbw) gj_step_cw<J, C>(a, live, orow, pos, myperm, singular, lane, k0);
+        GjStepsCW<J + 1, C>::run(a, live, orow, pos, myperm, singular, lane, nbw, k0);
+    }
+};
+template <int C>
+struct GjStepsCW<GJ_NB, C> {
+    static __device__ __forceinline__ void run(double (&)[C][GJ_NB], unsigned&, const int (&)[C], int (&)[C], int&, bool&, int, int, int) {}
+};
+template <int C>
+__device__ __forceinline__ void gj_chain_cw(GjCompactShared& cs, double (&LU)[GJ_NB][GJ_NB], int& s_sing, int& myperm, int nl, int lane, int nbw, int k0) {
+    double a[C][GJ_NB]; int orow[C], pos[C];
+    unsigned live = 0u;
+#pragma unroll
+    for (int q = 0; q < C; ++q) {
+        const int slot = C * lane + q;
+        const bool ok = slot < nl;
+        const int sc = ok ? slot : 0;
+#pragma unroll
+        for (int c = 0; c < GJ_NB; ++c) { const double v = cs.rows[c][sc]; a[q][c] = ok ? v : 0.0; }
+        orow[q] = ok ? cs.orow[sc] : 0;
+        pos[q] = -1;
+        live |= ok ? (1u << q) : 0u;
+    }
+    bool singular = false;
+    GjStepsCW<0, C>::run(a, live, orow, pos, myperm, singular, lane, nbw, k0);
+#pragma unroll
+    for (int q = 0; q < C; ++q) {
+        if (pos[q] >= 0) {
+            cs.pos[orow[q]] = pos[q];
+            double* dst = &LU[pos[q] - k0][0];
+#pragma unroll
+            for (int c = 0; c < GJ_NB; c += 2) *reinterpret_cast<double2*>(dst + c) = make_double2(a[q][c], a[q][c + 1]);
+        }
+    }
+    if (singular && lane == 0) s_sing = 1;
+}
+
 template <int NW, int RPL>
 struct GjPanelShared {
     double LU[GJ_NB][GJ_NB];
@@ -307,14 +397,16 @@
         }
     }
 }
-template <int NW, int RPL>
-__device__ __forceinline__ void gj_panel_factor(GjPanelShared<NW, RPL>& sh, double (&a)[RPL][GJ_NB], unsigned& live, int (&mypos)[RPL], int& myperm, int t, int nbw, int k0
+template <int NW, int RPL, bool CMP>
+__device__ __forceinline__ void gj_panel_factor(GjPanelShared<NW, RPL>& sh, double (&a)[RPL][GJ_NB], unsigned& live, int (&mypos)[RPL], int& myperm, int t, int nbw, int k0,
+                                                GjCompactShared* cs, int nl, int rank
 #ifdef DQ_GJ_STAMPS
                                                 , unsigned long long& gstart, unsigned long long& gsteps_end
 #endif
                                                 ) {
     constexpr int NWK = (NW + 1) & ~1;
     static_assert(RPL <= 4, "two key bits name the slot");
+    static_assert(!CMP || (NW == 4 && RPL == 1), "the compacted chain is written for one row per lane in at most four waves");
     const int lane = t & 63, wave = t >> 6;
     bool singular = false;
     myperm = 0;
@@ -323,6 +415,36 @@
     for (int e = t; e < GJ_NB * GJ_NB; e += blockDim.x) (&sh.LU[0][0])[e] = ((e >> 5) == (e & 31)) ? 1.0 : 0.0;
     if (t == 0) sh.s_sing = 0;
     if (t < 2 * NWK) (&sh.slot_key[0][0])[t] = 0ULL;
+    if constexpr (CMP) {
+        if (cs != nullptr && nl <= GJ_CMAX) {
+            cs->pos[t] = -1;
+            if ((live & 1u) && rank < GJ_CMAX) {
+#pragma unroll
+                for (int c = 0; c < GJ_NB; ++c) cs->rows[c][rank] = a[0][c];
+                cs->orow[rank] = t;
+            }
+            lds_wait();
+            __builtin_amdgcn_s_barrier();
+            asm volatile("" ::: "memory");
+#ifdef DQ_GJ_STAMPS
+            asm volatile("s_memtime %0\n\ts_waitcnt lgkmcnt(0)" : "=s"(gstart) :: "memory");
+#endif
+            if (wave == 0) {
+                if (nl <= 64) gj_chain_cw<1>(*cs, sh.LU, sh.s_sing, myperm, nl, lane, nbw, k0);
+                else gj_chain_cw<2>(*cs, sh.LU, sh.s_sing, myperm, nl, lane, nbw, k0);
+            }
+#ifdef DQ_GJ_STAMPS
+            asm volatile("s_waitcnt lgkmcnt(0)\n\ts_memtime %0\n\ts_waitcnt lgkmcnt(0)" : "=s"(gsteps_end) :: "memory");
+            if (t == 0 && k0 == DQ_GJ_STAMP_K0 && blockIdx.x == 0 && blockIdx.y == 0)
+                printf("gj panel k0=%d grid.x=%d, compacted: %d live rows on one wave, clocks over %d steps incl. the read-back and the deposit: %llu\n", k0, (int)gridDim.x, nl, nbw, gsteps_end - gstart);
+#endif
+            lds_wait();
+            __builtin_amdgcn_s_barrier();
+            asm volatile("" ::: "memory");
+            mypos[0] = cs->pos[t];
+            return;
+        }
+    }
     lds_wait();
     __builtin_amdgcn_s_barrier();
     asm volatile("" ::: "memory");
@@ -331,12 +453,12 @@
     unsigned long long gst[8] = {0, 0, 0, 0, 0, 0, 0, 0}, gprev;
     asm volatile("s_waitcnt vmcnt(0)\n\ts_memtime %0\n\ts_waitcnt lgkmcnt(0)" : "=s"(gprev) :: "memory"); gstart = gprev;
 #endif
-    GjStepsMW<0, NW, RPL>::run(a, live, mypos, myperm, singular, lane, wave, nbw, k0, sh.slot_row, sh.slot_key GST_PASS);
+    GjStepsMW<0, NW, RPL, CMP>::run(a, live, mypos, myperm, singular, lane, wave, nbw, k0, sh.slot_row, sh.slot_key GST_PASS);
 #ifdef DQ_GJ_STAMPS
     gsteps_end = gprev;
-    if (t == 0 && k0 == 0 && blockIdx.x == 0 && blockIdx.y == 0)
-        printf("gj panel k0=0 grid.x=%d, %d waves x %d rows per lane, clocks over %d steps (each segment includes one stamp, ~130): (loop) %llu | search %llu | publish %llu | barrier %llu | keys %llu | row %llu | fma %llu | total %llu\n",
-               (int)gridDim.x, (int)(blockDim.x >> 6), RPL, nbw, gst[0], gst[1], gst[2], gst[3], gst[4], gst[5], gst[6], gprev - gstart);
+    if (t == 0 && k0 == DQ_GJ_STAMP_K0 && blockIdx.x == 0 && blockIdx.y == 0)
+        printf("gj panel k0=%d grid.x=%d, %d waves x %d rows per lane, clocks over %d steps (each segment includes one stamp, ~130): (loop) %llu | search %llu | publish %llu | barrier %llu | keys %llu | row %llu | fma %llu | total %llu\n",
+               k0, (int)gridDim.x, (int)(blockDim.x >> 6), RPL, nbw, gst[0], gst[1], gst[2], gst[3], gst[4], gst[5], gst[6], gprev - gstart);
 #endif
 
     lds_wait();
@@ -352,13 +474,32 @@
     }
     if (singular && lane == 0) sh.s_sing = 1;
 }
+__device__ __forceinline__ int gj_compact_rank(const int* rowpos, int n, int t, bool compact, int& nl) {
+    int rank = 0;
+    nl = GJ_CMAX + 1;
+    if (compact) {
+        int tot = 0;
+        const int lane = t & 63, wave = t >> 6;
+        int pw[4];
+#pragma unroll
+        for (int w = 0; w < 4; ++w) { const int r = lane + 64 * w; pw[w] = rowpos[r < n ? r : n - 1]; }
+#pragma unroll
+        for (int w = 0; w < 4; ++w) {
+            const unsigned long long b = __ballot(lane + 64 * w < n && pw[w] < 0);
+            rank += w < wave ? __popcll(b) : (w == wave ? __popcll(b & ((1ULL << lane) - 1ULL)) : 0);
+            tot += __popcll(b);
+        }
+        nl = tot < GJ_CMAX ? tot : GJ_CMAX;
+    }
+    return rank;
+}
 #ifdef DQ_GJ_STAMPS
 #define GJ_STAMP_VM(x) asm volatile("s_waitcnt vmcnt(0)\n\ts_memtime %0\n\ts_waitcnt lgkmcnt(0)" : "=s"(x) :: "memory")
 #endif
 
 template <int NW, int RPL>
 __global__ __launch_bounds__(64 * NW) void gj_panel_mw_kernel(CMat Am, int* rowpos_p, long rowpos_stride, int* perm_p, long perm_stride, double* tinv_p,
-                                                          double* logabsdet, int accumulate, int* info, int n, int k0) {
+                                                          double* logabsdet, int accumulate, int* info, int n, int k0, int compact) {
     __shared__ __attribute__((aligned(16))) GjPanelShared<NW, RPL> sh;
     const int chain = blockIdx.y;
     const double* __restrict__ A = Am.at(chain);
@@ -375,10 +516,16 @@
     int oldpos[RPL], mypos[RPL], myperm;
     double a[RPL][GJ_NB];
     gj_panel_load<NW, RPL, false>(A, rowpos, n, k0, nbw, t, a, live, oldpos);
-#ifdef DQ_GJ_STAMPS
-    gj_panel_factor<NW, RPL>(sh, a, live, mypos, myperm, t, nbw, k0, gstart, gprev);
+    constexpr bool CMP = NW == 4 && RPL == 1;
+    __shared__ __attribute__((aligned(16))) std::conditional_t<CMP, GjCompactShared, int> s_cs;
+    GjCompactShared* cs = nullptr;
+    if constexpr (CMP) { if (compact) cs = &s_cs; }
+    int nl = GJ_CMAX + 1;
+    const int rank = CMP ? gj_compact_rank(rowpos, n, t, cs != nullptr && k0 > 0 && n - k0 <= GJ_CMAX, nl) : 0;
+#ifdef DQ_GJ_STAMPS
+    gj_panel_factor<NW, RPL, CMP>(sh, a, live, mypos, myperm, t, nbw, k0, cs, nl, rank, gstart, gprev);
 #else
-    gj_panel_factor<NW, RPL>(sh, a, live, mypos, myperm, t, nbw, k0);
+    gj_panel_factor<NW, RPL, CMP>(sh, a, live, mypos, myperm, t, nbw, k0, cs, nl, rank);
 #endif
 #pragma unroll
     for (int q = 0; q < RPL; ++q) {
@@ -397,7 +544,7 @@
 #ifdef DQ_GJ_STAMPS
     unsigned long long gend;
     GJ_STAMP_VM(gend);
-    if (t == 0 && k0 == 0 && blockIdx.y == 0) printf("   prologue %llu | steps %llu | LU hand-over (+ printf) %llu | epilogue %llu\n", gstart - gentry, gprev - gstart, gmid - gprev, gend - gmid);
+    if (t == 0 && k0 == DQ_GJ_STAMP_K0 && blockIdx.y == 0) printf("   prologue %llu | steps %llu | LU hand-over (+ printf) %llu | epilogue %llu\n", gstart - gentry, gprev - gstart, gmid - gprev, gend - gmid);
 #endif
 }
 
@@ -511,7 +658,7 @@
 
 template <int NW, int RPL>
 __global__ __launch_bounds__(64 * NW) void gj_step_kernel(Mat Am, Mat Bm, Mat SAm, Mat Xm, const int* rowpos_old_p, int* rowpos_new_p, long rowpos_stride,
-                                                          double* logabsdet, int accumulate, int* info, int n, int k0, int nA, int nS, int nCA) {
+                                                          double* logabsdet, int accumulate, int* info, int n, int k0, int nA, int nS, int nCA, int compact) {
     static_assert(NW == 4, "the update's 2 x 2 waves are the panel's");
     __shared__ __attribute__((aligned(16))) GjPanelShared<NW, RPL> sh;
     __shared__ __attribute__((aligned(16))) double s_inv[4 * 256];
@@ -535,6 +682,12 @@
     int oldpos[RPL], mypos[RPL], myperm;
     double a[RPL][GJ_NB];
     gj_panel_load<NW, RPL, true>(A, rowpos_old, n, k0, nbw, t, a, live, oldpos);
+    constexpr bool CMP = NW == 4 && RPL == 1;
+    __shared__ __attribute__((aligned(16))) std::conditional_t<CMP, GjCompactShared, int> s_cs;
+    GjCompactShared* cs = nullptr;
+    if constexpr (CMP) { if (compact) cs = &s_cs; }
+    int nl = GJ_CMAX + 1;
+    const int rank = CMP ? gj_compact_rank(rowpos_old, n, t, cs != nullptr && k0 > 0 && n - k0 <= GJ_CMAX, nl) : 0;
 
     const int row_tiles = nA + nS + 1;
     const int rt = blockIdx.x % row_tiles, ct = blockIdx.x / row_tiles;
@@ -569,9 +722,9 @@
     }
 
 #ifdef DQ_GJ_STAMPS
-    gj_panel_factor<NW, RPL>(sh, a, live, mypos, myperm, t, nbw, k0, gstart, gprev);
+    gj_panel_factor<NW, RPL, CMP>(sh, a, live, mypos, myperm, t, nbw, k0, cs, nl, rank, gstart, gprev);
 #else
-    gj_panel_factor<NW, RPL>(sh, a, live, mypos, myperm, t, nbw, k0);
+    gj_panel_factor<NW, RPL, CMP>(sh, a, live, mypos, myperm, t, nbw, k0, cs, nl, rank);
 #endif
 #pragma unroll
     for (int q = 0; q < RPL; ++q) {
@@ -661,7 +814,7 @@
 #ifdef DQ_GJ_STAMPS
     unsigned long long gend;
     GJ_STAMP_VM(gend);
-    if (t == 0 && k0 == 0 && blockIdx.x == 0 && blockIdx.y == 0)
+    if (t == 0 && k0 == DQ_GJ_STAMP_K0 && blockIdx.x == 0 && blockIdx.y == 0)
         printf("   fused step: prologue %llu | chain %llu | deposit (+ printf) %llu | inverses (wave 0) %llu | gather wait %llu | update %llu\n", gstart - gentry, gprev - gstart,
                gmid - gprev, ginv - gmid, ggather - ginv, gend - ggather);
 #endif
@@ -670,7 +823,7 @@
 bool gj_fused_default(int n) { return n > 128 && n <= 256; }
 
 int launch_gj_solve(Mat A, Mat B, Mat X, Mat SA, double* tinv, int* perm, long perm_stride, int* rowpos, int* rowpos_alt, long rowpos_stride,
-                    double* logabsdet, int accumulate_logdet, int* info, int n, int n_chains, bool fused, hipStream_t s) {
+                    double* logabsdet, int accumulate_logdet, int* info, int n, int n_chains, bool fused, bool compact, hipStream_t s) {
     if (n > 1024) { set_error("gj_solve supports n <= 1024"); return -1; }
     if (fused && rowpos_alt && gj_fused_fits(n)) {
         int p = 0;
@@ -679,14 +832,14 @@
             const int nA = (n + 31) / 32, nS = k0 / 32;
             const int nCA = (n - k0 - nbw + 31) / 32, nCB = (n + 31) / 32;
             hipLaunchKernelGGL((gj_step_kernel<4, 1>), dim3((nA + nS + 1) * (nCA + nCB), n_chains), dim3(256), 0, s, A, B, SA, X, (const int*)((p & 1) ? rowpos_alt : rowpos),
-                               (p & 1) ? rowpos : rowpos_alt, rowpos_stride, logabsdet, accumulate_logdet, info, n, k0, nA, nS, nCA);
+                               (p & 1) ? rowpos : rowpos_alt, rowpos_stride, logabsdet, accumulate_logdet, info, n, k0, nA, nS, nCA, compact ? 1 : 0);
         }
         DQ_HIP(hipGetLastError());
         return 0;
     }
     for (int k0 = 0; k0 < n; k0 += GJ_NB) {
         const dim3 pg(1, n_chains);
-#define DQ_GJ_PANEL(NW, RPL) hipLaunchKernelGGL((gj_panel_mw_kernel<NW, RPL>), pg, dim3(RPL == 1 ? 64 * ((n + 63) / 64) : 64 * NW), 0, s, CMat(A), rowpos, rowpos_stride, perm, perm_stride, tinv, logabsdet, accumulate_logdet, info, n, k0)
+#define DQ_GJ_PANEL(NW, RPL) hipLaunchKernelGGL((gj_panel_mw_kernel<NW, RPL>), pg, dim3(RPL == 1 ? 64 * ((n + 63) / 64) : 64 * NW), 0, s, CMat(A), rowpos, rowpos_stride, perm, perm_stride, tinv, logabsdet, accumulate_logdet, info, n, k0, compact ? 1 : 0)
         if (n > 768) DQ_GJ_PANEL(8, 2);
         else if (n > 576) DQ_GJ_PANEL(4, 3);
         else if (n > 512) DQ_GJ_PANEL(3, 3);
diff --git a/dqmc_amd/csrc/qr_panel.hip b/dqmc_amd/csrc/qr_panel.hip
--- a/dqmc_amd/csrc/qr_panel.hip
+++ b/dqmc_amd/csrc/qr_panel.hip
@@ -10,6 +10,17 @@
 #define QST(i) { unsigned long long t_; asm volatile("s_memtime %0\n\ts_waitcnt lgkmcnt(0)" : "=s"(t_) :: "memory"); if (threadIdx.x == 0) qst[i] = t_; }
 #else
 #define QST(i)
+#endif
+
+#ifdef DQ_QP_STAMPS
+#ifndef DQ_QP_STAMP_K
+#define DQ_QP_STAMP_K 0
+#endif
+#define QP_QST_PARAM , unsigned long long* qst
+#define QP_QST_ARG , qst
+#else
+#define QP_QST_PARAM
+#define QP_QST_ARG
 #endif
 
 constexpr int QP_B = 16;
@@ -155,6 +166,56 @@
     if (lane == 0 && wave == 0) sh.sel[J] = pcol;
 }
 
+constexpr int QP_CMAX = 64;
+template <int J, int NW>
+__device__ __forceinline__ void select_step_cw(double (&y)[QP_SEL], bool& live, int mc, int lane, PanelShared<NW>& sh) {
+    constexpr int par = J & 1;
+    double tl[4] = {0.0, 0.0, 0.0, 0.0};
+#pragma unroll
+    for (int i = J + 1; i < QP_SEL; ++i) tl[i & 3] = fma(y[i], y[i], tl[i & 3]);
+    const double tail = (tl[0] + tl[1]) + (tl[2] + tl[3]);
+    const double nrm2 = fma(y[J], y[J], tail);
+    const unsigned long long key = live ? (((unsigned long long)__double_as_longlong(nrm2) & ~0x7FFULL) | (unsigned long long)(1024 - mc)) : 0ULL;
+    const unsigned long long best = wave_max_u64(key);
+    if (best != 0ULL && key == best) {
+#pragma unroll
+        for (int i = J & ~1; i < QP_SEL; i += 2) *reinterpret_cast<double2*>(&sh.cand[par][i]) = double2{y[i], y[i + 1]};
+        sh.cand[par][QP_SEL] = tail;
+    }
+    asm volatile("s_waitcnt lgkmcnt(0)" ::: "memory");
+    const int pcol = 1024 - (int)(best & 0x7FFULL);
+    const double* xs = sh.cand[par];
+    double x[QP_SEL];
+#pragma unroll
+    for (int i = J & ~1; i < QP_SEL; i += 2) { const double2 v = *reinterpret_cast<const double2*>(&xs[i]); x[i] = v.x; x[i + 1] = v.y; }
+    double beta, tau, scale;
+    householder<1>(x[J], xs[QP_SEL], beta, tau, scale);
+    const double st = -scale * tau;
+    double dt[4] = {0.0, 0.0, 0.0, 0.0};
+#pragma unroll
+    for (int i = J + 1; i < QP_SEL; ++i) dt[i & 3] = fma(x[i], y[i], dt[i & 3]);
+    const double dot = (dt[0] + dt[1]) + (dt[2] + dt[3]);
+    const double cf = st * fma(scale, dot, y[J]);
+#pragma unroll
+    for (int i = J + 1; i < QP_SEL; ++i) y[i] = fma(x[i], cf, y[i]);
+    if (mc == pcol) live = false;
+    if (lane == 0) sh.sel[J] = pcol;
+    asm volatile("" ::: "memory");
+}
+template <int NW>
+__device__ __forceinline__ void select_compacted(double (&y)[QP_SEL], const double* cy, const int* ci, int nl, int lane, PanelShared<NW>& sh QP_QST_PARAM) {
+    bool live = lane < nl;
+    const int sc = live ? lane : 0;
+#pragma unroll
+    for (int i = 0; i < QP_SEL; ++i) { const double v = cy[i * QP_CMAX + sc]; y[i] = live ? v : 0.0; }
+    const int mc = live ? ci[sc] : -1;
+    QST(1)
+#define QP_CSTEP(J) select_step_cw<J, NW>(y, live, mc, lane, sh); QST(2 + J)
+    QP_CSTEP(0) QP_CSTEP(1) QP_CSTEP(2) QP_CSTEP(3) QP_CSTEP(4) QP_CSTEP(5) QP_CSTEP(6) QP_CSTEP(7)
+    QP_CSTEP(8) QP_CSTEP(9) QP_CSTEP(10) QP_CSTEP(11) QP_CSTEP(12) QP_CSTEP(13) QP_CSTEP(14) QP_CSTEP(15)
+#undef QP_CSTEP
+}
+
 template <int J, int NW, int CPL>
 __device__ __forceinline__ void panel_step(double (&a)[CPL][16], double (&trow)[QP_B], double& myscale, unsigned diag, unsigned blk_live, int c, int g, int wave,
                                            PanelShared<NW>& sh, double* tau_out) {
@@ -222,23 +283,25 @@
 __host__ __device__ __forceinline__ long qp_off_tm(int n) { return qp_off_vp(n) + (long)n * n; }
 __host__ __device__ __forceinline__ long qp_off_vtp(int n) { return qp_off_tm(n) + (long)QP_B * n; }
 
-#ifdef DQ_QP_STAMPS
-#define QP_QST_PARAM , unsigned long long* qst
-#define QP_QST_ARG , qst
-#else
-#define QP_QST_PARAM
-#define QP_QST_ARG
-#endif
-
-template <int NW, int CPL, class Pre, class Mid>
+
+template <int NW, int CPL, bool CMP, class Pre, class Mid>
 __device__ __forceinline__ bool qp_factor_panel(const double* A, const double* __restrict__ Y, const int* pivpos, int n, int k, PanelShared<NW>& sh,
                                                 double* tau_out, double (&a)[CPL][16], double (&trow)[QP_B], double& myscale, unsigned& diag, int& mycol,
-                                                Pre&& pre, Mid&& mid QP_QST_PARAM) {
+                                                double* cy, int* ci, Pre&& pre, Mid&& mid QP_QST_PARAM) {
+    static_assert(!CMP || (NW == 4 && CPL == 1), "the compacted selection is written for one column per lane in four waves");
     const int t = threadIdx.x, lane = t & 63, wave = t >> 6;
+    const bool compact = CMP && cy != nullptr && n - k <= QP_CMAX;
     QST(0)
     {
         unsigned live = 0u;
         double y[CPL][QP_SEL]; int pp[CPL];
+        int ppw[CMP ? 4 : 1];
+        if (CMP) {
+            if (compact) {
+#pragma unroll
+                for (int w = 0; w < 4; ++w) { const int col = lane + 64 * w; ppw[w] = pivpos[col < n ? col : n - 1]; }
+            }
+        }
 #pragma unroll
         for (int q = 0; q < CPL; ++q) {
             const int col = t + 64 * NW * q, cc = col < n ? col : n - 1;
@@ -257,11 +320,35 @@
             }
         }
         if (y[0][0] == 1.2345e300) live = 0u;
-        QST(1)
+        bool selected = false;
+        if constexpr (CMP) {
+            if (compact) {
+                QST(39)
+                int rank = 0, tot = 0;
+#pragma unroll
+                for (int w = 0; w < 4; ++w) {
+                    const unsigned long long b = __ballot(lane + 64 * w < n && ppw[w] < 0);
+                    rank += w < wave ? __popcll(b) : (w == wave ? __popcll(b & ((1ULL << lane) - 1ULL)) : 0);
+                    tot += __popcll(b);
+                }
+                const int nl = tot < QP_CMAX ? tot : QP_CMAX;
+                if ((live & 1u) && rank < QP_CMAX) {
+#pragma unroll
+                    for (int i = 0; i < QP_SEL; ++i) cy[i * QP_CMAX + rank] = y[0][i];
+                    ci[rank] = t;
+                }
+                lds_barrier();
+                if (wave == 0) select_compacted<NW>(y[0], cy, ci, nl, lane, sh QP_QST_ARG);
+                selected = true;
+            }
+        }
+        if (!selected) {
+            QST(1)
 #define QP_SEL_STEP(J) select_step<J, NW, CPL>(y, live, t, lane, wave, sh); QST(2 + J)
-        QP_SEL_STEP(0) QP_SEL_STEP(1) QP_SEL_STEP(2) QP_SEL_STEP(3) QP_SEL_STEP(4) QP_SEL_STEP(5) QP_SEL_STEP(6) QP_SEL_STEP(7)
-        QP_SEL_STEP(8) QP_SEL_STEP(9) QP_SEL_STEP(10) QP_SEL_STEP(11) QP_SEL_STEP(12) QP_SEL_STEP(13) QP_SEL_STEP(14) QP_SEL_STEP(15)
+            QP_SEL_STEP(0) QP_SEL_STEP(1) QP_SEL_STEP(2) QP_SEL_STEP(3) QP_SEL_STEP(4) QP_SEL_STEP(5) QP_SEL_STEP(6) QP_SEL_STEP(7)
+            QP_SEL_STEP(8) QP_SEL_STEP(9) QP_SEL_STEP(10) QP_SEL_STEP(11) QP_SEL_STEP(12) QP_SEL_STEP(13) QP_SEL_STEP(14) QP_SEL_STEP(15)
 #undef QP_SEL_STEP
+        }
     }
     lds_barrier();
     const int c = lane & 15, g = lane >> 4;
@@ -316,7 +403,12 @@
 #endif
     double a[CPL][16], trow[QP_B], myscale;
     unsigned diag; int mycol;
-    qp_factor_panel<NW, CPL>(A, Y, pivpos, n, k, sh, tau + k, a, trow, myscale, diag, mycol, [] { return false; }, [] {} QP_QST_ARG);
+    constexpr bool CMP = NW == 4 && CPL == 1;
+    __shared__ double s_cy[CMP ? QP_SEL * QP_CMAX : 1];
+    __shared__ int s_ci[CMP ? QP_CMAX : 1];
+    double* cy = nullptr; int* ci = nullptr;
+    if constexpr (CMP) { if (w.pw_compact) { cy = s_cy; ci = s_ci; } }
+    qp_factor_panel<NW, CPL, CMP>(A, Y, pivpos, n, k, sh, tau + k, a, trow, myscale, diag, mycol, cy, ci, [] { return false; }, [] {} QP_QST_ARG);
 #pragma unroll
     for (int b = 0; b < CPL; ++b) {
         const int r0 = 64 * NW * b + 64 * wave + 16 * g;
@@ -346,8 +438,9 @@
     asm volatile("s_waitcnt vmcnt(0)" ::: "memory");
     QST(35)
     __syncthreads();
-    if (t == 0 && k == 0 && blockIdx.y == 0) {
-        printf("panel k=0 n=%d (100 MHz ticks x 24 = clk @2.4GHz): load Y %llu | sel steps", n, qst[1] - qst[0]);
+    if (t == 0 && k == DQ_QP_STAMP_K && blockIdx.y == 0) {
+        if (cy != nullptr && n - k <= QP_CMAX) printf("panel k=%d n=%d: compaction (ranks, LDS pass, barrier, wave 0's read-back) %llu of the load segment\n", k, n, qst[1] - qst[39]);
+        printf("panel k=%d n=%d (100 MHz ticks x 24 = clk @2.4GHz): load Y %llu | sel steps", k, n, qst[1] - qst[0]);
         for (int j = 0; j < 16; ++j) printf(" %llu", qst[2 + j] - qst[1 + j]);
         printf(" | gather %llu | panel steps", qst[18] - qst[17]);
         for (int j = 0; j < 16; ++j) printf(" %llu", qst[19 + j] - qst[18 + j]);
@@ -590,7 +683,12 @@
     unsigned ticket = 0u;
     double a[CPL][16], trow[QP_B], myscale;
     unsigned diag; int mycol;
-    const bool factored = qp_factor_panel<NW, CPL>(A, Yr, pivpos, n, k, sh, s_tau, a, trow, myscale, diag, mycol, [&] {
+    constexpr bool CMP = NW == 4 && CPL == 1;
+    static_assert(!CMP || sizeof(red) >= sizeof(double) * QP_SEL * QP_CMAX, "the compaction buffer is the reduction buffer");
+    __shared__ int s_ci[CMP ? QP_CMAX : 1];
+    double* cy = nullptr; int* ci = nullptr;
+    if constexpr (CMP) { if (w.pw_compact) { cy = &red[0][0][0]; ci = s_ci; } }
+    const bool factored = qp_factor_panel<NW, CPL, CMP>(A, Yr, pivpos, n, k, sh, s_tau, a, trow, myscale, diag, mycol, cy, ci, [&] {
         if (__ballot(pp < 0) != 0ULL) return false;
         if (t == 0) s_ticket = __hip_atomic_fetch_add(counter, 1u, __ATOMIC_RELAXED, __HIP_MEMORY_SCOPE_AGENT);
         __syncthreads();
@@ -746,7 +844,8 @@
     asm volatile("s_waitcnt vmcnt(0)" ::: "memory");
     QST(38)
     __syncthreads();
-    if (t == 0 && (k == 0 || k == n / 2) && blockIdx.x == 0 && blockIdx.y == 0) {
+    if (t == 0 && (k == DQ_QP_STAMP_K || k == n / 2) && blockIdx.x == 0 && blockIdx.y == 0) {
+        if (cy != nullptr && n - k <= QP_CMAX) printf("step k=%d n=%d: compaction (ranks, LDS pass, barrier, wave 0's read-back) %llu of the load segment\n", k, n, qst[1] - qst[39]);
         printf("step k=%d n=%d (100 MHz ticks): loads %llu | sel steps", k, n, qst[1] - qst[0]);
         for (int j = 0; j < 16; ++j) printf(" %llu", qst[2 + j] - qst[1 + j]);
         printf(" | gather %llu | panel steps", qst[18] - qst[17]);
```

Result: faster. 13.76 sweeps/s, median of 6 (+1.6%).
